# JoeHEZHAO/Optical-Flow-Guided-Feature-Pytorch

Measured on AMD Instinct MI355X. Metric: OFF-forward clips/sec (7-seg 224x224), higher is better.
Workload: dtype f32 (split-fp32: every fp32 operand as three bf16 planes = the fp32 value exactly, six exact plane products on the bf16 MFMA pipe, f32 accumulate); 1 GPU; RGB_OFF forward, batch=64 clips/GPU x 7 segments, nine 224x224-geometry feature maps; global_batch=64, segments=7, parallelism=clip-shard x1, slice_mode=reference_flat

## Files before the change

optical-flow-guided-feature-pytorch_amd/csrc/conv_igemm.hip:

```cpp
#include <cstdio>
#include <cstdlib>

#include "offk_common.h"
#include "offk_internal.h"

namespace offk {

struct ConvArgs {
  const float* x; int x_cs, x_coff;
  int n_img, H, W, Ci, Ho, Wo, pad;
  const float* w;
  const float* bias;
  int Co;
  const float* res; int res_cs, res_coff;
  float* y; int y_cs, y_coff;
  int flags, M;
  int gm, gn, splitk;
  int co_limit;
  int batch;
  int spread;
  long long x_bs, w_bs, y_bs;
  int ngroups, g_batch[4], g_Ci[4];
  long long g_x[4], g_w[4], g_y[4];
  float* pool_part;
  int pool_hw;
  float* partial;
  int no_dma;
  unsigned x_bytes, w_bytes;
#ifdef OFFK_CONV_TIMING
  unsigned long long* dbg;
#endif
#ifdef OFFK_TUNING_KNOBS
  int ablate;
#endif
};

constexpr int kDmaStages = 2;
template <int KH, int KW, int S, int TM, int TN, int WM, int WN, int PREC>
__global__ __launch_bounds__(256, 1) void conv_igemm_kernel(ConvArgs p) {
  static_assert(PREC == 0 || PREC == 2 || PREC == 4, "fp32 core only");
  constexpr bool LEAN = PREC >= 2;
#ifdef OFFK_CONV_TIMING
  const unsigned long long tm_t0 = __builtin_readcyclecounter();
  unsigned long long tm_t1 = 0, tm_t2 = 0, tm_ta = 0;
#endif
  if (p.ngroups > 0) {
    int b = blockIdx.y, ci = p.g_Ci[0], first = 0;
    long long gx = p.g_x[0], gw = p.g_w[0], gy = p.g_y[0];
#pragma unroll
    for (int g = 1; g < 4; ++g) {
      first += p.g_batch[g - 1];
      if (g < p.ngroups && (int)blockIdx.y >= first) { b = blockIdx.y - first; ci = p.g_Ci[g]; gx = p.g_x[g]; gw = p.g_w[g]; gy = p.g_y[g]; }
    }
    p.x += gx + (long long)b * p.M * ci; p.w += gw + (long long)b * p.Co * ci; p.y += gy + (long long)b * p.M * p.Co;
    p.Ci = ci; p.x_cs = ci; p.x_bytes = (unsigned)p.M * (unsigned)ci * 4u; p.w_bytes = (unsigned)p.Co * (unsigned)ci * 4u;
  } else if (gridDim.y > 1) { p.x += blockIdx.y * p.x_bs; p.w += blockIdx.y * p.w_bs; p.y += blockIdx.y * p.y_bs; }
  constexpr bool DMA = PREC == 4;
  constexpr int DST = kDmaStages;
  constexpr int BM = 32 * TM * WM, BN = 32 * TN * WN;
  extern __shared__ __attribute__((aligned(16))) float smem[];
  float* As0 = smem;
  float* Bs0 = smem + 2 * BM * LDS_K;

  const int lane = threadIdx.x & 63, wave = threadIdx.x >> 6;
  const int tid = threadIdx.x & 255;
  const int wm = (wave & 3) / WN, wn = (wave & 3) % WN;
  int lid;
  {
    const int nblk = gridDim.x, bid = blockIdx.x, xcd = bid & 7, q = nblk >> 3, r = nblk & 7;
    lid = (xcd < r ? xcd * (q + 1) : r * (q + 1) + (xcd - r) * q) + (bid >> 3);
  }
  const int nt = lid % p.gn, mt = (lid / p.gn) % p.gm, zs = lid / (p.gn * p.gm);
  const int m0 = mt * BM, n0 = nt * BN;
  constexpr int TAPS = KH * KW;
  const int K = TAPS * p.Ci;
  const int nkt_all = TAPS * (p.Ci / BK);
  const int kt_begin = p.splitk == 1 ? 0 : (int)((long long)nkt_all * zs / p.splitk);
  const int kt_end = p.splitk == 1 ? nkt_all : (int)((long long)nkt_all * (zs + 1) / p.splitk);

  constexpr int RSH = 3, RSTEP = 32;
  constexpr int NRA = BM / RSTEP, NRB = BN / RSTEP;
  constexpr int VA = 1, VB = 1;
  const int kpos = DMA ? 4 * ((tid & 7) ^ ((tid >> 4) & 7)) : 4 * (tid & 7);

  int hi0[NRA], wi0[NRA];
  int pix0[NRA];
  const bool flat = TAPS == 1 && S == 1 && p.pad == 0 && LEAN;
#pragma unroll
  for (int r = 0; r < NRA; ++r) {
    int m = m0 + (tid >> RSH) + RSTEP * r;
    bool ok = m < p.M;
    if (flat) { hi0[r] = ok ? 0 : -100000; wi0[r] = 0; pix0[r] = ok ? m : 0; continue; }
    int mm = ok ? m : 0;
    int img = mm / (p.Ho * p.Wo);
    int rem = mm - img * (p.Ho * p.Wo);
    int ho = rem / p.Wo, wo = rem - ho * p.Wo;
    hi0[r] = ok ? ho * S - p.pad : -100000;
    wi0[r] = wo * S - p.pad;
    pix0[r] = img * p.H * p.W;
  }
  const float* xbase = p.x + p.x_coff + kpos;
  const bool relu_in = p.flags & OFFK_CONV_RELU_IN_;
  const float* wbase = p.w + (size_t)(n0 + (tid >> 3)) * K + 4 * (tid & 7);

  typedef unsigned u32x4 __attribute__((ext_vector_type(4)));
  int rowoff[LEAN ? NRA : 1], woff[LEAN ? NRB : 1];
  unsigned inv[LEAN ? NRA : 1];
  __amdgpu_buffer_rsrc_t xrs, wrs;
  if constexpr (LEAN) {
    const int bias_px = p.pad * p.W + p.pad;
    xrs = __builtin_amdgcn_make_buffer_rsrc(const_cast<float*>(p.x) + p.x_coff - (long)bias_px * p.x_cs, 0,
                                            (int)(p.x_bytes + (unsigned)bias_px * p.x_cs * 4u), 0x00020000);
    wrs = __builtin_amdgcn_make_buffer_rsrc(const_cast<float*>(p.w), 0, (int)p.w_bytes, 0x00020000);
#pragma unroll
    for (int r = 0; r < NRA; ++r) {
      rowoff[r] = hi0[r] < -50000 ? 0 : flat ? (pix0[r] * p.x_cs + kpos) * 4
                                             : ((pix0[r] + (hi0[r] + p.pad) * p.W + (wi0[r] + p.pad)) * p.x_cs + kpos) * 4;
      unsigned m = 0;
#pragma unroll
      for (int kh = 0; kh < KH; ++kh) m |= (unsigned)(hi0[r] + kh) >= (unsigned)p.H ? 1u << kh : 0u;
#pragma unroll
      for (int kw = 0; kw < KW; ++kw) m |= (unsigned)(wi0[r] + kw) >= (unsigned)p.W ? 0x10000u << kw : 0u;
      if (flat) m = hi0[r] < -50000 ? 1u : 0u;
      inv[r] = m;
      if constexpr (TAPS == 1) rowoff[r] = m ? (int)0x80000000 : rowoff[r];
    }
#pragma unroll
    for (int r = 0; r < NRB; ++r) woff[r] = ((n0 + (tid >> 3) + 32 * r) * K + kpos) * 4;
  }
  typedef int i32x4 __attribute__((ext_vector_type(4)));
  i32x4 xdesc = {0, 0, 0, 0}, wdesc = {0, 0, 0, 0};
  unsigned lds_base = 0;
  if constexpr (DMA) {
    const int bias_px = p.pad * p.W + p.pad;
    const unsigned long long xa = reinterpret_cast<unsigned long long>(p.x + p.x_coff - (long)bias_px * p.x_cs);
    const unsigned long long wa = reinterpret_cast<unsigned long long>(p.w);
    xdesc = i32x4{(int)(unsigned)xa, (int)(unsigned)(xa >> 32) & 0xffff, (int)(p.x_bytes + (unsigned)bias_px * p.x_cs * 4u), 0x00020000};
    wdesc = i32x4{(int)(unsigned)wa, (int)(unsigned)(wa >> 32) & 0xffff, (int)p.w_bytes, 0x00020000};
    lds_base = (unsigned)(size_t)((__attribute__((address_space(3))) char*)smem) +
               (unsigned)__builtin_amdgcn_readfirstlane((int)(threadIdx.x >> 6)) * (8 * 128);
  }
  auto dma16 = [&](const i32x4& desc, unsigned lds_addr, int voff, int soff) {
    asm volatile("s_mov_b32 m0, %0\n\ts_nop 0\n\tbuffer_load_dwordx4 %1, %2, %3 offen lds"
                 :: "s"(lds_addr), "v"(voff), "s"(desc), "s"(soff) : "memory", "m0");
  };
  int dm_soff_a = 0, dm_soff_b = 0, dm_kh = 0, dm_kw = 0;
  auto dma_prep = [&](int kt) {
    if constexpr (DMA) {
      int chunk = kt / TAPS, tap = kt - chunk * TAPS, c0 = chunk * BK;
      dm_kh = tap / KW; dm_kw = tap - dm_kh * KW;
      dm_soff_a = ((dm_kh * p.W + dm_kw) * p.x_cs + c0) * 4; dm_soff_b = kt * BK * 4;
    }
  };
  auto dma_piece = [&](const int i, const int stage) {
    if constexpr (DMA) {
      const unsigned la = lds_base + stage * (BM * 128), lb = lds_base + DST * (BM * 128) + stage * (BN * 128);
// ... 639 lines not shown
    default: return hipErrorInvalidConfiguration;
  }
}
template <int KH, int KW, int S>
static hipError_t launch_shape(const ConvArgs& a, int cfg, int prec, hipStream_t st) {
  if (prec != 0) return hipErrorInvalidValue;
  if (a.x_bytes && !(a.flags & OFFK_CONV_RELU_IN_) && !a.no_dma) return launch_prec<KH, KW, S, 4>(a, cfg, st);
  return a.x_bytes ? launch_prec<KH, KW, S, 2>(a, cfg, st) : launch_prec<KH, KW, S, 0>(a, cfg, st);
}

void conv2d_auto_plan(long long M, int Co, int nkt, int* cfg_out, int* splitk_out, int precision) {
  static const int cand[] = {1, 2, 3, 4, 6, 8, 12};
  if (precision == 0) {
    static const int cand32[] = {1, 2, 3, 4, 6, 8, 12, 16, 24, 32, 48, 64};
    const long long blocks = ((M + 63) / 64) * (Co / 64);
    int sk = 1;
    for (int c : cand32) {
      if (c > 1 && nkt / c < (blocks * sk < 512 ? 16 : 24)) break;
      sk = c;
      if (blocks * c >= 3500) break;
    }
    *cfg_out = 3;
    *splitk_out = sk;
    return;
  }
  int cfg = (nkt >= 36 && Co % 128 == 0) ? 4 : 3;
  long long blocks = ((M + kTileBM[cfg] - 1) / kTileBM[cfg]) * (Co / kTileBN[cfg]);
  int sk = 1;
  for (int c : cand) {
    if (nkt / c < 16) break;
    sk = c;
    if (blocks * c >= 1536) break;
  }
  *cfg_out = cfg;
  *splitk_out = sk;
}

hipError_t conv2d_launch(const ConvDesc& d, hipStream_t st, const char** why) {
  *why = nullptr;
  if (d.precision != 0) { *why = "conv2d: precision must be 0 (fp32; the bf16x3 mode was retired in ABI v9)"; return hipErrorInvalidValue; }
  const bool narrow = d.co_limit > 0 && d.co_limit < d.Co;
  if (d.Ci % 32 || d.Co % 64 || d.x_cs % 4 || d.x_coff % 4 || d.y_cs <= 0 || (!narrow && (d.y_cs % 4 || d.y_coff % 4)) ||
      (d.res && (d.res_cs % 4 || d.res_coff % 4))) {
    *why = "conv2d: need Ci % 32 == 0, Co % 64 == 0, 16-byte aligned channel slices";
    return hipErrorInvalidValue;
  }
  ConvArgs a;
  a.x = d.x; a.x_cs = d.x_cs; a.x_coff = d.x_coff;
  a.n_img = d.n_img; a.H = d.H; a.W = d.W; a.Ci = d.Ci; a.pad = d.pad;
  a.Ho = (d.H + 2 * d.pad - d.KH) / d.stride + 1;
  a.Wo = (d.W + 2 * d.pad - d.KW) / d.stride + 1;
  a.w = d.w; a.bias = d.bias; a.Co = d.Co;
  a.res = d.res; a.res_cs = d.res_cs; a.res_coff = d.res_coff;
  a.y = d.y; a.y_cs = d.y_cs; a.y_coff = d.y_coff;
  a.flags = d.flags;
  {
    const unsigned long long xb = ((unsigned long long)d.n_img * d.H * d.W * d.x_cs - d.x_coff) * 4ull;
    const unsigned long long bias = (unsigned long long)(d.pad * d.W + d.pad) * d.x_cs * 4ull;
    const unsigned long long wb = (unsigned long long)d.Co * d.KH * d.KW * d.Ci * 4ull;
    const bool fits = xb + bias < 0x7fffffffull && wb < 0x7fffffffull;
    a.x_bytes = fits ? (unsigned)xb : 0u;
    a.w_bytes = fits ? (unsigned)wb : 0u;
    a.no_dma = 0;
#ifdef OFFK_NO_CONV_DMA
    a.no_dma = 1;
#endif
#ifdef OFFK_TUNING_KNOBS
    { const char* e = getenv("OFFK_CONV_DMA"); if (e && *e == '0') a.no_dma = 1; }
    { const char* e = getenv("OFFK_CONV_LEAN"); if (e && !((atoi(e) >> (d.precision & 1)) & 1)) a.x_bytes = 0; }
#endif
  }
  long long M = (long long)d.n_img * a.Ho * a.Wo;
  if (M <= 0 || M > 0x7fffffffLL - 256) { *why = "conv2d: bad problem size"; return hipErrorInvalidValue; }
  a.M = (int)M;
  const int nkt = d.KH * d.KW * (d.Ci / 32);
  int cfg = d.tile_cfg, sk = d.splitk;
  if (cfg < 0 || sk < 1) conv2d_auto_plan(M, d.Co, nkt, &cfg, &sk, d.precision);
  if (sk > nkt) sk = nkt;
  if (narrow) sk = 1;
  a.co_limit = narrow ? d.co_limit : d.Co;
  a.pool_part = d.pool_part; a.pool_hw = d.pool_hw;
  a.batch = d.batch > 1 ? d.batch : 1; a.x_bs = d.x_bstride; a.w_bs = d.w_bstride; a.y_bs = d.y_bstride;
  a.ngroups = d.ngroups;
  for (int g = 0; g < 4; ++g) { a.g_batch[g] = d.g_batch[g]; a.g_Ci[g] = d.g_Ci[g]; a.g_x[g] = d.g_x[g]; a.g_w[g] = d.g_w[g]; a.g_y[g] = d.g_y[g]; }
  if (d.ngroups > 0) {
    if (d.ngroups > 4 || d.x_coff || d.y_coff || d.y_cs != d.Co) { *why = "conv2d: grouped batches are dense [M][Ci] x [Co][Ci] -> [M][Co] problems"; return hipErrorInvalidValue; }
    int nb = 0;
    for (int g = 0; g < d.ngroups; ++g) {
      if (d.g_Ci[g] < 32 || d.g_Ci[g] % 32 || d.g_batch[g] < 1) { *why = "conv2d: bad batch group"; return hipErrorInvalidValue; }
      nb += d.g_batch[g];
    }
    a.batch = nb;
  }
  if (a.batch > 1) {
    if (d.KH != 1 || d.KW != 1 || d.res || d.pool_part || cfg == 6 || cfg == 7 || cfg == 10 || a.batch > 65535) { *why = "conv2d: batched launches are plain 1x1 GEMMs on a generic tile"; return hipErrorInvalidValue; }
    sk = 1;
  }
  if (d.pool_part) {
    if (d.pool_hw < 32 || cfg == 6 || cfg == 7 || cfg == 10) { *why = "conv2d: pooled partial sums need >= 32 rows per image and a generic tile"; return hipErrorInvalidValue; }
    sk = 1;
  }
  if (sk > 1 && !d.partial) sk = 1;
  while (sk > 1 && d.partial_floats < (size_t)sk * (size_t)M * d.Co) --sk;
  a.splitk = sk; a.partial = d.partial; a.gm = a.gn = 0;
#ifdef OFFK_TUNING_KNOBS
  { const char* e = getenv("OFFK_CONV_ABLATE"); a.ablate = e ? atoi(e) : 0; }
#endif
#ifdef OFFK_CONV_TIMING
  {
    static unsigned long long* dbg = nullptr;
    if (!dbg) { (void)hipMalloc(reinterpret_cast<void**>(&dbg), 128); (void)hipMemset(dbg, 0, 128); }
    a.dbg = dbg;
    if (getenv("OFFK_CONV_TIMING_DUMP")) {
      unsigned long long h[16];
      (void)hipMemcpy(h, dbg, 128, hipMemcpyDeviceToHost);
      fprintf(stderr, "[conv timing] consumer mma %llu barrier %llu ktiles %llu | producer store %llu load-issue %llu barrier %llu\n", h[0], h[1], h[2], h[3], h[4], h[5]);
      if (h[11])
        fprintf(stderr, "[conv timing, LDS-DMA form, wave 0, cycles per block] prologue %.0f (setup %.0f, first tile %.0f)  K loop %.0f (%.1f K-tiles: %.0f per tile)  epilogue %.0f (to the last store's issue %.0f, drain %.0f) | blocks %llu\n",
                (double)h[8] / h[11], (double)h[13] / h[11], (double)(h[8] - h[13]) / h[11], (double)h[9] / h[11], (double)h[12] / h[11], (double)h[9] / (double)h[12],
                (double)h[10] / h[11], (double)h[14] / h[11], (double)(h[10] - h[14]) / h[11], h[11]);
      (void)hipMemset(dbg, 0, 128);
    }
  }
#endif
  const int key = d.KH * 100 + d.KW * 10 + d.stride;
  hipError_t e;
  if (cfg == 10) { *why = "conv2d: tile_cfg 10 (the half-chunk patch kernel) existed for the bf16x3 mode only, retired in ABI v9"; return hipErrorInvalidValue; }
  if (cfg == 6 || cfg == 7) {
    if (narrow || d.KH != d.KW || d.H != d.W || d.pad != d.KH / 2) {
      *why = "conv2d: the patch kernel (tile_cfg 6 / 7) needs a square map and pad = k / 2";
      return hipErrorInvalidValue;
    }
    if (sk > d.Ci / 32) sk = d.Ci / 32;
    a.splitk = sk;
    e = launch_patch_shape(a, d.KH, d.stride, d.H, cfg == 6 ? 4 : 2, d.precision, st);
    if (e == hipErrorInvalidConfiguration) *why = "conv2d: the patch kernel covers 7x7s2@28, 5x5s2@14, 3x3s1@14, 3x3s1@7 with Co % 128 (cfg 6) / % 64 (cfg 7)";
    return e;
  }
  switch (key) {
    case 111: e = launch_shape<1, 1, 1>(a, cfg, d.precision, st); break;
    case 331: e = launch_shape<3, 3, 1>(a, cfg, d.precision, st); break;
    case 552: e = launch_shape<5, 5, 2>(a, cfg, d.precision, st); break;
    case 772: e = launch_shape<7, 7, 2>(a, cfg, d.precision, st); break;
    default: *why = "conv2d: unsupported kernel/stride (have 1x1s1, 3x3s1, 5x5s2, 7x7s2)"; return hipErrorInvalidValue;
  }
  if (e == hipErrorInvalidConfiguration) *why = "conv2d: tile configuration does not divide Co";
  return e;
}

__global__ void pack_oihw_kernel(const float* __restrict__ src, float* __restrict__ dst, int Co, int Ci, int KHW) {
  size_t n = (size_t)Co * Ci * KHW;
  for (size_t i = blockIdx.x * (size_t)blockDim.x + threadIdx.x; i < n; i += (size_t)gridDim.x * blockDim.x) {
    int cl = (int)(i & 31);
    size_t t = i >> 5;
    int tap = (int)(t % KHW);
    t /= KHW;
    int chunk = (int)(t % (Ci >> 5));
    int co = (int)(t / (Ci >> 5));
    dst[i] = src[((size_t)co * Ci + chunk * 32 + cl) * KHW + tap];
  }
}

hipError_t pack_conv_weight_launch(const float* src, int Co, int Ci, int KH, int KW, float* dst, hipStream_t st) {
  size_t n = (size_t)Co * Ci * KH * KW;
  int blocks = (int)((n + 255) / 256);
  if (blocks > 4096) blocks = 4096;
  hipLaunchKernelGGL(pack_oihw_kernel, dim3(blocks), dim3(256), 0, st, src, dst, Co, Ci, KH * KW);
  return hipGetLastError();
}

}
```

optical-flow-guided-feature-pytorch_amd/csrc/offk_api.hip:

```cpp
#include "../../include/offk.h"

#include <algorithm>
#include <cmath>
#include <cstdio>
#include <cstdlib>
#include <cstring>
#include <map>
#include <string>
#include <vector>

#include "offk_internal.h"

using namespace offk;

typedef const void* const* MapPtrs;

static bool path_switch(const char* name, int* min_p = nullptr) {
  const char* e = getenv(name);
  if (e && min_p && atoi(e) > 1) *min_p = atoi(e);
  return !(e && *e == '0');
}

static ConvDesc conv_desc(const float* x, int x_cs, int x_coff, int n_img, int H, int W, int Ci, const float* w, const float* bias, int Co, int KH,
                          int KW, int stride, int pad, const float* res, int res_cs, int res_coff, int flags, float* y, int y_cs, int y_coff,
                          int tile_cfg = -1, int splitk = 0, float* partial = nullptr, size_t partial_floats = 0, int precision = 0) {
  ConvDesc d;
  d.x = x; d.x_cs = x_cs; d.x_coff = x_coff; d.n_img = n_img; d.H = H; d.W = W; d.Ci = Ci;
  d.w = w; d.bias = bias; d.Co = Co; d.KH = KH; d.KW = KW; d.stride = stride; d.pad = pad;
  d.res = res; d.res_cs = res_cs; d.res_coff = res_coff; d.flags = flags;
  d.y = y; d.y_cs = y_cs; d.y_coff = y_coff;
  d.tile_cfg = tile_cfg; d.splitk = splitk; d.partial = partial; d.partial_floats = partial_floats; d.precision = precision;
  return d;
}

static hipError_t wino_gemms_launch(const WinoGroup* grp, int ngrp, int npoints, int rows, int Ci, int Co, const float* V, const float* U,
                                    float* M, bool persistent, hipStream_t s, const char** why, const void* U_planes = nullptr) {
  if (persistent || U_planes) {
    WinoGemmArgs a{};
    a.x = V; a.w = U; a.y = M; a.M = rows; a.Co = Co; a.ngroups = ngrp;
    for (int gi = 0; gi < ngrp; ++gi) {
      a.g_batch[gi] = grp[gi].batch; a.g_K[gi] = grp[gi].kmul * Ci;
      a.g_x[gi] = grp[gi].v_off; a.g_w[gi] = grp[gi].u_off; a.g_y[gi] = grp[gi].m_off;
    }
    a.w_planes = U_planes;
    if (U_planes && wino_gemm_split_supported(a)) return wino_gemm_split_launch(a, s);
    if (persistent && wino_gemm_supported(a)) return wino_gemm_launch(a, s);
  }
  const int K0 = grp[0].kmul * Ci;
  ConvDesc d = conv_desc(V, K0, 0, rows, 1, 1, K0, U, nullptr, Co, 1, 1, 1, 0, nullptr, 0, 0, 0, M, Co, 0, 3, 1);
#ifdef OFFK_TUNING_KNOBS
  { const char* e = getenv("OFFK_WINO_CFG"); if (e && (Co % 128 == 0 || atoi(e) == 1 || atoi(e) == 2)) d.tile_cfg = atoi(e); }
#endif
  d.batch = npoints; d.x_bstride = (long long)rows * K0; d.w_bstride = (long long)Co * K0; d.y_bstride = (long long)rows * Co;
  if (ngrp > 1) {
    d.ngroups = ngrp;
    for (int gi = 0; gi < ngrp; ++gi) {
      d.g_batch[gi] = grp[gi].batch; d.g_Ci[gi] = grp[gi].kmul * Ci;
      d.g_x[gi] = grp[gi].v_off; d.g_w[gi] = grp[gi].u_off; d.g_y[gi] = grp[gi].m_off;
    }
  }
  return conv2d_launch(d, s, why);
}
static bool wino_gemm_stage_default() {
  static const bool on = path_switch("OFFK_WINO_GEMM");
  return on;
}

namespace {

struct SiteSpec { const char* name; int C, H; };
const SiteSpec kSites[kNumSites] = {{"3a", 256, 28}, {"3b", 320, 28}, {"3c", 576, 14}, {"4a", 576, 14}, {"4b", 576, 14},
                                    {"4c", 608, 14}, {"4d", 608, 14}, {"5a", 1024, 7}, {"5b", 1024, 7}};
const int kPwOrder[kNumSites] = {7, 8, 5, 6, 2, 3, 4, 1, 0};
const int kSiteFusion[kNumSites] = {0, 0, 1, 1, 1, 1, 1, 2, 2};
const int kSiteCoff[kNumSites] = {0, 160, 0, 160, 320, 480, 640, 0, 160};
const int kFusionC[3] = {320, 1056, 832};

struct ConvSpec { const char* key; int Co, Ci, K, stride, pad; };
enum ConvId {
  C_T28, C1_28A, C2_28A, C3_28A, CB_28A, C1_28B, C2_28B, C3_28B, C1_28C, C2_28C, C3_28C,
  C_T14, C1_14A, C2_14A, C3_14A, CE_14A, C1_14B, C2_14B, C3_14B,
  C_T7, C1_7, C2_7, C3_7, CB_7, kNumConvs
};
const ConvSpec kConvs[kNumConvs] = {
    {"motion_conv_trans_28", 64, 320, 7, 2, 3},      {"motion_conv1_trans_28a", 64, 64, 1, 1, 0},
    {"motion_conv2_trans_28a", 64, 64, 3, 1, 1},     {"motion_conv3_trans_28a", 256, 64, 1, 1, 0},
    {"motion_conv_branch_28a", 256, 64, 1, 1, 0},    {"motion_conv1_trans_28b", 64, 256, 1, 1, 0},
    {"motion_conv2_trans_28b", 64, 64, 3, 1, 1},     {"motion_conv3_trans_28b", 256, 64, 1, 1, 0},
    {"motion_conv1_trans_28c", 64, 256, 1, 1, 0},    {"motion_conv2_trans_28c", 64, 64, 3, 1, 1},
    {"motion_conv3_trans_28c", 256, 64, 1, 1, 0},    {"motion_conv_trans_14", 128, 1056, 5, 2, 2},
    {"motion_conv1_trans_14a", 128, 128, 1, 1, 0},   {"motion_conv2_trans_14a", 128, 128, 3, 1, 1},
    {"motion_conv3_trans_14a", 512, 128, 1, 1, 0},   {"motion_conv_expand_trans_14a", 512, 128, 1, 1, 0},
    {"motion_conv1_trans_14b", 128, 512, 1, 1, 0},   {"motion_conv2_trans_14b", 128, 128, 3, 1, 1},
    {"motion_conv3_trans_14b", 512, 128, 3, 1, 1},   {"motion_conv_trans", 256, 832, 3, 1, 1},
    {"motion_conv1_trans", 256, 256, 1, 1, 0},       {"motion_conv2_trans", 256, 256, 3, 1, 1},
    {"motion_conv3_trans", 1024, 256, 1, 1, 0},      {"motion_conv_branch_trans", 1024, 256, 1, 1, 0}};
struct MergedSpec { const char* name; int main_id, branch_id; };
const MergedSpec kMerged[3] = {{"merged_28a", C3_28A, CB_28A}, {"merged_14a", C3_14A, CE_14A}, {"merged_7", C3_7, CB_7}};
const int kTunedP240[kNumConvs][2] = {
    {3, 2}, {-1, 0}, {-1, 0}, {-1, 0}, {-1, 0}, {-1, 0}, {-1, 0}, {-1, 0}, {-1, 0}, {-1, 0}, {-1, 0},
    {4, 4}, {-1, 0}, {-1, 0}, {-1, 0}, {-1, 0}, {-1, 0}, {-1, 0}, {-1, 0},
    {-1, 0}, {-1, 0}, {-1, 0}, {-1, 0}, {-1, 0}};
const int kMergedPlan[2][3][2] = {
    {{3, 1}, {3, 1}, {3, 1}},
    {{1, 1}, {3, 1}, {3, 1}}};
struct HeadSpec { const char* key; int C; };
const HeadSpec kHeads[3] = {{"fc_action_motion", 1024}, {"fc_action_motion_28", 256}, {"fc_action_motion_14", 512}};
const char* kSobelKey = "sobel_edge_diagonal.conv.weight";

enum SlotKind { SK_GEN_W, SK_GEN_B, SK_DOWN_W, SK_DOWN_B, SK_DW_W, SK_DW_B, SK_SOBEL, SK_CONV_W, SK_CONV_B, SK_FC_W, SK_FC_B };
struct Slot {
  std::string key;
  std::vector<int64_t> shape;
  SlotKind kind;
  int idx;
  bool set = false;
};

struct Derived {
  float* u = nullptr;
  float* u_planes = nullptr;
  float* u2 = nullptr;
  float* planes = nullptr;
  float* gemm_planes = nullptr;
  float* head = nullptr;
};
constexpr int kNumDerived = kNumConvs + 3;
constexpr int merged_slot(int m) { return kNumConvs + m; }

thread_local std::string g_err;

size_t align_up(size_t v, size_t a) { return (v + a - 1) / a * a; }

}

struct offk_handle {
  offk_config cfg;
  int N = 0, P = 0;
  std::vector<Slot> slots;
  std::map<std::string, int> index;
  float* pw_w[kNumSites] = {};
  float* pw_wt16[kNumSites] = {};
// ... 87 lines not shown

constexpr size_t kTraceMaxEvents = 1 << 16;
int trace_mark(offk_handle* h, hipStream_t st, const char* name) {
  if (h->profiling != 2 || h->tr_marks.size() >= kTraceMaxEvents) return OFFK_OK;
  int id = -1;
  if (name) {
    for (size_t i = 0; i < h->tr_names.size() && id < 0; ++i)
      if (h->tr_names[i] == name) id = (int)i;
    if (id < 0) { id = (int)h->tr_names.size(); h->tr_names.push_back(name); }
  }
  if (h->tr_marks.size() >= h->tr_events.size()) {
    hipEvent_t e;
    HIP_TRY(h, hipEventCreate(&e));
    h->tr_events.push_back(e);
  }
  HIP_TRY(h, hipEventRecord(h->tr_events[h->tr_marks.size()], st));
  h->tr_marks.push_back(id);
  return OFFK_OK;
}

int dev_alloc(offk_handle* h, float** p, size_t nfloats) {
  void* q = nullptr;
  HIP_TRY(h, hipMalloc(&q, nfloats * sizeof(float)));
  HIP_TRY(h, hipMemset(q, 0, nfloats * sizeof(float)));
  h->allocs.push_back(q);
  *p = static_cast<float*>(q);
  return OFFK_OK;
}

void add_slot(offk_handle* h, const std::string& key, std::vector<int64_t> shape, SlotKind kind, int idx) {
  Slot s;
  s.key = key; s.shape = std::move(shape); s.kind = kind; s.idx = idx;
  h->index[key] = (int)h->slots.size();
  h->slots.push_back(std::move(s));
}

void add_region(offk_handle* h, const std::string& name, size_t nfloats) {
  size_t off = align_up(h->ws_bytes, 256);
  h->regions[name] = std::make_pair(off, nfloats * sizeof(float));
  h->ws_bytes = off + nfloats * sizeof(float);
}

float* region(const offk_handle* h, void* ws, const char* name) {
  auto it = h->regions.find(name);
  return reinterpret_cast<float*>(static_cast<char*>(ws) + it->second.first);
}

void ub_plan(int H, int* strips, int* rows) {
  *rows = H >= 28 ? 7 : H;
  *strips = (H + *rows - 1) / *rows;
}
constexpr int kUbTpix = 8;

void plan_workspace(offk_handle* h) {
  const size_t N = h->N, P = h->P;
  for (int s = 0; s < kNumSites; ++s) {
    size_t hw = (size_t)kSites[s].H * kSites[s].H;
    add_region(h, std::string("G_") + kSites[s].name, N * hw * kGenCh);
    add_region(h, std::string("D_") + kSites[s].name, P * hw * kDownCh);
  }
  add_region(h, "fusion_28", P * 784 * 320);
  add_region(h, "fusion_14", P * 196 * 1056);
  add_region(h, "fusion_7", P * 49 * 832);
  add_region(h, "xt_28", P * 196 * 128);
  add_region(h, "t1_28", P * 196 * 64);
  add_region(h, "sa_28", P * 196 * 256);
  add_region(h, "sb_28", P * 196 * 256);
  add_region(h, "xu_14", P * 49 * 256);
  add_region(h, "u1_14", P * 49 * 128);
  add_region(h, "sa_14", P * 49 * 512);
  add_region(h, "xv_7", P * 49 * 512);
  add_region(h, "v1_7", P * 49 * 256);
  add_region(h, "sum_7", P * 49 * 1024);
  add_region(h, "logit_7", P * (size_t)h->cfg.num_classes);
  add_region(h, "logit_14", P * (size_t)h->cfg.num_classes);
  add_region(h, "logit_28", P * (size_t)h->cfg.num_classes);
  add_region(h, "pooled_7", P * 1024);
  add_region(h, "pooled_14", P * 512);
  add_region(h, "pooled_28", P * 256);
  add_region(h, "poolpart_28", (size_t)4 * P * 256);
  add_region(h, "poolpart_7", ((P * 49 + 31) / 32) * 2 * 1024);
  add_region(h, "poolpart_14", ((P * 49 + 31) / 32) * 2 * 512);
  if (h->cfg.precision == OFFK_PRECISION_FP32) {
    add_region(h, "wino_v", std::max((size_t)kWinoUnits4 * P * 1056, (size_t)kWino7Tiles * P * kWino7Units * 320));
    add_region(h, "wino_m", (size_t)kWinoPoints * P * 512);
    add_region(h, "poolpart_14t", (size_t)4 * P * 512);
    if (h->pool_first7) add_region(h, "poolpart_7t", (size_t)4 * P * 512);
  }
  h->splitk_floats = (size_t)std::min<size_t>(64, std::max<size_t>(8, 1536 / P)) * P * 196 * 64;
  add_region(h, "splitk", h->splitk_floats);
  h->ws_bytes = align_up(h->ws_bytes, 256);

  const size_t fwd_bytes = h->ws_bytes;
  long long work = 0;
  for (int s = 0; s < kNumSites; ++s) {
    const int hw = kSites[s].H * kSites[s].H;
    work += (long long)N * ((hw + 31) / 32) * ((kSites[s].C + 127) / 128);
  }
  h->wg_kpb = (int)std::max<long long>(4, (work + 1535) / 1536);
  for (int s = 0; s < kNumSites; ++s) {
    const size_t hw = (size_t)kSites[s].H * kSites[s].H;
    const std::string n = kSites[s].name;
    int strips, rows;
    ub_plan(kSites[s].H, &strips, &rows);
    const size_t kt_total = N * ((hw + 31) / 32), nchunks = (kt_total + h->wg_kpb - 1) / h->wg_kpb;
    const size_t cpad = (size_t)((kSites[s].C + 127) / 128) * 128;
    add_region(h, "dG_" + n, N * hw * kGenCh);
    add_region(h, "dD_" + n, P * hw * kDownCh);
    add_region(h, "dwp_" + n, P * strips * 10 * kDownCh);
    add_region(h, "wgs_" + n, nchunks * kUnitCh * cpad);
    add_region(h, "wgb_" + n, nchunks * kUnitCh);
    auto slot = [&](const std::string& key, size_t count) {
      h->grad_slots[key] = std::make_pair(h->grad_floats, count);
      h->grad_floats += count;
    };
    slot("motion_conv_gen_" + n + ".weight", (size_t)kGenCh * kSites[s].C);
    slot("motion_conv_gen_" + n + ".bias", kGenCh);
    slot("motion_spatial_down_" + n + ".weight", (size_t)kDownCh * kSites[s].C);
    slot("motion_spatial_down_" + n + ".bias", kDownCh);
    if (h->cfg.variant != OFFK_VARIANT_DIAG_SOBEL) {
      slot("motion_spatial_grad_" + n + ".weight", (size_t)kDownCh * 9);
      slot("motion_spatial_grad_" + n + ".bias", kDownCh);
    }
  }
  h->train_ws_bytes = align_up(h->ws_bytes, 256);
  h->ws_bytes = fwd_bytes;
}

struct DeviceGuard {
  int prev = -1;
  bool changed = false;
  explicit DeviceGuard(int want) {
    if (hipGetDevice(&prev) == hipSuccess && prev != want) changed = hipSetDevice(want) == hipSuccess;
  }
  ~DeviceGuard() { if (changed) (void)hipSetDevice(prev); }
};

int check_ready(offk_handle* h) {
  for (const Slot& s : h->slots)
    if (!s.set) return fail(h, OFFK_ERR_MISSING_WEIGHT, "weight not set: " + s.key);
  return OFFK_OK;
}

bool slot_set(const offk_handle* h, const std::string& key) {
  auto it = h->index.find(key);
  return it != h->index.end() && h->slots[it->second].set;
}

int site_weights_ready(offk_handle* h, int site, bool need_pw, bool need_dw) {
  const std::string n = kSites[site].name;
  if (need_pw)
    for (const char* k : {"motion_conv_gen_", "motion_spatial_down_"})
      for (const char* sfx : {".weight", ".bias"})
        if (!slot_set(h, std::string(k) + n + sfx)) return fail(h, OFFK_ERR_MISSING_WEIGHT, std::string("weight not set: ") + k + n + sfx);
  if (need_dw) {
    if (h->cfg.variant == OFFK_VARIANT_DIAG_SOBEL) {
      if (!slot_set(h, kSobelKey)) return fail(h, OFFK_ERR_MISSING_WEIGHT, std::string("weight not set: ") + kSobelKey);
    } else {
      for (const char* sfx : {".weight", ".bias"})
        if (!slot_set(h, "motion_spatial_grad_" + n + sfx)) return fail(h, OFFK_ERR_MISSING_WEIGHT, "weight not set: motion_spatial_grad_" + n + sfx);
    }
  }
  return OFFK_OK;
}

void pw_weight_ptrs(const offk_handle* h, int site, const float** w, const float** w_down, const float** b,
                    const float** b_down) {
// ... 219 lines not shown
  for (int i = 0; i < kNumSites; ++i) {
    const int s = kPwOrder[i];
    PtSite& o = pt.s[i];
    const offk_feat_parts& fp = feats[s];
    for (int q = 0; q < 4; ++q) { o.xp[q] = q < fp.n_parts ? fp.data[q] : nullptr; o.cp[q] = q < fp.n_parts ? fp.channels[q] : 0; }
    o.nparts = fp.n_parts;
    pw_weight_ptrs(h, s, &o.w, &o.w_down, &o.bias, &o.bias_down);
    o.wt = nullptr;
    o.wt16 = h->pw_wt16[s];
    o.wt16s = h->pw_wt16s[s];
    o.D = region(h, ws, (std::string("D_") + kSites[s].name).c_str());
    o.M = region(h, ws, fus[kSiteFusion[s]]);
    o.m_cs = kFusionC[kSiteFusion[s]]; o.m_coff = kSiteCoff[s];
    o.C = kSites[s].C; o.HW = kSites[s].H * kSites[s].H;
  }
  if (ev) HIP_TRY(h, hipEventRecord(ev[0], st));
  TRY(launch_k1t(h, st, pt, feat_dtype, cl));
  if (ev) HIP_TRY(h, hipEventRecord(ev[1], st));
  { int rc = trace_mark(h, st, "units:sobel S-blocks (K2 spatial half)"); if (rc != OFFK_OK) return rc; }
  { int rc = run_sobel_tdiff_all(h, st, ws, 3); if (rc != OFFK_OK) return rc; }
  if (ev) HIP_TRY(h, hipEventRecord(ev[2], st));
  return OFFK_OK;
}

int check_feat_train(offk_handle* h, const FeatKind& k, int feat_dtype, const void* const* feats, int first, int count, const char* fn) {
  const std::string f(fn), maps = std::string(": ") + k.noun + " feature map";
  if (!(feat_dtype == OFFK_FEAT_F32 && k.f32_ok) && feat_dtype != OFFK_FEAT_BF16 && feat_dtype != OFFK_FEAT_F16)
    return fail(h, OFFK_ERR_INVALID, f + ": unknown feat_dtype " + std::to_string(feat_dtype) + " (OFFK_FEAT_F32 / _BF16 / _F16)");
  if (!k.cl && h->cfg.feat_layout == OFFK_FEAT_NHWC) return fail(h, OFFK_ERR_INVALID, f + maps + "s are NCHW-only (this handle is NHWC)");
  for (int i = 0; i < count; ++i) {
    const SiteSpec& site = kSites[first + i];
    if (!feats[i]) return fail(h, OFFK_ERR_INVALID, f + ": null feature map");
    if (reinterpret_cast<uintptr_t>(feats[i]) & (k.align_train - 1))
      return fail(h, OFFK_ERR_INVALID, f + maps + " pointers must be " + std::to_string(k.align_train) + "-byte aligned (site " + site.name + ")");
    if (feat_dtype != OFFK_FEAT_F32 && (unsigned long long)h->N * site.H * site.H * site.C * 2ull >= kFeat16MaxBytes)
      return fail(h, OFFK_ERR_INVALID, f + ": 16-bit feature maps of 2 GiB or more are not supported (site " + site.name + ")");
  }
  return OFFK_OK;
}

int pw_reduce_site(offk_handle* h, void* stream, const FeatKind* k, int feat_dtype, int site, const void* feat, float* G, float* D, const char* fn) {
  if (!h || site < 0 || site >= kNumSites || !feat || !G || !D) return fail(h, OFFK_ERR_INVALID, std::string(fn) + ": bad argument");
  if (k) TRY(check_feat_train(h, *k, feat_dtype, &feat, site, 1, fn));
  TRY(site_weights_ready(h, site, true, false));
  DeviceGuard guard(h->cfg.device);
  hipStream_t st = static_cast<hipStream_t>(stream);
  PwParams pp;
  memset(&pp, 0, sizeof(pp));
  pp.nsites = 1; pp.L = h->cfg.length; pp.P = h->P; pp.slice_mode = h->cfg.slice_mode;
  pp.nhwc = k ? k->cl : h->cfg.feat_layout == OFFK_FEAT_NHWC;
  pp.zeros = h->zero_page;
  TRY(finalize_pw(h, st));
  fill_pw_site(h, site, whole_map(site, static_cast<const float*>(feat)), G, D, &pp.s[0]);
  pp.total_blocks = pw_blocks_for(pp.s[0].M);
  return launch_k1(h, st, pp, feat_dtype, false);
}

int off_units_whole(offk_handle* h, void* stream, const FeatKind* k, int feat_dtype, const void* const feats[OFFK_NUM_SITES], void* workspace,
                    bool train, uint64_t drop_seed, double drop_p, const char* fn) {
  if (!h || !feats || !workspace) return fail(h, OFFK_ERR_INVALID, std::string(fn) + ": null argument");
  DropCfg drop;
  if (train) TRY(make_drop(h, drop_seed, drop_p, &drop));
  if (k) TRY(check_feat_train(h, *k, feat_dtype, feats, 0, kNumSites, fn));
  offk_feat_parts parts[kNumSites];
  TRY(whole_maps(h, feats, parts, fn));
  for (int s = 0; s < kNumSites; ++s) TRY(site_weights_ready(h, s, true, true));
  DeviceGuard guard(h->cfg.device);
  return run_off_units(h, static_cast<hipStream_t>(stream), parts, workspace, nullptr, k ? k->cl : h->cfg.feat_layout == OFFK_FEAT_NHWC, drop,
                       feat_dtype);
}

struct View { const float* p; int cs, coff; };

enum DerivedKind {
  DK_U_F43,
  DK_U_POLY,
  DK_U_F54,
  DK_CHAIN_U2,
  DK_PLANES,
  DK_U_PLANES,
  DK_HEAD_COMPOSED
};
DerivedKind u_kind(const ConvSpec& c) { return c.K == 7 ? DK_U_F54 : c.K == 5 ? DK_U_POLY : DK_U_F43; }
int u_units(DerivedKind k) { return k == DK_U_F54 ? kWino7Units : k == DK_U_POLY ? kWinoUnits4 : kWinoPoints; }
size_t u_elems(const ConvSpec& c) { return (size_t)u_units(u_kind(c)) * c.Co * c.Ci; }
int wino_phases(const ConvSpec& c) { return u_kind(c) == DK_U_POLY ? 4 : 1; }
int wino_conv_groups(const ConvSpec& c, long long rows, WinoGroup grp[4]) {
  return u_kind(c) == DK_U_F54 ? wino7_groups(rows, c.Ci, c.Co, grp) : wino_groups(wino_phases(c), rows, c.Ci, c.Co, grp);
}
size_t plane_floats(size_t elems) { return (elems * 3 + 1) / 2; }

enum { ON_7X7 = 1, ON_SPLIT_GEMM = 2, ON_CHAIN_WINO = 4, ON_SPLIT_CHAIN = 8, ON_SPLIT_MID = 16, ON_POOL_FIRST7 = 32 };
struct DerivedRow {
  int slot;
  DerivedKind kind;
  float* Derived::*image;
  int needs = 0;
  int skip_bit = 0;
  int alloc_K = 0;
};
bool derived_exists(const offk_handle* h, const DerivedRow& r) {
  const int on = h->wino_7x7 * ON_7X7 | h->split_gemm * ON_SPLIT_GEMM | h->chain_wino * ON_CHAIN_WINO | (h->chain && h->split_chain) * ON_SPLIT_CHAIN |
                 (h->wino_mid && h->split_mid) * ON_SPLIT_MID | h->pool_first7 * ON_POOL_FIRST7;
  const bool shape = r.kind != DK_U_PLANES || (kConvs[r.slot].Co % 64 == 0 && kConvs[r.slot].Ci >= 64);
  return h->winograd && !(r.needs & ~on) && shape && !(h->split_gemm_skip & r.skip_bit);
}

const DerivedRow kDerived[] = {
    {C3_14B, DK_U_F43, &Derived::u}, {C_T7, DK_U_F43, &Derived::u}, {C2_7, DK_U_F43, &Derived::u}, {C2_14A, DK_U_F43, &Derived::u},
    {C2_14B, DK_U_F43, &Derived::u}, {C_T14, DK_U_POLY, &Derived::u}, {C_T28, DK_U_F54, &Derived::u, ON_7X7},
    {C3_14B, DK_U_PLANES, &Derived::u_planes, ON_SPLIT_GEMM, 1}, {C_T7, DK_U_PLANES, &Derived::u_planes, ON_SPLIT_GEMM, 2},
    {C2_7, DK_U_PLANES, &Derived::u_planes, ON_SPLIT_GEMM, 4}, {C2_14A, DK_U_PLANES, &Derived::u_planes, ON_SPLIT_GEMM, 8},
    {C2_14B, DK_U_PLANES, &Derived::u_planes, ON_SPLIT_GEMM, 16}, {C_T14, DK_U_PLANES, &Derived::u_planes, ON_SPLIT_GEMM, 32},
    {C_T28, DK_U_PLANES, &Derived::u_planes, ON_7X7 | ON_SPLIT_GEMM, 64},
    {merged_slot(1), DK_PLANES, &Derived::gemm_planes, ON_SPLIT_GEMM, 128}, {merged_slot(2), DK_PLANES, &Derived::gemm_planes, ON_SPLIT_GEMM, 128},
    {C1_14B, DK_PLANES, &Derived::gemm_planes, ON_SPLIT_GEMM, 128},
    {C2_28A, DK_CHAIN_U2, &Derived::u2, ON_CHAIN_WINO}, {C2_28B, DK_CHAIN_U2, &Derived::u2, ON_CHAIN_WINO}, {C2_28C, DK_CHAIN_U2, &Derived::u2, ON_CHAIN_WINO},
    {C1_28A, DK_PLANES, &Derived::planes, ON_SPLIT_CHAIN, 0, 256}, {C2_28A, DK_PLANES, &Derived::planes, ON_SPLIT_CHAIN}, {C3_28A, DK_PLANES, &Derived::planes, ON_SPLIT_CHAIN},
    {CB_28A, DK_PLANES, &Derived::planes, ON_SPLIT_CHAIN},
    {C1_28B, DK_PLANES, &Derived::planes, ON_SPLIT_CHAIN}, {C2_28B, DK_PLANES, &Derived::planes, ON_SPLIT_CHAIN}, {C3_28B, DK_PLANES, &Derived::planes, ON_SPLIT_CHAIN},
    {C1_28C, DK_PLANES, &Derived::planes, ON_SPLIT_CHAIN}, {C2_28C, DK_PLANES, &Derived::planes, ON_SPLIT_CHAIN}, {C3_28C, DK_PLANES, &Derived::planes, ON_SPLIT_CHAIN},
    {C1_14A, DK_PLANES, &Derived::planes, ON_SPLIT_MID}, {C1_7, DK_PLANES, &Derived::planes, ON_SPLIT_MID},
    {merged_slot(2), DK_HEAD_COMPOSED, &Derived::head, ON_POOL_FIRST7}};

struct Matrix { const float* w; int Co, K; };
Matrix slot_matrix(const offk_handle* h, int slot) {
  if (slot < kNumConvs) return Matrix{h->conv_w[slot], kConvs[slot].Co, kConvs[slot].Ci * kConvs[slot].K * kConvs[slot].K};
  const MergedSpec& m = kMerged[slot - kNumConvs];
  return Matrix{h->merged_w[slot - kNumConvs], kConvs[m.main_id].Co, kConvs[m.main_id].Ci + kConvs[m.branch_id].Ci};
}
size_t derived_floats(const offk_handle* h, const DerivedRow& r) {
  switch (r.kind) {
    case DK_U_F43: case DK_U_POLY: case DK_U_F54: return (size_t)u_units(r.kind) * kConvs[r.slot].Co * kConvs[r.slot].Ci;
    case DK_CHAIN_U2: return (size_t)16 * 64 * 64;
    case DK_PLANES: { const Matrix m = slot_matrix(h, r.slot); return plane_floats((size_t)m.Co * (r.alloc_K ? r.alloc_K : m.K)); }
    case DK_U_PLANES: return plane_floats(u_elems(kConvs[r.slot]));
    case DK_HEAD_COMPOSED: return (size_t)h->cfg.num_classes * (slot_matrix(h, r.slot).K + 1);
  }
  return 0;
}
int pack_derived(offk_handle* h, const DerivedRow& r, hipStream_t st) {
  const Derived& d = h->derived[r.slot];
  switch (r.kind) {
    case DK_U_F43: case DK_U_POLY:
      HIP_TRY(h, wino_weight_launch(h->conv_w[r.slot], kConvs[r.slot].Co, kConvs[r.slot].Ci, wino_phases(kConvs[r.slot]), d.u, st));
      break;
    case DK_U_F54: HIP_TRY(h, wino7_weight_launch(h->conv_w[r.slot], kConvs[r.slot].Co, kConvs[r.slot].Ci, d.u, st)); break;
    case DK_CHAIN_U2: HIP_TRY(h, chain_wino_weight_launch(h->conv_w[r.slot], d.u2, st)); break;
    case DK_PLANES: {
      const Matrix m = slot_matrix(h, r.slot);
      HIP_TRY(h, wino_pack_split_launch(m.w, d.*r.image, m.Co, m.K, 1, st));
      break;
    }
    case DK_U_PLANES: {
      const ConvSpec& c = kConvs[r.slot];
      WinoGroup grp[4];
      const int ngrp = wino_conv_groups(c, 1, grp);
      for (int g = 0; g < ngrp; ++g)
        HIP_TRY(h, wino_pack_split_launch(d.u + grp[g].u_off, reinterpret_cast<char*>(d.u_planes) + grp[g].u_off * 6, c.Co, grp[g].kmul * c.Ci, grp[g].batch, st));
      break;
    }
    case DK_HEAD_COMPOSED: {
      const Matrix m = slot_matrix(h, r.slot);
      HIP_TRY(h, head_compose_launch(h->fc_w[0], h->fc_b[0], h->cfg.num_classes, m.w, h->merged_b[r.slot - kNumConvs], m.Co, m.K, d.head,
                                     d.head + (size_t)h->cfg.num_classes * m.K, st));
      break;
    }
  }
  return OFFK_OK;
}

int finalize_merged(offk_handle* h, hipStream_t st) {
  if (!h->merged_dirty) return OFFK_OK;
  for (int m = 0; m < 3; ++m) {
    const ConvSpec& a = kConvs[kMerged[m].main_id];
    const ConvSpec& b = kConvs[kMerged[m].branch_id];
    const size_t K = (size_t)a.Ci + b.Ci;
    HIP_TRY(h, hipMemcpy2DAsync(h->merged_w[m], K * 4, h->conv_w[kMerged[m].main_id], (size_t)a.Ci * 4, (size_t)a.Ci * 4, a.Co, hipMemcpyDeviceToDevice, st));
    HIP_TRY(h, hipMemcpy2DAsync(h->merged_w[m] + a.Ci, K * 4, h->conv_w[kMerged[m].branch_id], (size_t)b.Ci * 4, (size_t)b.Ci * 4, a.Co, hipMemcpyDeviceToDevice, st));
    HIP_TRY(h, vec_add_launch(h->conv_b[kMerged[m].main_id], h->conv_b[kMerged[m].branch_id], h->merged_b[m], a.Co, st));
  }
  h->merged_dirty = false;
  return OFFK_OK;
}
int finalize_derived(offk_handle* h, hipStream_t st) {
  if (!h->derived_dirty) return OFFK_OK;
  for (const DerivedRow& r : kDerived)
    if (h->derived[r.slot].*r.image) TRY(pack_derived(h, r, st));
  h->derived_dirty = false;
  return OFFK_OK;
}

constexpr int RI = OFFK_CONV_RELU_IN_, RP = OFFK_CONV_RELU_PRE_, RO = OFFK_CONV_RELU_POST_;
int trace_mark(offk_handle* h, hipStream_t st, const char* key, const char* what) {
  return h->profiling != 2 ? OFFK_OK : trace_mark(h, st, (std::string(key) + what).c_str());
}
WinoMidArgs wino_mid_args(const float* M, const float* bias_in, int phases_in, int n_img, int Cin, float* x, int x_cs, int x_coff, const float* w1,
                          const float* b1, int Cmid, float* V, const void* w1p = nullptr) {
  WinoMidArgs m;
  m.M = M; m.bias_in = bias_in; m.phases_in = phases_in; m.x = x; m.x_cs = x_cs; m.x_coff = x_coff;
  m.w1 = w1; m.b1 = b1; m.Cin = Cin; m.Cmid = Cmid; m.n_img = n_img; m.V = V; m.w1p = w1p;
  return m;
}
ChainArgs chain_args(const float* x, int x_cs, int x_coff, int n_img, int Cin, int relu_in, const float* w1, const float* b1, const float* w2,
                     const float* b2, const float* w3, const float* b3, int K3, const float* res, int res_cs, int res_coff, float* y, int y_cs,
                     int y_coff) {
  ChainArgs a{};
  a.x = x; a.x_cs = x_cs; a.x_coff = x_coff; a.Cin = Cin; a.relu_in = relu_in ? 1 : 0;
  a.w1 = w1; a.b1 = b1; a.w2 = w2; a.b2 = b2; a.w3 = w3; a.b3 = b3; a.K3 = K3;
  a.res = res; a.res_cs = res_cs; a.res_coff = res_coff; a.y = y; a.y_cs = y_cs; a.y_coff = y_coff;
  a.n_img = n_img; a.relu_out = 1;
  const unsigned long long xb = ((unsigned long long)n_img * 196 * x_cs - x_coff) * 4ull;
  a.x_bytes = xb < 0x7fffffffull ? (unsigned)xb : 0u;
  return a;
}

struct Fwd {
  offk_handle* h;
  hipStream_t s;
  void* ws;
  int n;
  hipEvent_t* ev = nullptr;
  float *F14, *F7;
  float *wino_V, *wino_M;
  float* splitk;
  float *out7, *out14, *out28;
  float *l7, *l14, *l28;
  FcPooledJobs fcj{};
  bool wino, w7, mid, w5, chained, fold, fold14t, pool7;

  float* reg(const char* name) const { return region(h, ws, name); }

  int init(offk_handle* handle, hipStream_t st, void* workspace, float* o7, float* o14, float* o28, bool stage_only = false) {
    h = handle; s = st; ws = workspace; n = h->P; out7 = o7; out14 = o14; out28 = o28;
    if (h->profiling == 1 && !stage_only) {
      const size_t per = OFFK_NUM_STAGES + 1;
      if ((h->ev_used + 1) * per > h->events.size() && h->events.size() < 4096 * per) {
        for (size_t i = 0; i < per; ++i) {
          hipEvent_t e;
          HIP_TRY(h, hipEventCreate(&e));
          h->events.push_back(e);
        }
      }
      if ((h->ev_used + 1) * per <= h->events.size()) ev = &h->events[h->ev_used++ * per];
    }
    wino = h->winograd;
    w7 = h->derived[C_T28].u && wino && h->wino_7x7 && n >= h->wino7_min_p;
    mid = wino && h->wino_mid;
    w5 = wino && h->wino_5x5 && n >= h->wino5_min_p;
    chained = h->chain && n >= h->chain_min_p && (unsigned long long)n * 196 * 256 * 4ull < 0x7fffffffull;
    auto generic = [](int cfg) { return cfg != 6 && cfg != 7 && cfg != 10; };
    fold = h->fold_pool && generic(h->conv_cfg[C3_14B]) && generic(h->merged_cfg[2]);
    fold14t = wino && h->fold_pool;
    pool7 = h->pool_first7 && mid && fold14t && h->derived[merged_slot(2)].head;
    F14 = reg("fusion_14"); F7 = reg("fusion_7"); splitk = reg("splitk");
    wino_V = wino ? reg("wino_v") : nullptr;
    wino_M = wino ? reg("wino_m") : nullptr;
    const bool cons = h->cfg.consensus == OFFK_CONSENSUS_AVG;
    l7 = cons ? reg("logit_7") : out7; l14 = cons ? reg("logit_14") : out14; l28 = cons ? reg("logit_28") : out28;
    fcj.n_img = n; fcj.ncls = h->cfg.num_classes;
    return OFFK_OK;
  }

  int conv_raw(const char* name, int Co, int Ci, int K, int stride, int pad, const float* w, const float* bias, int cfg, int sk, int H, View x,
               const float* res, int res_cs, int res_coff, int flags, float* y, int y_cs, int y_coff, const void* w_planes, float* pool_part) {
    if (w_planes && K == 1 && stride == 1 && pad == 0 && !res && !(flags & OFFK_CONV_RELU_IN_)) {
      WinoGemmArgs a{};
      a.x = x.p; a.w = w; a.y = y; a.M = n * H * H; a.Co = Co; a.ngroups = 1; a.g_batch[0] = 1; a.g_K[0] = Ci;
      a.w_planes = w_planes;
      a.epilogue = 1; a.x_rs = x.cs; a.x_coff = x.coff; a.y_rs = y_cs; a.y_coff = y_coff; a.bias = bias;
      a.relu = (flags & (OFFK_CONV_RELU_PRE_ | OFFK_CONV_RELU_POST_)) ? 1 : 0;
      a.pool_part = pool_part; a.pool_hw = pool_part ? H * H : 0;
      if (wino_gemm_split_supported(a)) {
        TRY(trace_mark(h, s, name));
        hipError_t e = wino_gemm_split_launch(a, s);
        if (e != hipSuccess) return fail_hip(h, e, name);
        return OFFK_OK;
      }
    }
    ConvDesc d = conv_desc(x.p, x.cs, x.coff, n, H, H, Ci, w, bias, Co, K, K, stride, pad, res, res_cs, res_coff, flags, y, y_cs, y_coff, cfg, sk,
                           splitk, h->splitk_floats, h->cfg.precision);
    d.pool_part = pool_part; d.pool_hw = pool_part ? H * H / (stride * stride) : 0;
    const char* why = nullptr;
    TRY(trace_mark(h, s, name));
    hipError_t e = conv2d_launch(d, s, &why);
    if (e != hipSuccess) return fail(h, why ? OFFK_ERR_INVALID : OFFK_ERR_HIP, std::string(name) + ": " + (why ? why : hipGetErrorString(e)));
    return OFFK_OK;
  }
  int conv(ConvId id, int H, View x, const float* res, int res_cs, int res_coff, int flags, float* y, int y_cs, int y_coff, float* pool_part = nullptr) {
    const ConvSpec& c = kConvs[id];
    return conv_raw(c.key, c.Co, c.Ci, c.K, c.stride, c.pad, h->conv_w[id], h->conv_b[id], h->conv_cfg[id], h->conv_splitk[id], H, x, res, res_cs,
                    res_coff, flags, y, y_cs, y_coff, h->derived[id].gemm_planes, pool_part);
  }
  int conv_merged(int m, int H, View x, int flags, float* y, int y_cs, int y_coff, float* pool_part = nullptr) {
    const Matrix w = slot_matrix(h, merged_slot(m));
    return conv_raw(kMerged[m].name, w.Co, w.K, 1, 1, 0, w.w, h->merged_b[m], h->merged_cfg[m], h->merged_sk[m], H, x, nullptr, 0, 0, flags, y, y_cs,
                    y_coff, h->derived[merged_slot(m)].gemm_planes, pool_part);
  }

  int wino_in(ConvId id, View x) {
    const ConvSpec& c = kConvs[id];
    TRY(trace_mark(h, s, c.key, " [winograd: input transform]"));
    if (u_kind(c) == DK_U_F54) HIP_TRY(h, wino7_input_launch(x.p, x.cs, x.coff, n, c.Ci, wino_V, s));
    else HIP_TRY(h, wino_input_launch(x.p, x.cs, x.coff, n, c.Ci, wino_phases(c), wino_V, s));
    return OFFK_OK;
  }
  int wino_mm(ConvId id) {
    const ConvSpec& c = kConvs[id];
    const bool f54 = u_kind(c) == DK_U_F54;
    TRY(trace_mark(h, s, c.key, f54 ? " [winograd: 64 GEMMs]" : " [winograd: 121 GEMMs]"));
    const int rows = f54 ? kWino7Tiles * n : n;
    WinoGroup grp[4];
    const int ngrp = wino_conv_groups(c, rows, grp);
    const char* why = nullptr;
    hipError_t e = wino_gemms_launch(grp, ngrp, f54 ? kWino7Points : kWinoPoints, rows, c.Ci, c.Co, wino_V, h->derived[id].u, wino_M, h->wino_gemm, s, &why,
                                     h->derived[id].u_planes);
    if (e != hipSuccess) return fail(h, why ? OFFK_ERR_INVALID : OFFK_ERR_HIP, std::string(c.key) + " (winograd): " + (why ? why : hipGetErrorString(e)));
    return OFFK_OK;
  }
  int wino_out(ConvId id, const float* res, int res_cs, int res_coff, int flags, float* y, int y_cs, int y_coff, float* pool_t, int pool_cs = 0) {
    const ConvSpec& c = kConvs[id];
    TRY(trace_mark(h, s, c.key, " [winograd: output transform]"));
    if (u_kind(c) == DK_U_F54) HIP_TRY(h, wino7_output_launch(wino_M, n, c.Co, h->conv_b[id], flags, y, y_cs, y_coff, s));
    else HIP_TRY(h, wino_output_launch(wino_M, n, c.Co, wino_phases(c), h->conv_b[id], res, res_cs, res_coff, flags, y, y_cs, y_coff, pool_t, s, pool_cs, 0));
    return OFFK_OK;
  }
  int wino_conv(ConvId id, View x, const float* res, int res_cs, int res_coff, int flags, float* y, int y_cs, int y_coff, float* pool_t) {
    TRY(wino_in(id, x));
    TRY(wino_mm(id));
    return wino_out(id, res, res_cs, res_coff, flags, y, y_cs, y_coff, pool_t);
  }
  int wino_between(ConvId a, ConvId c1, float* xa, int xa_cs, int xa_coff, const char* name, float* pool_t = nullptr) {
    const bool has = c1 != kNumConvs;
    WinoMidArgs m = wino_mid_args(wino_M, h->conv_b[a], wino_phases(kConvs[a]), n, kConvs[a].Co, xa, xa_cs, xa_coff, has ? h->conv_w[c1] : nullptr,
                                        has ? h->conv_b[c1] : nullptr, kConvs[has ? c1 : a].Co, wino_V, has ? h->derived[c1].planes : nullptr);
    m.pool_part = pool_t; m.pool_cs = xa_cs; m.pool_coff = xa_coff;
    TRY(trace_mark(h, s, name));
    HIP_TRY(h, wino_mid_launch(m, s));
    return OFFK_OK;
  }
  int conv_t_c1_c2(ConvId ct, bool wino_t, int H, View F, ConvId c1, ConvId c2, float* xx, int cs, float* t, const char* between,
                   float* pool_t = nullptr) {
    const int half = cs / 2;
    if (wino_t && mid) {
      TRY(wino_in(ct, F));
      TRY(wino_mm(ct));
      TRY(wino_between(ct, c1, xx, cs, half, between, pool_t));
      TRY(wino_mm(c2));
      return wino_out(c2, nullptr, 0, 0, RP, xx, cs, 0, pool_t, pool_t ? cs : 0);
    }
    if (wino_t) TRY(wino_conv(ct, F, nullptr, 0, 0, RP, xx, cs, half, nullptr));
    else TRY(conv(ct, H, F, nullptr, 0, 0, RP, xx, cs, half));
    TRY(conv(c1, 7, View{xx, cs, half}, nullptr, 0, 0, RP, t, half, 0));
    if (wino) return wino_conv(c2, View{t, half, 0}, nullptr, 0, 0, RP, xx, cs, 0, nullptr);
    return conv(c2, 7, View{t, half, 0}, nullptr, 0, 0, RP, xx, cs, 0);
  }

  int chain(const char* name, View x, int Cin, int relu_in, ConvId c1, ConvId c2, ConvId c3, int m, bool split_branch, const float* res, float* y, int y_cs, int y_coff) {
    const bool merged = m >= 0 && !split_branch;
    ChainArgs a = chain_args(x.p, x.cs, x.coff, n, Cin, relu_in, h->conv_w[c1], h->conv_b[c1], h->conv_w[c2], h->conv_b[c2],
                             merged ? h->merged_w[m] : h->conv_w[c3], merged ? h->merged_b[m] : h->conv_b[c3], merged ? 128 : 64, res, 256, 0, y, y_cs, y_coff);
    a.u2 = h->derived[c2].u2;
    a.w1p = h->derived[c1].planes; a.w2p = h->derived[c2].planes; a.w3p = h->derived[c3].planes;
    if (split_branch) { a.wbp = h->derived[kMerged[m].branch_id].planes; a.bbr = h->conv_b[kMerged[m].branch_id]; }
    TRY(trace_mark(h, s, name));
    const char* why = nullptr;
    hipError_t e = chain14_split_supported(a) ? chain14_split_launch(a, s, &why) : chain14_launch(a, s, &why);
    if (e != hipSuccess) return fail(h, why ? OFFK_ERR_INVALID : OFFK_ERR_HIP, std::string(name) + ": " + (why ? why : hipGetErrorString(e)));
    return OFFK_OK;
  }

  int head(int k, float* logits, const float* part, int tiles, const float* x, int x_cs, int x_coff, int Hh, int maxpool, const char* pooled_name) {
    const int C = kHeads[k].C;
    if (part) { fcj.job[fcj.njobs++] = FcPooledJob{part, 49, tiles, C, h->fc_w[k], h->fc_b[k], logits}; return OFFK_OK; }
    float* pooled = reg(pooled_name);
    TRY(trace_mark(h, s, k == 0 ? "head_7 (pool + fc)" : k == 1 ? "head_28 (pool + fc)" : "head_14 (pool + fc)"));
    hipError_t e = pool_launch(x, x_cs, x_coff, n, Hh, Hh, C, maxpool, pooled, s);
    if (e == hipSuccess) e = fc_launch(pooled, n, C, h->fc_w[k], h->fc_b[k], h->cfg.num_classes, logits, s);
    if (e != hipSuccess) return fail_hip(h, e, "head");
    return OFFK_OK;
  }

  int units(const offk_feat_parts feats[], int feat_dtype, bool cl) {
    if (cl) return run_off_units_fused(h, s, feats, ws, ev, feat_dtype, true);
    if (h->fused_units && h->cfg.feat_layout != OFFK_FEAT_NHWC) return run_off_units_fused(h, s, feats, ws, ev, feat_dtype);
    return run_off_units(h, s, feats, ws, ev, h->cfg.feat_layout == OFFK_FEAT_NHWC);
  }

  int fusion28() {
    float *F28 = reg("fusion_28"), *xt = reg("xt_28"), *t1 = reg("t1_28"), *sa = reg("sa_28"), *sb = reg("sb_28");
    if (w7) TRY(wino_conv(C_T28, View{F28, 320, 0}, nullptr, 0, 0, 0, xt, 128, 64, nullptr));
    else TRY(conv(C_T28, 28, View{F28, 320, 0}, nullptr, 0, 0, 0, xt, 128, 64));
    if (chained) {
      TRY(chain("chain_28a = motion_conv1_trans_28a + motion_conv2_trans_28a + merged_28a", View{xt, 128, 64}, 64, 1, C1_28A, C2_28A, C3_28A, 0,
                h->derived[CB_28A].planes != nullptr, nullptr, sa, 256, 0));
      TRY(chain("chain_28b = motion_conv1_trans_28b + motion_conv2_trans_28b + motion_conv3_trans_28b", View{sa, 256, 0}, 256, 0, C1_28B, C2_28B, C3_28B,
// ... 909 lines not shown
  if (!x || !w || !y || n_img < 1 || H < 1 || W < 1) return fail(nullptr, OFFK_ERR_INVALID, "offk_conv2d: bad argument");
  return offk_conv2d_ex(stream, x, x_cstride, x_coff, n_img, H, W, Ci, w, bias, Co, KH, KW, stride, pad, res, res_cstride, res_coff, flags, y,
                        y_cstride, y_coff, -1, 0, nullptr, 0, 0);
}

int offk_conv2d_ex(void* stream, const float* x, int x_cstride, int x_coff, int n_img, int H, int W, int Ci, const float* w,
                   const float* bias, int Co, int KH, int KW, int stride, int pad, const float* res, int res_cstride,
                   int res_coff, int flags, float* y, int y_cstride, int y_coff, int tile_cfg, int splitk, float* partial,
                   size_t partial_floats, int precision) {
  if (!x || !w || !y || n_img < 1 || H < 1 || W < 1) return fail(nullptr, OFFK_ERR_INVALID, "offk_conv2d_ex: bad argument");
  const ConvDesc d = conv_desc(x, x_cstride, x_coff, n_img, H, W, Ci, w, bias, Co, KH, KW, stride, pad, res, res_cstride, res_coff, flags, y,
                               y_cstride, y_coff, tile_cfg, splitk, partial, partial_floats, precision);
  const char* why = nullptr;
  hipError_t e = conv2d_launch(d, static_cast<hipStream_t>(stream), &why);
  if (e != hipSuccess) return fail(nullptr, why ? OFFK_ERR_INVALID : OFFK_ERR_HIP, why ? why : hipGetErrorString(e));
  return OFFK_OK;
}

int offk_bottleneck_chain14(void* stream, const float* x, int x_cstride, int x_coff, int n_img, int Cin, int relu_in,
                            const float* w1, const float* b1, const float* w2_packed, const float* b2, const float* w3,
                            const float* b3, int K3, const float* res, int res_cstride, int res_coff, float* y, int y_cstride,
                            int y_coff) {
  if (!x || !w1 || !b1 || !w2_packed || !b2 || !w3 || !b3 || !y || n_img < 1)
    return fail(nullptr, OFFK_ERR_INVALID, "offk_bottleneck_chain14: bad argument");
  const ChainArgs a = chain_args(x, x_cstride, x_coff, n_img, Cin, relu_in, w1, b1, w2_packed, b2, w3, b3, K3, res, res_cstride, res_coff, y,
                                 y_cstride, y_coff);
  const char* why = nullptr;
  hipError_t e = chain14_launch(a, static_cast<hipStream_t>(stream), &why);
  if (e != hipSuccess) return fail(nullptr, why ? OFFK_ERR_INVALID : OFFK_ERR_HIP, why ? why : hipGetErrorString(e));
  return OFFK_OK;
}

int offk_bottleneck_chain14_split(void* stream, const float* x, int x_cstride, int x_coff, int n_img, int Cin, int relu_in,
                                  const float* w1, const float* b1, const float* w2_packed, const float* b2, const float* w3,
                                  const float* b3, const float* branch_w, const float* branch_b, const float* res, int res_cstride,
                                  int res_coff, float* y, int y_cstride, int y_coff, void* scratch, size_t scratch_bytes) {
  const char* who = "offk_bottleneck_chain14_split";
  if (!x || !w1 || !b1 || !w2_packed || !b2 || !w3 || !b3 || !y || !scratch || n_img < 1 || (Cin != 64 && Cin != 256) || (branch_w && !branch_b))
    return fail(nullptr, OFFK_ERR_INVALID, std::string(who) + ": bad argument");
  if (x_coff < 0 || y_coff < 0 || (res && res_coff < 0)) return fail(nullptr, OFFK_ERR_INVALID, std::string(who) + ": negative channel offset");
  if (x_cstride < x_coff + Cin) return fail(nullptr, OFFK_ERR_INVALID, std::string(who) + ": x_cstride < x_coff + Cin");
  if (y_cstride < y_coff + 256) return fail(nullptr, OFFK_ERR_INVALID, std::string(who) + ": y_cstride < y_coff + 256");
  if (res && res_cstride < res_coff + 256) return fail(nullptr, OFFK_ERR_INVALID, std::string(who) + ": res_cstride < res_coff + 256");
  if (branch_w && res) return fail(nullptr, OFFK_ERR_INVALID, std::string(who) + ": the branch form takes no residual (res must be NULL)");
  {
    const size_t rows = (size_t)n_img * 196 * sizeof(float);
    const uintptr_t y0 = reinterpret_cast<uintptr_t>(y), y1 = y0 + rows * (size_t)y_cstride;
    const uintptr_t x0 = reinterpret_cast<uintptr_t>(x), x1 = x0 + rows * (size_t)x_cstride;
    if (y0 < x1 && x0 < y1) return fail(nullptr, OFFK_ERR_INVALID, std::string(who) + ": y overlaps x (the chain does not run in place)");
    if (res) {
      const uintptr_t r0 = reinterpret_cast<uintptr_t>(res), r1 = r0 + rows * (size_t)res_cstride;
      if (y0 < r1 && r0 < y1) return fail(nullptr, OFFK_ERR_INVALID, std::string(who) + ": y overlaps res (the chain does not run in place)");
    }
  }
  const size_t e1 = (size_t)64 * Cin, e2 = (size_t)64 * 576, e3 = (size_t)256 * 64;
  if (scratch_bytes < 6 * (e1 + e2 + 2 * e3)) return fail(nullptr, OFFK_ERR_INVALID, std::string(who) + ": scratch too small");
  hipStream_t st = static_cast<hipStream_t>(stream);
  char* sp = static_cast<char*>(scratch);
  ChainArgs a = chain_args(x, x_cstride, x_coff, n_img, Cin, relu_in, w1, b1, w2_packed, b2, w3, b3, 64, res, res_cstride, res_coff, y, y_cstride,
                           y_coff);
  a.w1p = sp; a.w2p = sp + 6 * e1; a.w3p = sp + 6 * (e1 + e2);
  hipError_t e = wino_pack_split_launch(w1, const_cast<void*>(a.w1p), 64, Cin, 1, st);
  if (e == hipSuccess) e = wino_pack_split_launch(w2_packed, const_cast<void*>(a.w2p), 64, 576, 1, st);
  if (e == hipSuccess) e = wino_pack_split_launch(w3, const_cast<void*>(a.w3p), 256, 64, 1, st);
  if (e == hipSuccess && branch_w) {
    a.wbp = sp + 6 * (e1 + e2 + e3); a.bbr = branch_b;
    e = wino_pack_split_launch(branch_w, const_cast<void*>(a.wbp), 256, 64, 1, st);
  }
  if (e != hipSuccess) return fail_hip(nullptr, e, who);
  const char* why = nullptr;
  e = chain14_split_launch(a, st, &why);
  if (e != hipSuccess) return fail(nullptr, why ? OFFK_ERR_INVALID : OFFK_ERR_HIP, std::string(who) + ": " + (why ? why : hipGetErrorString(e)));
  return OFFK_OK;
}

namespace {
int winograd_entry(const char* who, void* stream, const float* x, int x_cstride, int x_coff, int n_img, int Ci, int phases,
                   const float* w_packed, const float* bias, int Co, const float* res, int res_cstride, int res_coff, int flags,
                   float* y, int y_cstride, int y_coff, float* scratch, size_t scratch_floats, float* pool_part) {
  if (!x || !w_packed || !y || !scratch || n_img < 1 || Ci < 32 || (Ci & 31) || Co < 64 || (Co & 63) || (flags & OFFK_CONV_RELU_IN_))
    return fail(nullptr, OFFK_ERR_INVALID, std::string(who) + ": bad argument (Ci % 32 == 0, Co % 64 == 0, no RELU_IN)");
  const bool f54 = phases == 7;
  const size_t T = f54 ? (size_t)kWino7Tiles * n_img : (size_t)n_img;
  const size_t units = f54 ? kWino7Units : phases == 4 ? kWinoUnits4 : kWinoPoints, points = f54 ? kWino7Points : kWinoPoints;
  const size_t need = units * Ci * ((size_t)Co + T) + points * T * Co;
  if (scratch_floats < need) return fail(nullptr, OFFK_ERR_INVALID, std::string(who) + ": scratch too small");
  hipStream_t st = static_cast<hipStream_t>(stream);
  float* U = scratch;
  float* V = U + units * Co * Ci;
  float* M = V + units * T * Ci;
  hipError_t e = f54 ? wino7_weight_launch(w_packed, Co, Ci, U, st) : wino_weight_launch(w_packed, Co, Ci, phases, U, st);
  if (e == hipSuccess) e = f54 ? wino7_input_launch(x, x_cstride, x_coff, n_img, Ci, V, st) : wino_input_launch(x, x_cstride, x_coff, n_img, Ci, phases, V, st);
  if (e != hipSuccess) return fail_hip(nullptr, e, who);
  WinoGroup grp[4];
  const int ngrp = f54 ? wino7_groups((long long)T, Ci, Co, grp) : wino_groups(phases, (long long)T, Ci, Co, grp);
  {
    const char* why = nullptr;
    e = wino_gemms_launch(grp, ngrp, (int)points, (int)T, Ci, Co, V, U, M, wino_gemm_stage_default(), st, &why);
    if (e != hipSuccess) return fail(nullptr, why ? OFFK_ERR_INVALID : OFFK_ERR_HIP, why ? why : hipGetErrorString(e));
  }
  e = f54 ? wino7_output_launch(M, n_img, Co, bias, flags, y, y_cstride, y_coff, st)
          : wino_output_launch(M, n_img, Co, phases, bias, res, res_cstride, res_coff, flags, y, y_cstride, y_coff, pool_part, st);
  if (e != hipSuccess) return fail_hip(nullptr, e, who);
  return OFFK_OK;
}
}

int offk_winograd_conv3x3(void* stream, const float* x, int x_cstride, int x_coff, int n_img, int Ci, const float* w_packed,
                          const float* bias, int Co, const float* res, int res_cstride, int res_coff, int flags, float* y,
                          int y_cstride, int y_coff, float* scratch, size_t scratch_floats, float* pool_part) {
  return winograd_entry("offk_winograd_conv3x3", stream, x, x_cstride, x_coff, n_img, Ci, 1, w_packed, bias, Co, res, res_cstride,
                        res_coff, flags, y, y_cstride, y_coff, scratch, scratch_floats, pool_part);
}

int offk_winograd_conv5x5s2(void* stream, const float* x, int x_cstride, int x_coff, int n_img, int Ci, const float* w_packed,
                            const float* bias, int Co, const float* res, int res_cstride, int res_coff, int flags, float* y,
                            int y_cstride, int y_coff, float* scratch, size_t scratch_floats) {
  return winograd_entry("offk_winograd_conv5x5s2", stream, x, x_cstride, x_coff, n_img, Ci, 4, w_packed, bias, Co, res, res_cstride,
                        res_coff, flags, y, y_cstride, y_coff, scratch, scratch_floats, nullptr);
}

int offk_winograd_conv7x7s2(void* stream, const float* x, int x_cstride, int x_coff, int n_img, int Ci, const float* w_packed,
                            const float* bias, int Co, int flags, float* y, int y_cstride, int y_coff, float* scratch,
                            size_t scratch_floats) {
  return winograd_entry("offk_winograd_conv7x7s2", stream, x, x_cstride, x_coff, n_img, Ci, 7, w_packed, bias, Co, nullptr, 0, 0, flags, y, y_cstride,
                        y_coff, scratch, scratch_floats, nullptr);
}

int offk_winograd_between(void* stream, const float* M, const float* bias_in, int phases_in, int n_img, int Cin, float* x,
                          int x_cstride, int x_coff, const float* w1, const float* b1, int Cmid, float* V) {
  const char* who = "offk_winograd_between";
  if (!M || !V || n_img < 1 || (w1 && !b1) || (x && (x_cstride < x_coff + Cin || (x_cstride & 3) || (x_coff & 3) || x_coff < 0)))
    return fail(nullptr, OFFK_ERR_INVALID, std::string(who) + ": bad argument");
  if (!wino_mid_supported(Cin, Cmid, w1 != nullptr, phases_in))
    return fail(nullptr, OFFK_ERR_INVALID, std::string(who) + ": shape not built ((Cin, Cmid) = (128, 128) / (256, 256); phases_in 1, or 4 with Cin 128)");
  hipError_t e = wino_mid_launch(wino_mid_args(M, bias_in, phases_in, n_img, Cin, x, x_cstride, x_coff, w1, b1, Cmid, V), static_cast<hipStream_t>(stream));
  if (e != hipSuccess) return fail_hip(nullptr, e, who);
  return OFFK_OK;
}

int offk_winograd_between_ex(void* stream, const float* M, const float* bias_in, int phases_in, int n_img, int Cin, float* x,
                             int x_cstride, int x_coff, const float* w1, const float* b1, int Cmid, float* V, int precision,
                             void* scratch, size_t scratch_bytes) {
  const char* who = "offk_winograd_between_ex";
  if (precision == OFFK_PRECISION_FP32) return offk_winograd_between(stream, M, bias_in, phases_in, n_img, Cin, x, x_cstride, x_coff, w1, b1, Cmid, V);
  if (precision != OFFK_PRECISION_F32SPLIT || !w1 || !b1 || !scratch || scratch_bytes < (size_t)Cmid * Cin * 6)
    return fail(nullptr, OFFK_ERR_INVALID, std::string(who) + ": split-fp32 needs the 1x1 conv and Cmid * Cin * 6 bytes of scratch");
  if (!M || !V || n_img < 1 || (x && (x_cstride < x_coff + Cin || (x_cstride & 3) || (x_coff & 3) || x_coff < 0)))
    return fail(nullptr, OFFK_ERR_INVALID, std::string(who) + ": bad argument");
  if (!wino_mid_supported(Cin, Cmid, true, phases_in))
    return fail(nullptr, OFFK_ERR_INVALID, std::string(who) + ": shape not built ((Cin, Cmid) = (128, 128) / (256, 256); phases_in 1, or 4 with Cin 128)");
  hipStream_t st = static_cast<hipStream_t>(stream);
  hipError_t e = wino_pack_split_launch(w1, scratch, Cmid, Cin, 1, st);
  if (e != hipSuccess) return fail_hip(nullptr, e, who);
  e = wino_mid_launch(wino_mid_args(M, bias_in, phases_in, n_img, Cin, x, x_cstride, x_coff, w1, b1, Cmid, V, scratch), st);
  if (e != hipSuccess) return fail_hip(nullptr, e, who);
  return OFFK_OK;
}

int offk_batched_gemm_nt(void* stream, const float* x, const float* w, float* y, int batch, int M, int K, int Co, int precision,
                         void* scratch, size_t scratch_bytes) {
  const char* who = "offk_batched_gemm_nt";
  if (!x || !w || !y || batch < 1 || M < 1 || K < 32 || (K & 31) || Co < 64 || (Co & 63))
    return fail(nullptr, OFFK_ERR_INVALID, std::string(who) + ": bad argument (K % 32 == 0, Co % 64 == 0)");
  if (precision != OFFK_PRECISION_FP32 && precision != OFFK_PRECISION_F32SPLIT)
    return fail(nullptr, OFFK_ERR_INVALID, std::string(who) + ": precision must be OFFK_PRECISION_FP32 or OFFK_PRECISION_F32SPLIT");
  hipStream_t st = static_cast<hipStream_t>(stream);
  WinoGroup grp{batch, 1, 0, 0, 0};
  const void* planes = nullptr;
  if (precision == OFFK_PRECISION_F32SPLIT) {
    if (K < 64) return fail(nullptr, OFFK_ERR_INVALID, std::string(who) + ": the split-fp32 form takes K >= 64");
    if (!scratch || scratch_bytes < (size_t)batch * Co * K * 6)
      return fail(nullptr, OFFK_ERR_INVALID, std::string(who) + ": scratch smaller than batch * Co * K * 6 bytes (the plane image of w)");
    hipError_t e = wino_pack_split_launch(w, scratch, Co, K, batch, st);
    if (e != hipSuccess) return fail_hip(nullptr, e, who);
    planes = scratch;
  }
  const char* why = nullptr;
  hipError_t e = wino_gemms_launch(&grp, 1, batch, M, K, Co, x, w, y, true, st, &why, planes);
  if (e != hipSuccess) return fail(nullptr, why ? OFFK_ERR_INVALID : OFFK_ERR_HIP, std::string(who) + ": " + (why ? why : hipGetErrorString(e)));
  return OFFK_OK;
}

int offk_set_conv_plan(offk_handle* h, const char* conv_key, int tile_cfg, int splitk) {
  if (!h || !conv_key) return fail(h, OFFK_ERR_INVALID, "offk_set_conv_plan: null argument");
  for (int c = 0; c < kNumConvs; ++c)
    if (!strcmp(kConvs[c].key, conv_key)) {
      h->conv_cfg[c] = tile_cfg < 0 ? -1 : tile_cfg;
      h->conv_splitk[c] = splitk < 1 ? 0 : splitk;
      return OFFK_OK;
    }
  for (int m = 0; m < 3; ++m)
    if (!strcmp(kMerged[m].name, conv_key)) {
      h->merged_cfg[m] = tile_cfg < 0 ? -1 : tile_cfg;
      h->merged_sk[m] = splitk < 1 ? 0 : splitk;
      return OFFK_OK;
    }
  return fail(h, OFFK_ERR_UNKNOWN_KEY, std::string("offk_set_conv_plan: unknown conv ") + conv_key);
}

int offk_pack_conv_weight(void* stream, const float* w_oihw, int Co, int Ci, int KH, int KW, float* w_ohwi) {
  if (!w_oihw || !w_ohwi || Co < 1 || Ci < 32 || (Ci & 31) || KH < 1 || KW < 1) return fail(nullptr, OFFK_ERR_INVALID, "offk_pack_conv_weight: bad argument (Ci % 32 == 0)");
  hipError_t e = pack_conv_weight_launch(w_oihw, Co, Ci, KH, KW, w_ohwi, static_cast<hipStream_t>(stream));
  if (e != hipSuccess) return fail_hip(nullptr, e, "offk_pack_conv_weight");
  return OFFK_OK;
}

int offk_head(void* stream, const float* x, int x_cstride, int x_coff, int n_img, int H, int W, int C, int maxpool,
              const float* fc_w, const float* fc_b, int num_classes, float* out) {
  if (!x || !fc_w || !fc_b || !out) return fail(nullptr, OFFK_ERR_INVALID, "offk_head: null argument");
  const char* why = nullptr;
  hipError_t e = head_launch(x, x_cstride, x_coff, n_img, H, W, C, maxpool, fc_w, fc_b, num_classes, out,
                             static_cast<hipStream_t>(stream), &why);
  if (e != hipSuccess) return fail(nullptr, why ? OFFK_ERR_INVALID : OFFK_ERR_HIP, why ? why : hipGetErrorString(e));
  return OFFK_OK;
}

int offk_segment_consensus(void* stream, const float* x, int B, int T, int C, float* out) {
  if (!x || !out || B < 1 || T < 1 || C < 1) return fail(nullptr, OFFK_ERR_INVALID, "offk_segment_consensus: bad argument");
  hipError_t e = consensus_launch(x, B, T, C, out, static_cast<hipStream_t>(stream));
  if (e != hipSuccess) return fail_hip(nullptr, e, "offk_segment_consensus");
  return OFFK_OK;
}

int offk_score_fusion(void* stream, const float* const* scores, const float* weights, int n_sets, int videos, int crops,
                      int classes, float* fused, int32_t* pred) {
  if (!scores || !weights || !fused || n_sets < 1 || n_sets > 8 || videos < 1 || crops < 1 || classes < 1)
    return fail(nullptr, OFFK_ERR_INVALID, "offk_score_fusion: bad argument (1..8 score sets)");
  for (int i = 0; i < n_sets; ++i)
    if (!scores[i]) return fail(nullptr, OFFK_ERR_INVALID, "offk_score_fusion: null score set");
  hipError_t e = score_fusion_launch(scores, weights, n_sets, videos, crops, classes, fused, pred, static_cast<hipStream_t>(stream));
  if (e != hipSuccess) return fail_hip(nullptr, e, "offk_score_fusion");
  return OFFK_OK;
}

int offk_nchw_to_nhwc(void* stream, const float* src, int n_img, int C, int HW, float* dst) {
  if (!src || !dst || n_img < 1 || n_img > 65535 || C < 1 || HW < 1) return fail(nullptr, OFFK_ERR_INVALID, "offk_nchw_to_nhwc: bad argument");
  hipError_t e = nchw_to_nhwc_launch(src, n_img, C, HW, dst, static_cast<hipStream_t>(stream));
  if (e != hipSuccess) return fail_hip(nullptr, e, "offk_nchw_to_nhwc");
  return OFFK_OK;
}

int offk_nhwc_to_nchw(void* stream, const float* src, int cstride, int coff, int n_img, int C, int HW, float* dst) {
  if (!src || !dst || n_img < 1 || n_img > 65535 || C < 1 || HW < 1 || coff < 0 || coff + C > cstride)
    return fail(nullptr, OFFK_ERR_INVALID, "offk_nhwc_to_nchw: bad argument");
  hipError_t e = nhwc_to_nchw_launch(src, cstride, coff, n_img, C, HW, dst, static_cast<hipStream_t>(stream));
  if (e != hipSuccess) return fail_hip(nullptr, e, "offk_nhwc_to_nchw");
  return OFFK_OK;
}

}
// ... 1 lines not shown
```

optical-flow-guided-feature-pytorch_amd/csrc/offk_common.h:

```cpp
#pragma once
#include <hip/hip_runtime.h>
#include <stdint.h>

namespace offk {

typedef float f32x16 __attribute__((ext_vector_type(16)));

constexpr int BK = 32;
constexpr int LDS_K = BK + 4;

template <int TM, int TN>
struct WaveAcc {
  f32x16 acc[TM][TN];

  __device__ __forceinline__ void zero() {
#pragma unroll
    for (int a = 0; a < TM; ++a)
#pragma unroll
      for (int b = 0; b < TN; ++b)
#pragma unroll
        for (int r = 0; r < 16; ++r) acc[a][b][r] = 0.f;
  }

  __device__ __forceinline__ void mma_ktile(const float* As, const float* Bs, int lane) {
    const int r = lane & 31, h = lane >> 5;
    float4 a[2][TM], b[2][TN];
    auto rd = [&](int g, float4 (&aa)[TM], float4 (&bb)[TN]) {
#pragma unroll
      for (int t = 0; t < TM; ++t)
        aa[t] = *reinterpret_cast<const float4*>(As + (t * 32 + r) * LDS_K + 8 * g + 4 * h);
#pragma unroll
      for (int t = 0; t < TN; ++t)
        bb[t] = *reinterpret_cast<const float4*>(Bs + (t * 32 + r) * LDS_K + 8 * g + 4 * h);
    };
    rd(0, a[0], b[0]);
#pragma unroll
    for (int g = 0; g < BK / 8; ++g) {
      if (g + 1 < BK / 8) rd(g + 1, a[(g + 1) & 1], b[(g + 1) & 1]);
      __builtin_amdgcn_sched_barrier(0);
#pragma unroll
      for (int tm = 0; tm < TM; ++tm)
#pragma unroll
        for (int tn = 0; tn < TN; ++tn) {
          acc[tm][tn] = __builtin_amdgcn_mfma_f32_32x32x2f32(a[g & 1][tm].x, b[g & 1][tn].x, acc[tm][tn], 0, 0, 0);
          acc[tm][tn] = __builtin_amdgcn_mfma_f32_32x32x2f32(a[g & 1][tm].y, b[g & 1][tn].y, acc[tm][tn], 0, 0, 0);
          acc[tm][tn] = __builtin_amdgcn_mfma_f32_32x32x2f32(a[g & 1][tm].z, b[g & 1][tn].z, acc[tm][tn], 0, 0, 0);
          acc[tm][tn] = __builtin_amdgcn_mfma_f32_32x32x2f32(a[g & 1][tm].w, b[g & 1][tn].w, acc[tm][tn], 0, 0, 0);
        }
      __builtin_amdgcn_sched_barrier(0);
    }
  }
};

typedef __bf16 bf16x8 __attribute__((ext_vector_type(8)));

__device__ __forceinline__ int xcd_contiguous(int j, int n) {
#ifdef OFFK_NO_XCD_REMAP
  return j;
#endif
  const int c = j & 7, idx = j >> 3, q = n >> 3, r = n & 7;
  return (c < r ? c * (q + 1) : r * (q + 1) + (c - r) * q) + idx;
}

__device__ __forceinline__ int acc_row(int reg, int h) { return (reg & 3) + 8 * (reg >> 2) + 4 * h; }

__device__ __forceinline__ float4 relu4(float4 v) {
  return make_float4(fmaxf(v.x, 0.f), fmaxf(v.y, 0.f), fmaxf(v.z, 0.f), fmaxf(v.w, 0.f));
}

__host__ __device__ __forceinline__ unsigned long long mix64(unsigned long long z) {
  z = (z ^ (z >> 30)) * 0xBF58476D1CE4E5B9ull;
  z = (z ^ (z >> 27)) * 0x94D049BB133111EBull;
  return z ^ (z >> 31);
}
__device__ __forceinline__ float4 drop_mul(unsigned long long base, unsigned long long q, unsigned thresh, float scale) {
  const unsigned long long u = mix64(base + (q + 1) * 0x9E3779B97F4A7C15ull);
  return make_float4(((unsigned)u & 0xFFFFu) >= thresh ? scale : 0.f, ((unsigned)(u >> 16) & 0xFFFFu) >= thresh ? scale : 0.f,
                     ((unsigned)(u >> 32) & 0xFFFFu) >= thresh ? scale : 0.f, (unsigned)(u >> 48) >= thresh ? scale : 0.f);
}

}
```

optical-flow-guided-feature-pytorch_amd/csrc/offk_internal.h:

```cpp
#pragma once
#include <hip/hip_runtime.h>
#include <stddef.h>
#include <stdint.h>

namespace offk {

hipError_t lds_attr_once(const void* kernel, int bytes);

constexpr int OFFK_CONV_RELU_IN_ = 1, OFFK_CONV_RELU_PRE_ = 2, OFFK_CONV_RELU_POST_ = 4;
constexpr int kNumSites = 9;
constexpr int kGenCh = 128, kDownCh = 32, kUnitCh = 160;

struct ConvDesc {
  const float* x; int x_cs, x_coff;
  int n_img, H, W, Ci;
  const float* w;
  const float* bias;
  int Co, KH, KW, stride, pad;
  const float* res; int res_cs, res_coff;
  int flags;
  float* y; int y_cs, y_coff;
  int tile_cfg = -1, splitk = 0;
  float* partial = nullptr;
  size_t partial_floats = 0;
  int precision = 0;
  int co_limit = 0;
  int batch = 1;
  long long x_bstride = 0, w_bstride = 0, y_bstride = 0;
  int ngroups = 0;
  int g_batch[4] = {0, 0, 0, 0}, g_Ci[4] = {0, 0, 0, 0};
  long long g_x[4] = {0, 0, 0, 0}, g_w[4] = {0, 0, 0, 0}, g_y[4] = {0, 0, 0, 0};
  float* pool_part = nullptr;
  int pool_hw = 0;
};
void conv2d_auto_plan(long long M, int Co, int nkt, int* cfg_out, int* splitk_out, int precision);
hipError_t conv2d_launch(const ConvDesc& d, hipStream_t st, const char** why);
hipError_t pack_conv_weight_launch(const float* src, int Co, int Ci, int KH, int KW, float* dst, hipStream_t st);

struct ChainArgs {
  const float* x; int x_cs, x_coff;
  int Cin;
  int relu_in;
  const float* w1; const float* b1;
  const float* w2; const float* b2;
  const float* u2;
  const float* w3; const float* b3;
  int K3;
  const float* res; int res_cs, res_coff;
  float* y; int y_cs, y_coff;
  int n_img, relu_out;
  unsigned x_bytes;
  const void* w1p = nullptr; const void* w2p = nullptr; const void* w3p = nullptr;
  const void* wbp = nullptr; const float* bbr = nullptr;
#ifdef OFFK_CHAIN_TIMING
  unsigned long long* dbg;
#endif
};
hipError_t chain14_launch(const ChainArgs& a, hipStream_t st, const char** why);
bool chain14_split_supported(const ChainArgs& a);
hipError_t chain14_split_launch(const ChainArgs& a, hipStream_t st, const char** why);
hipError_t chain_wino_weight_launch(const float* w2_packed, float* U, hipStream_t st);

constexpr int kWinoPoints = 121, kWinoUnits4 = 400;
hipError_t wino_weight_launch(const float* w_packed, int Co, int Ci, int phases, float* U, hipStream_t st);
hipError_t wino_input_launch(const float* x, int x_cs, int x_coff, int n_img, int Ci, int phases, float* V, hipStream_t st);
hipError_t wino_output_launch(const float* M, int n_img, int Co, int phases, const float* bias, const float* res, int res_cs,
                              int res_coff, int flags, float* y, int y_cs, int y_coff, float* pool_part, hipStream_t st, int pool_cs = 0,
                              int pool_coff = 0);
struct WinoGroup { int batch, kmul; long long v_off, u_off, m_off; };
int wino_groups(int phases, long long rows, int Ci, int Co, WinoGroup out[4]);
struct WinoGemmArgs {
  const float* x; const float* w; float* y;
  int M, Co;
  int ngroups, g_batch[4], g_K[4];
  long long g_x[4], g_w[4], g_y[4];
  int gm, gn, total_items;
  const void* w_planes = nullptr;
  long long x_bytes = 0, w_bytes = 0, y_bytes = 0;
  int epilogue = 0, x_rs = 0, x_coff = 0, y_rs = 0, y_coff = 0, relu = 0, pool_hw = 0;
  const float* bias = nullptr;
  float* pool_part = nullptr;
};
bool wino_gemm_supported(const WinoGemmArgs& a);
hipError_t wino_gemm_launch(const WinoGemmArgs& a, hipStream_t st);
bool wino_gemm_split_supported(const WinoGemmArgs& a);
hipError_t wino_gemm_split_launch(const WinoGemmArgs& a, hipStream_t st);
hipError_t wino_pack_split_launch(const float* U, void* img, int Co, int K, int nproblems, hipStream_t st);
struct WinoMidArgs {
  const float* M;
  const float* bias_in;
  int phases_in;
  float* x; int x_cs, x_coff;
  const float* w1;
  const float* b1;
  int Cin, Cmid, n_img;
  float* V;
  int nsplit = 0;
  const void* w1p = nullptr;
  float* pool_part = nullptr;
  int pool_cs = 0, pool_coff = 0;
};
bool wino_mid_supported(int Cin, int Cmid, bool gemm, int phases_in);
hipError_t wino_mid_launch(const WinoMidArgs& a, hipStream_t st);
constexpr int kWino7Units = 225, kWino7Points = 64, kWino7Tiles = 9;
hipError_t wino7_weight_launch(const float* w_packed, int Co, int Ci, float* U, hipStream_t st);
hipError_t wino7_input_launch(const float* x, int x_cs, int x_coff, int n_img, int Ci, float* V, hipStream_t st);
hipError_t wino7_output_launch(const float* M, int n_img, int Co, const float* bias, int flags, float* y, int y_cs, int y_coff, hipStream_t st);
int wino7_groups(long long T, int Ci, int Co, WinoGroup out[4]);

struct PwSite {
  const float* xp[4];
  int cp[4];
  int nparts;
  const float* w;
  const float* w_down;
  const float* bias;
  const float* bias_down;
  float* G;
  float* D;
  int C, HW, M;
  int blk_begin;
};
struct PwParams {
  PwSite s[kNumSites];
  int nsites, total_blocks;
  int L, P, slice_mode, nhwc;
  const float* zeros;
#ifdef OFFK_TUNING_KNOBS
  int ablate;
#endif
};
int pw_blocks_for(int M);
hipError_t pw_reduce_launch(const PwParams& p, hipStream_t st);
constexpr int kFeatF32 = 0, kFeatBf16 = 1, kFeatF16 = 2;
constexpr int kFeatCl = 4;
bool pw_reduce_feat16_supported(const PwParams& p);
hipError_t pw_reduce_feat16_launch(const PwParams& p, int feat_dtype, hipStream_t st);
hipError_t pw_reduce_cl16_launch(const PwParams& p, int feat_dtype, hipStream_t st);

struct UfsSite {
  const float* xp[4];
  int cp[4];
  int nparts;
  const float* wg;
  const float* wd;
  void* wimg;
  const float* bias;
  const float* bias_down;
  float* G;
  float* D;
  int C, HW, M;
  int blk_begin;
  int pack_begin;
};
struct UfsParams {
  UfsSite s[kNumSites];
  int nsites, total_blocks, pack_blocks, L, P, slice_mode;
};
int units_fwd_split_pack_blocks(int C);
size_t units_fwd_split_image_bytes(int C);
hipError_t units_fwd_split_pack_launch(const UfsParams& p, hipStream_t st);
hipError_t units_fwd_split_launch(const UfsParams& p, int feat_dtype, bool cl, hipStream_t st);

struct PtSite {
  const float* xp[4];
  int cp[4];
  int nparts;
  const float* w;
  const float* w_down;
  const float* wt;
  const float* wt16;
  const void* wt16s;
  const float* bias;
  const float* bias_down;
  float* D;
  float* M;
  int m_cs, m_coff;
  int C, HW;
  int chunks;
  int nrem;
  int rsh;
  int qpc;
  int blk_begin;
};
struct PtParams {
  PtSite s[kNumSites];
  int nsites, total_blocks;
  int B, L, P, slice_mode, tgroups;
  int f32split;
  int bdirect;
  const float* zeros;
// ... 174 lines not shown
```

optical-flow-guided-feature-pytorch_amd/csrc/wino_gemm.hip:

```cpp
#include <cstdio>
#include <cstdlib>

#include "offk_common.h"
#include "offk_internal.h"

namespace offk {

namespace {
typedef int i32x4 __attribute__((ext_vector_type(4)));
typedef float f32x16 __attribute__((ext_vector_type(16)));
constexpr int WG_BM = 64, WG_BN = 64;
constexpr int WG_STAGE = (WG_BM + WG_BN) * 128;
constexpr int WG_LDS = 2 * WG_STAGE;
constexpr int WG_RESIDENT = 4 * 256;
}

__global__ __launch_bounds__(256) void wino_gemm_kernel(WinoGemmArgs p) {
  extern __shared__ __attribute__((aligned(16))) char wg_lds[];
  const int tid = threadIdx.x, lane = tid & 63;
  const int wave = __builtin_amdgcn_readfirstlane(tid >> 6);
  const int wm = wave >> 1, wn = wave & 1;
  const int r32 = lane & 31, hh = lane >> 5;
  const unsigned lds_base = (unsigned)(size_t)((__attribute__((address_space(3))) char*)wg_lds);

  const int lrow = tid >> 3, kpos = 4 * ((tid & 7) ^ ((tid >> 4) & 7));
  const unsigned dma_dst = lds_base + (unsigned)wave * (8 * 128);
  auto dma16 = [&](const i32x4& desc, unsigned lds_addr, int voff, int soff) {
    asm volatile("s_mov_b32 m0, %0\n\ts_nop 0\n\tbuffer_load_dwordx4 %1, %2, %3 offen lds"
                 :: "s"(lds_addr), "v"(voff), "s"(desc), "s"(soff) : "memory", "m0");
  };
  const int sw = hh ^ ((r32 >> 1) & 7);
  int aoff[4], boff[4];
#pragma unroll
  for (int g = 0; g < 4; ++g) {
    aoff[g] = (wm * 32 + r32) * 128 + ((sw ^ (2 * g)) << 4);
    boff[g] = WG_BM * 128 + (wn * 32 + r32) * 128 + ((sw ^ (2 * g)) << 4);
  }

  const int gx = p.gm * p.gn;
  const int nK0 = p.g_K[0], nK1 = p.g_K[1], nK2 = p.g_K[2], nK3 = p.g_K[3];
  const int nB0 = p.g_batch[0], nB1 = p.g_batch[1], nB2 = p.g_batch[2];
  const long long oX0 = p.g_x[0], oX1 = p.g_x[1], oX2 = p.g_x[2], oX3 = p.g_x[3];
  const long long oW0 = p.g_w[0], oW1 = p.g_w[1], oW2 = p.g_w[2], oW3 = p.g_w[3];
  const long long oY0 = p.g_y[0], oY1 = p.g_y[1], oY2 = p.g_y[2], oY3 = p.g_y[3];
  const int ngroups = p.ngroups, argM = p.M, argCo = p.Co, gn = p.gn, total_items = p.total_items;
  const float* const argx = p.x; const float* const argw = p.w; float* const argy = p.y;
  struct Item {
    i32x4 adesc, bdesc;
    int a_off[2], b_off[2];
    int nkt;
    float* y;
    int m0, n0;
  };
  auto locate = [&](int l, Item& it) {
    const int prob = __builtin_amdgcn_readfirstlane(l / gx), bx = l - prob * gx;
    const int xcd = bx & 7, q = gx >> 3, r = gx & 7;
    const int lid = (xcd < r ? xcd * (q + 1) : r * (q + 1) + (xcd - r) * q) + (bx >> 3);
    const int mt = __builtin_amdgcn_readfirstlane(lid / gn), nt = lid - mt * gn;
    int b = prob, K = nK0;
    long long ox = oX0, ow = oW0, oy = oY0;
    if (ngroups > 1 && prob >= nB0) { b = prob - nB0; K = nK1; ox = oX1; ow = oW1; oy = oY1; }
    if (ngroups > 2 && prob >= nB0 + nB1) { b = prob - nB0 - nB1; K = nK2; ox = oX2; ow = oW2; oy = oY2; }
    if (ngroups > 3 && prob >= nB0 + nB1 + nB2) { b = prob - nB0 - nB1 - nB2; K = nK3; ox = oX3; ow = oW3; oy = oY3; }
    const float* xa = argx + ox + (long long)b * argM * K;
    const float* wa = argw + ow + (long long)b * argCo * K;
    it.y = argy + oy + (long long)b * argM * argCo;
    const unsigned long long xu = reinterpret_cast<unsigned long long>(xa), wu = reinterpret_cast<unsigned long long>(wa);
    auto sc = [](int v) { return __builtin_amdgcn_readfirstlane(v); };
    it.adesc = i32x4{sc((int)(unsigned)xu), sc((int)(unsigned)(xu >> 32) & 0xffff), sc(argM * K * 4), 0x00020000};
    it.bdesc = i32x4{sc((int)(unsigned)wu), sc((int)(unsigned)(wu >> 32) & 0xffff), sc(argCo * K * 4), 0x00020000};
    it.m0 = mt * WG_BM; it.n0 = nt * WG_BN; it.nkt = sc(K >> 5);
#pragma unroll
    for (int r = 0; r < 2; ++r) {
      const int m = it.m0 + lrow + 32 * r;
      it.a_off[r] = m < argM ? (m * K + kpos) * 4 : (int)0x80000000;
      it.b_off[r] = ((it.n0 + lrow + 32 * r) * K + kpos) * 4;
    }
  };
  auto dma_piece = [&](const Item& it, const int i, int t, const int st) {
    const unsigned dst = dma_dst + st * WG_STAGE + (i < 2 ? i * 32 * 128 : WG_BM * 128 + (i - 2) * 32 * 128);
    const int soff = __builtin_amdgcn_readfirstlane(t * 128);
#ifdef OFFK_WG_ABLATE
    if (i < 2) dma16(it.adesc, dst, (OFFK_WG_ABLATE & 1) ? (int)0x80000000 : it.a_off[i], soff);
    else dma16(it.bdesc, dst, (OFFK_WG_ABLATE & 2) ? (int)0x80000000 : it.b_off[i - 2], soff);
#else
    if (i < 2) dma16(it.adesc, dst, it.a_off[i], soff);
    else dma16(it.bdesc, dst, it.b_off[i - 2], soff);
#endif
  };

  f32x16 acc;
  auto zero = [&]() {
#pragma unroll
    for (int i = 0; i < 16; ++i) acc[i] = 0.f;
    asm volatile("" : "+a"(acc));
  };
  auto mma = [&](const int st, const bool issue, const Item& ld, int ld_t) {
    const char* const base = wg_lds + st * WG_STAGE;
    float4 a[2], b[2];
    a[0] = *reinterpret_cast<const float4*>(base + aoff[0]);
    b[0] = *reinterpret_cast<const float4*>(base + boff[0]);
#pragma unroll
    for (int g = 0; g < 4; ++g) {
      if (g + 1 < 4) {
        a[(g + 1) & 1] = *reinterpret_cast<const float4*>(base + aoff[g + 1]);
        b[(g + 1) & 1] = *reinterpret_cast<const float4*>(base + boff[g + 1]);
      }
      __builtin_amdgcn_sched_barrier(0);
      if (issue && g < 2) {
        dma_piece(ld, g, ld_t, st ^ 1);
        dma_piece(ld, g + 2, ld_t, st ^ 1);
        __builtin_amdgcn_sched_barrier(0);
      }
      acc = __builtin_amdgcn_mfma_f32_32x32x2f32(a[g & 1].x, b[g & 1].x, acc, 0, 0, 0);
      acc = __builtin_amdgcn_mfma_f32_32x32x2f32(a[g & 1].y, b[g & 1].y, acc, 0, 0, 0);
      acc = __builtin_amdgcn_mfma_f32_32x32x2f32(a[g & 1].z, b[g & 1].z, acc, 0, 0, 0);
      acc = __builtin_amdgcn_mfma_f32_32x32x2f32(a[g & 1].w, b[g & 1].w, acc, 0, 0, 0);
      __builtin_amdgcn_sched_barrier(0);
    }
    asm volatile("" : "+a"(acc));
  };
  auto store_tile = [&](const Item& it) {
    const unsigned long long yu = reinterpret_cast<unsigned long long>(it.y);
    const __amdgpu_buffer_rsrc_t yrs = __builtin_amdgcn_make_buffer_rsrc(reinterpret_cast<float*>(yu), 0, argM * argCo * 4, 0x00020000);
    const int co4 = argCo * 4, mb = it.m0 + wm * 32;
    const int voff = (4 * hh * argCo + it.n0 + wn * 32 + r32) * 4;
#pragma unroll
    for (int reg = 0; reg < 16; ++reg)
      __builtin_amdgcn_raw_buffer_store_b32(__float_as_uint(acc[reg]), yrs, voff + (mb + (reg & 3) + 8 * (reg >> 2)) * co4, 0, 0);
  };

  int l = (int)blockIdx.x;
  Item cp, ld;
  locate(l, ld);
  cp = ld;
#pragma unroll
  for (int i = 0; i < 4; ++i) dma_piece(ld, i, 0, 0);
  int ld_t = 1, cp_t = 0;
  bool more = true;
  bool ld_next = false;
  zero();
  asm volatile("s_waitcnt vmcnt(0)" ::: "memory");
  __syncthreads();

  auto step = [&](const int ST) -> bool {
    if (more && ld_t == ld.nkt) {
      l += (int)gridDim.x;
      if (l < total_items) { locate(l, ld); ld_t = 0; ld_next = true; } else more = false;
    }
    mma(ST, more, ld, ld_t);
    if (more) ++ld_t;
    ++cp_t;
    const bool item_done = cp_t == cp.nkt;
    if (item_done) {
      store_tile(cp);
      asm volatile("s_waitcnt vmcnt(16)" ::: "memory");
    } else {
      asm volatile("s_waitcnt vmcnt(0)" ::: "memory");
    }
    __syncthreads();
    if (item_done) {
      if (!ld_next) return false;
      cp.y = ld.y; cp.m0 = ld.m0; cp.n0 = ld.n0; cp.nkt = ld.nkt; cp_t = 0; ld_next = false;
      zero();
    }
    return true;
  };
  for (;;) {
    if (!step(0)) break;
    if (!step(1)) break;
  }
}

bool wino_gemm_supported(const WinoGemmArgs& a) {
  if (a.M <= 0 || a.Co % WG_BN || a.ngroups < 1 || a.ngroups > 4) return false;
  long long problems = 0;
  for (int g = 0; g < a.ngroups; ++g) {
    if (a.g_K[g] % 32 || a.g_K[g] <= 0 || (long long)a.M * a.g_K[g] * 4 >= 0x7fffff00ll || (long long)a.Co * a.g_K[g] * 4 >= 0x7fffff00ll) return false;
    problems += a.g_batch[g];
  }
  if ((long long)a.M * a.Co * 4 >= 0x7f000000ll) return false;
  const long long total = problems * ((a.M + WG_BM - 1) / WG_BM) * (a.Co / WG_BN);
  return total > 0 && total < (1ll << 30);
}

hipError_t wino_gemm_launch(const WinoGemmArgs& a_in, hipStream_t st) {
  WinoGemmArgs a = a_in;
  if (!wino_gemm_supported(a)) return hipErrorInvalidValue;
  int problems = 0;
  for (int g = 0; g < a.ngroups; ++g) problems += a.g_batch[g];
  a.gm = (a.M + WG_BM - 1) / WG_BM;
  a.gn = a.Co / WG_BN;
  a.total_items = (int)((long long)problems * a.gm * a.gn);
  hipError_t e = lds_attr_once(reinterpret_cast<const void*>(wino_gemm_kernel), WG_LDS);
  if (e != hipSuccess) return e;
  const int grid = a.total_items < WG_RESIDENT ? a.total_items : WG_RESIDENT;
  hipLaunchKernelGGL(wino_gemm_kernel, dim3(grid), dim3(256), WG_LDS, st, a);
  return hipGetLastError();
}

}
```

optical-flow-guided-feature-pytorch_amd/csrc/wino_gemm_split.hip:

```cpp
#include <climits>
#include <cstdio>
#include <cstdlib>

#include "offk_common.h"
#include "offk_internal.h"

#ifndef OFFK_GS_EXP
#define OFFK_GS_EXP 0
#endif

namespace offk {

namespace {
typedef float f32x4 __attribute__((ext_vector_type(4)));
typedef unsigned u32x4 __attribute__((ext_vector_type(4)));
typedef unsigned u32x2 __attribute__((ext_vector_type(2)));
constexpr int GS_BM = 64;
constexpr int GS_GRP = 256;
constexpr int GS_PLANE = 4 * GS_GRP;
constexpr int GS_RT = 3 * GS_PLANE;
constexpr int GS_STAGE = 4 * GS_RT;
constexpr int GS_LDS = 2 * GS_STAGE;
#ifndef OFFK_GS_BLOCKS
#define OFFK_GS_BLOCKS 3
#endif
#ifndef OFFK_GS_BLOCKS_CT1
#define OFFK_GS_BLOCKS_CT1 3
#endif
constexpr int GS_RESIDENT = OFFK_GS_BLOCKS * 256;
constexpr int GS_RESIDENT_CT1 = OFFK_GS_BLOCKS_CT1 * 256;
constexpr int GS_OOB = (int)0x80000000;
}

template <int CT, bool EPI>
__global__ __launch_bounds__(256, OFFK_GS_BLOCKS) void wino_gemm_split_kernel(WinoGemmArgs p) {
  constexpr int NT = 4 * CT;
  constexpr int GS_BN = 64 * CT;
  extern __shared__ __attribute__((aligned(16))) char gs_planes[];
  const int tid = threadIdx.x, lane = tid & 63;
  const int wave = __builtin_amdgcn_readfirstlane(tid >> 6);
  const int li = lane & 15, lg = lane >> 4;

  const int lrow = tid >> 3, lc = tid & 7, lgp = lc >> 1;
  char* const pl_wr = gs_planes + (lrow >> 4) * GS_RT + lgp * GS_GRP + (((lrow & 15) ^ (2 * lgp)) << 4) + (lc & 1) * 8;
  const char* const xrd = gs_planes + lg * GS_GRP + ((li ^ (2 * lg)) << 4);

  const __amdgpu_buffer_rsrc_t xrs = __builtin_amdgcn_make_buffer_rsrc(const_cast<float*>(p.x), 0, (int)p.x_bytes, 0x00020000);
  const __amdgpu_buffer_rsrc_t wrs = __builtin_amdgcn_make_buffer_rsrc(const_cast<void*>(p.w_planes), 0, (int)p.w_bytes, 0x00020000);
  const __amdgpu_buffer_rsrc_t yrs = __builtin_amdgcn_make_buffer_rsrc(p.y, 0, (int)p.y_bytes, 0x00020000);

  const int gx = p.gm * p.gn;
  const int nK0 = p.g_K[0], nK1 = p.g_K[1], nK2 = p.g_K[2], nK3 = p.g_K[3];
  const int nB0 = p.g_batch[0], nB1 = p.g_batch[1], nB2 = p.g_batch[2];
  const long long oX0 = p.g_x[0], oX1 = p.g_x[1], oX2 = p.g_x[2], oX3 = p.g_x[3];
  const long long oW0 = p.g_w[0], oW1 = p.g_w[1], oW2 = p.g_w[2], oW3 = p.g_w[3];
  const long long oY0 = p.g_y[0], oY1 = p.g_y[1], oY2 = p.g_y[2], oY3 = p.g_y[3];
  const int ngroups = p.ngroups, argM = p.M, argCo = p.Co, total_items = p.total_items;
  const int gm = p.gm;
  const int main_items = (total_items / gx / 8) * 8 * gx;
  const int x_rs = p.x_rs, y_rs = EPI ? p.y_rs : p.Co;
  const int ukstep = (argCo >> 4) * 3072;
  const int grid = (int)gridDim.x;
  auto sc = [](int v) { return __builtin_amdgcn_readfirstlane(v); };

  int x_l = (int)blockIdx.x, x_t = 0, x_nkt = 0, x_soff = 0, x_off[2] = {GS_OOB, GS_OOB};
  int pu_soff = 0, pu_nkt = 0, pc_ysoff = 0, pc_m0 = 0, pc_n0 = 0;
  int pd_ysoff = 0, pd_m0 = 0, pd_n0 = 0, pd_nkt = 0;
  auto locate = [&](int l) {
    int prob, lid;
    if (l < main_items) { const int j = l >> 3, jq = sc(j / gx); prob = jq * 8 + (l & 7); lid = j - jq * gx; }
    else { const int lr = l - main_items; const int pq = sc(lr / gx); prob = (main_items / gx) + pq; lid = lr - pq * gx; }
    prob = sc(prob);
    const int nt = sc(lid / gm), mt = lid - nt * gm;
    int b = prob, K = nK0;
    long long ox = oX0, ow = oW0, oy = oY0;
    if (ngroups > 1 && prob >= nB0) { b = prob - nB0; K = nK1; ox = oX1; ow = oW1; oy = oY1; }
    if (ngroups > 2 && prob >= nB0 + nB1) { b = prob - nB0 - nB1; K = nK2; ox = oX2; ow = oW2; oy = oY2; }
    if (ngroups > 3 && prob >= nB0 + nB1 + nB2) { b = prob - nB0 - nB1 - nB2; K = nK3; ox = oX3; ow = oW3; oy = oY3; }
    const int m0 = mt * GS_BM, n0 = nt * GS_BN;
    x_soff = sc((int)((ox + (long long)b * argM * K) * 4));
    x_nkt = sc(K >> 5);
#pragma unroll
    for (int r2 = 0; r2 < 2; ++r2) {
      const int m = m0 + lrow + 32 * r2;
      x_off[r2] = m < argM ? (m * (EPI ? x_rs : K) + lc * 4) * 4 : GS_OOB;
    }
    pu_soff = sc((int)((ow + (long long)b * argCo * K) * 6) + ((n0 >> 4) + CT * wave) * 3072);
    pu_nkt = x_nkt;
    pc_ysoff = sc((int)((oy + (long long)b * argM * argCo) * 4));
    pc_m0 = m0; pc_n0 = n0;
  };
  int u_l = x_l, u_t = 0, u_nkt = 0, u_soff = 0, u_voff = lane * 16;
  int c_l = x_l, c_t = 0, c_nkt = 0, c_ysoff = 0, c_m0 = 0, c_n0 = 0;

  u32x4 xr[2][2];
  u32x4 wr[2][CT][3];
  auto load_x = [&](const int set, const int r) {
    xr[set][r] = __builtin_bit_cast(u32x4, __builtin_amdgcn_raw_buffer_load_b128(xrs, x_off[r], x_soff + x_t * 128, 0));
  };
  auto load_u = [&](const int set, const int n) {
#if defined(OFFK_GS_EXP) && (OFFK_GS_EXP & 16)
    wr[set][n / 3][n % 3] = __builtin_bit_cast(u32x4, __builtin_amdgcn_raw_buffer_load_b128(wrs, u_voff, u_soff + n * 1024, 0));
#else
    wr[set][n / 3][n % 3] = __builtin_bit_cast(u32x4, __builtin_amdgcn_raw_buffer_load_b128(wrs, u_voff, u_soff + u_t * ukstep + n * 1024, 0));
#endif
  };
  auto adv_x = [&]() {
    ++x_t;
    if (x_t == x_nkt) {
      x_l += grid; x_t = 0;
      if (x_l < total_items) locate(x_l);
      else { x_off[0] = GS_OOB; x_off[1] = GS_OOB; x_nkt = INT_MAX; }
    }
  };
  auto adv_u = [&]() {
    ++u_t;
    if (u_t == u_nkt) {
      u_l += grid; u_t = 0;
      if (u_l < total_items) { u_soff = pu_soff; u_nkt = pu_nkt; pd_ysoff = pc_ysoff; pd_m0 = pc_m0; pd_n0 = pc_n0; pd_nkt = pu_nkt; }
      else { u_voff = GS_OOB; u_nkt = INT_MAX; }
    }
  };

  typedef float f32x2 __attribute__((ext_vector_type(2)));
  unsigned ch[4], cm[4];
  f32x2 cr[2], cl[2];
  auto cut_slice = [&](const int s, const int set, const int r, const int st) {
    const u32x4& x = xr[set][r];
    if (s == 0) {
#pragma unroll
      for (int e = 0; e < 4; ++e) ch[e] = x[e] & 0xffff0000u;
    } else if (s == 1) {
#pragma unroll
      for (int e = 0; e < 2; ++e)
        cr[e] = f32x2{__uint_as_float(x[2 * e]), __uint_as_float(x[2 * e + 1])} - f32x2{__uint_as_float(ch[2 * e]), __uint_as_float(ch[2 * e + 1])};
    } else if (s == 2) {
#pragma unroll
      for (int e = 0; e < 4; ++e) cm[e] = __float_as_uint(cr[e >> 1][e & 1]) & 0xffff0000u;
    } else if (s == 3) {
#pragma unroll
      for (int e = 0; e < 2; ++e) cl[e] = cr[e] - f32x2{__uint_as_float(cm[2 * e]), __uint_as_float(cm[2 * e + 1])};
    } else {
      char* dst = pl_wr + st * GS_STAGE + r * 2 * GS_RT + (s - 4) * GS_PLANE;
      u32x2 d;
      if (s == 4) d = u32x2{__builtin_amdgcn_perm(x[1], x[0], 0x07060302), __builtin_amdgcn_perm(x[3], x[2], 0x07060302)};
      else if (s == 5) d = u32x2{__builtin_amdgcn_perm(cm[1], cm[0], 0x07060302), __builtin_amdgcn_perm(cm[3], cm[2], 0x07060302)};
      else d = u32x2{__builtin_amdgcn_perm(__float_as_uint(cl[0][1]), __float_as_uint(cl[0][0]), 0x07060302),
                     __builtin_amdgcn_perm(__float_as_uint(cl[1][1]), __float_as_uint(cl[1][0]), 0x07060302)};
      *reinterpret_cast<u32x2*>(dst) = d;
    }
  };
  constexpr int CUT_SLICES = 7;

  f32x4 acc[NT], acs[NT];
#pragma unroll
  for (int i = 0; i < NT; ++i) { acc[i] = f32x4{0.f, 0.f, 0.f, 0.f}; acs[i] = f32x4{0.f, 0.f, 0.f, 0.f}; }
  auto mf = [&](f32x4 c, const u32x4& a, const u32x4& b) {
    return __builtin_amdgcn_mfma_f32_16x16x32_bf16(__builtin_bit_cast(bf16x8, a), __builtin_bit_cast(bf16x8, b), c, 0, 0, 0);
  };
#define OFFK_SB __builtin_amdgcn_sched_barrier(0)

  const int st_voff = (li * y_rs + CT * wave * 16 + 4 * lg) * 4;
  auto store_item = [&]() {
    const int ybase = c_ysoff + (c_m0 * y_rs + c_n0) * 4;
#pragma unroll
    for (int i = 0; i < NT; ++i) acc[i] += acs[i];
    if (EPI) {
#pragma unroll
      for (int ct = 0; ct < CT; ++ct) {
        f32x4 b4 = {0.f, 0.f, 0.f, 0.f};
        if (p.bias) b4 = *reinterpret_cast<const f32x4*>(p.bias + c_n0 + (CT * wave + ct) * 16 + 4 * lg);
#pragma unroll
        for (int rt = 0; rt < 4; ++rt) {
          f32x4& a = acc[rt * CT + ct];
          a += b4;
          if (p.relu) a = f32x4{fmaxf(a.x, 0.f), fmaxf(a.y, 0.f), fmaxf(a.z, 0.f), fmaxf(a.w, 0.f)};
        }
      }
      if (p.pool_part) {
#pragma unroll
        for (int sl = 0; sl < 2; ++sl) {
          const int slab = (c_m0 >> 5) + sl;
          const int b1 = ((slab * 32) / p.pool_hw + 1) * p.pool_hw;
#pragma unroll
          for (int ct = 0; ct < CT; ++ct) {
            f32x4 s0 = {0.f, 0.f, 0.f, 0.f}, s1 = {0.f, 0.f, 0.f, 0.f};
#pragma unroll
            for (int h2 = 0; h2 < 2; ++h2) {
              const int m = slab * 32 + h2 * 16 + li;
              const f32x4 v = acc[(2 * sl + h2) * CT + ct];
              const bool in = m < argM, first = m < b1;
              const f32x4 z4 = {0.f, 0.f, 0.f, 0.f};
              s0 += in && first ? v : z4;
              s1 += in && !first ? v : z4;
            }
#pragma unroll
            for (int d = 1; d < 16; d <<= 1) {
#pragma unroll
              for (int e = 0; e < 4; ++e) { s0[e] += __shfl_xor(s0[e], d); s1[e] += __shfl_xor(s1[e], d); }
            }
            if (li == 0 && slab * 32 < argM) {
              float* pp = p.pool_part + (size_t)slab * 2 * argCo + c_n0 + (CT * wave + ct) * 16 + 4 * lg;
              *reinterpret_cast<f32x4*>(pp) = s0;
              *reinterpret_cast<f32x4*>(pp + argCo) = s1;
            }
          }
        }
      }
    }
#pragma unroll
    for (int i = 0; i < NT; ++i) {
      const int rt = i / CT;
      const int voff = li < argM - c_m0 - rt * 16 ? st_voff : GS_OOB;
      __builtin_amdgcn_raw_buffer_store_b128(__builtin_bit_cast(u32x4, acc[i]), yrs, voff, ybase + (rt * 16 * y_rs + (i % CT) * 16) * 4, 0);
      OFFK_SB;
      asm volatile("s_nop 1");
      OFFK_SB;
    }
#pragma unroll
    for (int i = 0; i < NT; ++i) { acc[i] = f32x4{0.f, 0.f, 0.f, 0.f}; acs[i] = f32x4{0.f, 0.f, 0.f, 0.f}; }
  };

  locate(x_l);
  u_soff = pu_soff; u_nkt = pu_nkt;
  c_ysoff = pc_ysoff; c_m0 = pc_m0; c_n0 = pc_n0; c_nkt = pu_nkt;
  load_x(0, 0); load_x(0, 1);
  adv_x();
  load_x(1, 0); load_x(1, 1);
  adv_x();
#pragma unroll
  for (int n = 0; n < 3 * CT; ++n) load_u(0, n);
  adv_u();
#pragma unroll
  for (int r = 0; r < 2; ++r)
#pragma unroll
    for (int s = 0; s < CUT_SLICES; ++s) cut_slice(s, 0, r, 0);
  __syncthreads();

  auto step = [&](const int ST) -> bool {
    u32x4 xb[4][3];
    const char* const rd = xrd + ST * GS_STAGE;
#pragma unroll
    for (int rt = 0; rt < 4; ++rt) xb[rt][0] = *reinterpret_cast<const u32x4*>(rd + rt * GS_RT);
#pragma unroll
    for (int rt = 0; rt < 4; ++rt) xb[rt][2] = *reinterpret_cast<const u32x4*>(rd + rt * GS_RT + 2 * GS_PLANE);
#pragma unroll
    for (int rt = 0; rt < 4; ++rt) xb[rt][1] = *reinterpret_cast<const u32x4*>(rd + rt * GS_RT + GS_PLANE);
    OFFK_SB;
    constexpr int WP[6] = {2, 0, 1, 1, 0, 0}, XP[6] = {0, 2, 1, 0, 1, 0};
    constexpr int NJ = 2 + 3 * CT + 2 * CUT_SLICES, NS = 5 * NT;
    auto job = [&](const int j) {
      if (j < 2) { if (!(OFFK_GS_EXP & 8)) load_x(ST, j); }
      else if (j < 2 + 2 * CUT_SLICES) { if (!(OFFK_GS_EXP & 1)) { const int c = j - 2; cut_slice(c % CUT_SLICES, ST ^ 1, c / CUT_SLICES, ST ^ 1); } }
      else if (!(OFFK_GS_EXP & 4)) { const int u = j - 2 - 2 * CUT_SLICES; load_u(ST ^ 1, (u % CT) * 3 + 2 - u / CT); }
    };
#pragma unroll
    for (int q = 0; q < 6; ++q) {
#pragma unroll
      for (int i = 0; i < NT; ++i) {
        const int n = q * NT + i, rt = i / CT, ct = i % CT;
        if (q < 5) acs[i] = mf(acs[i], wr[ST][ct][WP[q]], xb[rt][XP[q]]);
        else acc[i] = mf(acc[i], wr[ST][ct][WP[q]], xb[rt][XP[q]]);
        if (n < NS) {
#pragma unroll
          for (int j = (n * NJ + NS - 1) / NS; j < ((n + 1) * NJ + NS - 1) / NS; ++j) job(j);
        }
        OFFK_SB;
      }
    }
    ++c_t;
    bool go_on = true;
    if (c_t == c_nkt) {
      store_item();
      c_l += grid; c_t = 0;
      if (c_l < total_items) { c_ysoff = pd_ysoff; c_m0 = pd_m0; c_n0 = pd_n0; c_nkt = pd_nkt; }
      else go_on = false;
    }
    adv_u();
    adv_x();
    __syncthreads();
    return go_on;
  };
  for (;;) {
    if (!step(0)) break;
    if (!step(1)) break;
  }
}

__global__ void wino_pack_split_kernel(const float* __restrict__ U, uint4* __restrict__ img, int Co, int K, int nproblems) {
  const long long item = (long long)blockIdx.x * blockDim.x + threadIdx.x;
  const int nct = Co >> 4, nkt = K >> 5;
  const long long per = (long long)nkt * nct * 64;
  if (item >= per * nproblems) return;
  const int prob = (int)(item / per);
  const int rem = (int)(item - prob * per);
  const int lane = rem & 63, ct = (rem >> 6) % nct, kt = (rem >> 6) / nct;
  const int li = lane & 15, g = lane >> 4;
  const float* row = U + ((size_t)prob * Co + ct * 16 + li) * K + kt * 32 + 8 * g;
  unsigned h[8], m[8], l[8];
#pragma unroll
  for (int e = 0; e < 8; ++e) {
    const unsigned x = __float_as_uint(row[e]);
    h[e] = x & 0xffff0000u;
    const float r1 = __uint_as_float(x) - __uint_as_float(h[e]);
    m[e] = __float_as_uint(r1) & 0xffff0000u;
    l[e] = __float_as_uint(r1 - __uint_as_float(m[e]));
  }
  auto pk = [](const unsigned (&v)[8]) {
    return uint4{(v[0] >> 16) | (v[1] & 0xffff0000u), (v[2] >> 16) | (v[3] & 0xffff0000u), (v[4] >> 16) | (v[5] & 0xffff0000u),
                 (v[6] >> 16) | (v[7] & 0xffff0000u)};
  };
  uint4* o = img + (((size_t)prob * nkt + kt) * nct + ct) * 3 * 64 + lane;
  o[0] = pk(h); o[64] = pk(m); o[128] = pk(l);
}

hipError_t wino_pack_split_launch(const float* U, void* img, int Co, int K, int nproblems, hipStream_t st) {
  if (Co % 16 || K % 32 || nproblems <= 0) return hipErrorInvalidValue;
  const long long items = (long long)nproblems * (K / 32) * (Co / 16) * 64;
  hipLaunchKernelGGL(wino_pack_split_kernel, dim3((unsigned)((items + 255) / 256)), dim3(256), 0, st, U, reinterpret_cast<uint4*>(img), Co, K,
                     nproblems);
  return hipGetLastError();
}

bool wino_gemm_split_supported(const WinoGemmArgs& a) {
  if (!a.w_planes || a.M <= 0 || a.Co % 64 || a.ngroups < 1 || a.ngroups > 4) return false;
  long long problems = 0, xe = 0, we = 0, ye = 0;
  for (int g = 0; g < a.ngroups; ++g) {
    if (a.g_K[g] % 32 || a.g_K[g] < 64 || a.g_batch[g] <= 0) return false;
    problems += a.g_batch[g];
    xe = std::max(xe, a.g_x[g] + (long long)a.g_batch[g] * a.M * a.g_K[g]);
    we = std::max(we, a.g_w[g] + (long long)a.g_batch[g] * a.Co * a.g_K[g]);
    ye = std::max(ye, a.g_y[g] + (long long)a.g_batch[g] * a.M * a.Co);
    if ((long long)a.M * a.g_K[g] * 4 >= 0x7fffff00ll) return false;
  }
  if (xe * 4 >= 0x7fffff00ll || we * 6 >= 0x7fffff00ll || ye * 4 >= 0x7fffff00ll) return false;
  const long long total = problems * ((a.M + GS_BM - 1) / GS_BM) * (a.Co / 64);
  return total > 0 && total < (1ll << 30);
}

hipError_t wino_gemm_split_launch(const WinoGemmArgs& a_in, hipStream_t st) {
  WinoGemmArgs a = a_in;
  if (!wino_gemm_split_supported(a)) return hipErrorInvalidValue;
  long long problems = 0, xe = 0, we = 0, ye = 0;
  for (int g = 0; g < a.ngroups; ++g) {
    problems += a.g_batch[g];
    xe = std::max(xe, a.g_x[g] + (long long)a.g_batch[g] * a.M * a.g_K[g]);
    we = std::max(we, a.g_w[g] + (long long)a.g_batch[g] * a.Co * a.g_K[g]);
    ye = std::max(ye, a.g_y[g] + (long long)a.g_batch[g] * a.M * a.Co);
  }
  a.x_bytes = xe * 4; a.w_bytes = we * 6; a.y_bytes = ye * 4;
  a.gm = (a.M + GS_BM - 1) / GS_BM;
  const bool wide = a.Co % 128 == 0;
  a.gn = a.Co / (wide ? 128 : 64);
  a.total_items = (int)(problems * a.gm * a.gn);
  const bool epi = a.epilogue != 0;
  if (epi) {
    if (problems != 1 || a.x_rs < a.g_K[0] || a.y_rs < a.Co || ((a.x_rs | a.y_rs | a.x_coff | a.y_coff) & 3) || a.x_coff < 0 || a.y_coff < 0 ||
        (a.pool_part && a.pool_hw < 32))
      return hipErrorInvalidValue;
    a.x += a.x_coff; a.y += a.y_coff;
    a.x_bytes = ((long long)(a.M - 1) * a.x_rs + a.g_K[0]) * 4;
    a.y_bytes = ((long long)(a.M - 1) * a.y_rs + a.Co) * 4;
    if (a.x_bytes >= 0x7fffff00ll || a.y_bytes >= 0x7fffff00ll) return hipErrorInvalidValue;
  }
  const void* fn = wide ? (epi ? reinterpret_cast<const void*>(wino_gemm_split_kernel<2, true>) : reinterpret_cast<const void*>(wino_gemm_split_kernel<2, false>))
                        : (epi ? reinterpret_cast<const void*>(wino_gemm_split_kernel<1, true>) : reinterpret_cast<const void*>(wino_gemm_split_kernel<1, false>));
  hipError_t e = lds_attr_once(fn, GS_LDS);
  if (e != hipSuccess) return e;
  const int resident = wide ? GS_RESIDENT : GS_RESIDENT_CT1;
  const int grid = a.total_items < resident ? a.total_items : resident;
  if (wide && epi) hipLaunchKernelGGL((wino_gemm_split_kernel<2, true>), dim3(grid), dim3(256), GS_LDS, st, a);
  else if (wide) hipLaunchKernelGGL((wino_gemm_split_kernel<2, false>), dim3(grid), dim3(256), GS_LDS, st, a);
  else if (epi) hipLaunchKernelGGL((wino_gemm_split_kernel<1, true>), dim3(grid), dim3(256), GS_LDS, st, a);
  else hipLaunchKernelGGL((wino_gemm_split_kernel<1, false>), dim3(grid), dim3(256), GS_LDS, st, a);
  return hipGetLastError();
}

}
```

optical-flow-guided-feature-pytorch_amd/csrc/winograd.hip:

```cpp
#include "offk_common.h"
#include "offk_internal.h"
#include "winograd_common.h"

namespace offk {

namespace {
template <int NPH, int CY, int CX>
__device__ __forceinline__ void wino_input_tile(const float* __restrict__ xi, int x_cs, int R, int img, int Ci, int pa, int pb,
                                                unsigned c, float* __restrict__ V) {
  constexpr int NY = CY ? 5 : 6, NX = CX ? 5 : 6, W = NPH == 1 ? 7 : 14, STEP = NPH == 1 ? 1 : 2;
  constexpr int oy = CY ? 4 : 0, ox = CX ? 4 : 0;
  const unsigned c4 = c * 4u;
  float t[NY][NX];
#pragma unroll
  for (int j = 0; j < NX; ++j)
#pragma unroll
    for (int i = 0; i < NY; ++i) {
      const int row = oy - 1 + i, col = ox - 1 + j;
      t[i][j] = row >= 0 && row < 7 && col >= 0 && col < 7
                    ? *reinterpret_cast<const float*>(reinterpret_cast<const char*>(xi + (size_t)((STEP * row + pa) * W + STEP * col + pb) * x_cs) + c4)
                    : 0.f;
    }
#pragma unroll
  for (int j = 0; j < NX; ++j) {
// ... 81 lines not shown
      float v = yv[j] + bv;
      if (relu_pre) v = fmaxf(v, 0.f);
      if (a.res) v += a.res[pix * a.res_cs + a.res_coff + c];
      if (relu_post) v = fmaxf(v, 0.f);
      a.y[pix * a.y_cs + a.y_coff + c] = v;
      psum += v;
    }
  }
  if (a.pool_part) a.pool_part[((size_t)img * 4 + 2 * CY + CX) * a.pool_cs + a.pool_coff + c] = psum;
}
}
template <int NPH>
__global__ __launch_bounds__(256) void wino_output_kernel(WinoOutArgs a) {
  const int cw = (a.Co + 63) >> 6;
  const int wid = __builtin_amdgcn_readfirstlane((int)((blockIdx.x * 256u + threadIdx.x) >> 6));
  if (wid >= 4 * a.n_img * cw) return;
  const int cls = wid / (a.n_img * cw), r0 = wid - cls * (a.n_img * cw), img = r0 / cw;
  const unsigned c = (unsigned)(r0 - img * cw) * 64u + (threadIdx.x & 63u);
  if (c >= (unsigned)a.Co) return;
  switch (cls) {
    case 0: wino_output_tile<NPH, 0, 0>(a, img, c); break;
    case 1: wino_output_tile<NPH, 0, 1>(a, img, c); break;
    case 2: wino_output_tile<NPH, 1, 0>(a, img, c); break;
    default: wino_output_tile<NPH, 1, 1>(a, img, c); break;
  }
}

namespace {
template <int NPH, int CY, int CX>
__device__ __forceinline__ void wino_weight_tile(const float (&g)[3][3], int Co, int co, int Ci, int ci, int pa, int pb, int kk,
                                                 float* __restrict__ U) {
  constexpr int NY = CY ? 5 : 6, NX = CX ? 5 : 6;
  float t[NY][3];
#pragma unroll
  for (int v = 0; v < 3; ++v) {
    float gc[3], u[NY];
#pragma unroll
    for (int i = 0; i < 3; ++i) gc[i] = g[i][v];
    wg(gc, u);
#pragma unroll
    for (int i = 0; i < NY; ++i) t[i][v] = u[i];
  }
  const int K = NPH * Ci;
#pragma unroll
  for (int i = 0; i < NY; ++i) {
    float u[NX];
    wg(t[i], u);
#pragma unroll
    for (int j = 0; j < NX; ++j) {
      if constexpr (NPH == 1) {
        U[((size_t)wino_mindex<1, CY, CX>(i, j) * Co + co) * K + kk] = u[j];
      } else {
        WinoPlace pl;
        if (wino_place4<CY, CX>(i, j, pa, pb, pl))
          U[((size_t)pl.base_ci * Co + ((size_t)pl.idx * Co + co) * pl.kmul + pl.slot) * Ci + ci] = u[j];
      }
    }
  }
}
}
template <int NPH>
__global__ __launch_bounds__(256) void wino_weight_kernel(const float* __restrict__ w, int Co, int Ci, float* __restrict__ U) {
  constexpr int KS = NPH == 1 ? 3 : 5, STEP = NPH == 1 ? 1 : 2;
  const int K = NPH * Ci;
  const long long gid = (long long)blockIdx.x * 256 + threadIdx.x;
  if (gid >= (long long)Co * K) return;
  const int co = (int)(gid / K), kk = (int)(gid - (long long)co * K);
  const int ph = kk / Ci, ci = kk - ph * Ci, pa = ph >> 1, pb = ph & 1;
  const float* wp = w + ((size_t)(co * (Ci / 32) + ci / 32) * (KS * KS)) * 32 + (ci & 31);
  float g[3][3];
#pragma unroll
  for (int i = 0; i < 3; ++i)
#pragma unroll
    for (int j = 0; j < 3; ++j) {
      const int kh = STEP * i + pa, kw = STEP * j + pb;
      g[i][j] = kh < KS && kw < KS ? wp[(size_t)(kh * KS + kw) * 32] : 0.f;
    }
  wino_weight_tile<NPH, 0, 0>(g, Co, co, Ci, ci, pa, pb, kk, U);
  wino_weight_tile<NPH, 0, 1>(g, Co, co, Ci, ci, pa, pb, kk, U);
  wino_weight_tile<NPH, 1, 0>(g, Co, co, Ci, ci, pa, pb, kk, U);
  wino_weight_tile<NPH, 1, 1>(g, Co, co, Ci, ci, pa, pb, kk, U);
}

int wino_groups(int phases, long long rows, int Ci, int Co, WinoGroup out[4]) {
  if (phases == 1) { out[0] = WinoGroup{kWinoPoints, 1, 0, 0, 0}; return 1; }
  const int batch[4] = {81, 18, 18, 4}, kmul[4] = {4, 2, 2, 1}, base[4] = {0, 324, 360, 396}, first[4] = {0, 81, 99, 117};
  for (int g = 0; g < 4; ++g)
    out[g] = WinoGroup{batch[g], kmul[g], (long long)base[g] * rows * Ci, (long long)base[g] * Co * Ci, (long long)first[g] * rows * Co};
  return 4;
}

hipError_t wino_weight_launch(const float* w_packed, int Co, int Ci, int phases, float* U, hipStream_t st) {
  const long long n = (long long)Co * Ci * phases;
  if (phases == 4) hipLaunchKernelGGL(wino_weight_kernel<4>, dim3((unsigned)((n + 255) / 256)), dim3(256), 0, st, w_packed, Co, Ci, U);
  else hipLaunchKernelGGL(wino_weight_kernel<1>, dim3((unsigned)((n + 255) / 256)), dim3(256), 0, st, w_packed, Co, Ci, U);
  return hipGetLastError();
}

hipError_t wino_input_launch(const float* x, int x_cs, int x_coff, int n_img, int Ci, int phases, float* V, hipStream_t st) {
  const long long waves = (long long)4 * n_img * phases * ((Ci + 63) / 64);
  if (phases == 4) hipLaunchKernelGGL(wino_input_kernel<4>, dim3((unsigned)((waves + 3) / 4)), dim3(256), 0, st, x, x_cs, x_coff, n_img, Ci, V);
  else hipLaunchKernelGGL(wino_input_kernel<1>, dim3((unsigned)((waves + 3) / 4)), dim3(256), 0, st, x, x_cs, x_coff, n_img, Ci, V);
  return hipGetLastError();
}

hipError_t wino_output_launch(const float* M, int n_img, int Co, int phases, const float* bias, const float* res, int res_cs,
                              int res_coff, int flags, float* y, int y_cs, int y_coff, float* pool_part, hipStream_t st, int pool_cs, int pool_coff) {
  if (pool_part && pool_cs > 0 && (pool_coff < 0 || pool_coff + Co > pool_cs)) return hipErrorInvalidValue;
  WinoOutArgs a;
  a.M = M; a.bias = bias; a.res = res; a.res_cs = res_cs; a.res_coff = res_coff;
  a.y = y; a.y_cs = y_cs; a.y_coff = y_coff; a.pool_part = pool_part;
  a.pool_cs = pool_cs > 0 ? pool_cs : Co; a.pool_coff = pool_cs > 0 ? pool_coff : 0;
  a.n_img = n_img; a.Co = Co; a.flags = flags;
  const long long waves = (long long)4 * n_img * ((Co + 63) / 64);
  if (phases == 4) hipLaunchKernelGGL(wino_output_kernel<4>, dim3((unsigned)((waves + 3) / 4)), dim3(256), 0, st, a);
  else hipLaunchKernelGGL(wino_output_kernel<1>, dim3((unsigned)((waves + 3) / 4)), dim3(256), 0, st, a);
  return hipGetLastError();
}

}
```

optical-flow-guided-feature-pytorch_amd/csrc/winograd7.hip:

```cpp
#include "offk_common.h"
#include "offk_internal.h"

namespace offk {

namespace {
__device__ __forceinline__ void bt8(const float (&d)[8], float (&t)[8]) {
  t[0] = fmaf(-5.25f, d[4], fmaf(5.25f, d[2], -d[0])) + d[6];
  t[1] = fmaf(-4.25f, d[4], fmaf(-4.25f, d[3], d[1] + d[2])) + d[5] + d[6];
  t[2] = fmaf(-4.25f, d[4], fmaf(4.25f, d[3], -d[1] + d[2])) - d[5] + d[6];
  t[3] = fmaf(0.5f, d[5], fmaf(-5.0f, d[4], fmaf(-2.5f, d[3], fmaf(4.0f, d[2], 2.0f * d[1])))) + d[6];
  t[4] = fmaf(-0.5f, d[5], fmaf(-5.0f, d[4], fmaf(2.5f, d[3], fmaf(4.0f, d[2], -2.0f * d[1])))) + d[6];
  t[5] = fmaf(2.0f, d[5], fmaf(-1.25f, d[4], fmaf(-2.5f, d[3], fmaf(0.25f, d[2], 0.5f * d[1])))) + d[6];
  t[6] = fmaf(-2.0f, d[5], fmaf(-1.25f, d[4], fmaf(2.5f, d[3], fmaf(0.25f, d[2], -0.5f * d[1])))) + d[6];
  t[7] = fmaf(-5.25f, d[5], fmaf(5.25f, d[3], -d[1])) + d[7];
}
__device__ __forceinline__ void at5x8(const float (&m)[8], float (&s)[5]) {
  s[0] = m[0] + m[1] + m[2] + m[3] + m[4] + m[5] + m[6];
  s[1] = fmaf(-2.0f, m[6], fmaf(2.0f, m[5], fmaf(-0.5f, m[4], fmaf(0.5f, m[3], m[1] - m[2]))));
  s[2] = fmaf(4.0f, m[6], fmaf(4.0f, m[5], fmaf(0.25f, m[4], fmaf(0.25f, m[3], m[1] + m[2]))));
  s[3] = fmaf(-8.0f, m[6], fmaf(8.0f, m[5], fmaf(-0.125f, m[4], fmaf(0.125f, m[3], m[1] - m[2]))));
  s[4] = fmaf(16.0f, m[6], fmaf(16.0f, m[5], fmaf(0.0625f, m[4], fmaf(0.0625f, m[3], m[1] + m[2])))) + m[7];
}
__device__ __forceinline__ void g8(const float (&g)[4], float (&u)[8]) {
  u[0] = -g[0];
  u[1] = fmaf((float)-0.2222222222222222, g[3], fmaf((float)-0.2222222222222222, g[2], fmaf((float)-0.2222222222222222, g[1], (float)-0.2222222222222222 * g[0])));
  u[2] = fmaf((float)0.2222222222222222, g[3], fmaf((float)-0.2222222222222222, g[2], fmaf((float)0.2222222222222222, g[1], (float)-0.2222222222222222 * g[0])));
  u[3] = fmaf((float)0.08888888888888889, g[3], fmaf((float)0.17777777777777778, g[2], fmaf((float)0.35555555555555557, g[1], (float)0.7111111111111111 * g[0])));
  u[4] = fmaf((float)-0.08888888888888889, g[3], fmaf((float)0.17777777777777778, g[2], fmaf((float)-0.35555555555555557, g[1], (float)0.7111111111111111 * g[0])));
  u[5] = fmaf((float)0.08888888888888889, g[3], fmaf((float)0.044444444444444446, g[2], fmaf((float)0.022222222222222223, g[1], (float)0.011111111111111112 * g[0])));
  u[6] = fmaf((float)-0.08888888888888889, g[3], fmaf((float)0.044444444444444446, g[2], fmaf((float)-0.022222222222222223, g[1], (float)0.011111111111111112 * g[0])));
  u[7] = g[3];
}

struct Wino7Place { int base_ci, idx, kmul, slot; };
__device__ __forceinline__ bool wino7_place(int p, int q, int pa, int pb, Wino7Place& o) {
  if (p != 0 && q != 0) { o = Wino7Place{0, (p - 1) * 7 + (q - 1), 4, 2 * pa + pb}; return true; }
  if (p == 0 && q != 0) { o = Wino7Place{196, q - 1, 2, pb}; return pa == 1; }
  if (q == 0 && p != 0) { o = Wino7Place{210, p - 1, 2, pa}; return pb == 1; }
  o = Wino7Place{224, 0, 1, 0};
  return pa == 1 && pb == 1;
}
__device__ __forceinline__ int wino7_mindex(int p, int q) {
  return p != 0 && q != 0 ? (p - 1) * 7 + (q - 1) : (p == 0 && q != 0 ? 49 + q - 1 : (q == 0 && p != 0 ? 56 + p - 1 : 63));
}
}

__global__ __launch_bounds__(256) void wino7_input_kernel(const float* __restrict__ x, int x_cs, int x_coff, int n_img, int Ci,
                                                          float* __restrict__ V) {
  const int T = n_img * kWino7Tiles, cw = (Ci + 63) >> 6;
  const int wid = __builtin_amdgcn_readfirstlane((int)((blockIdx.x * 256u + threadIdx.x) >> 6));
  if (wid >= T * 4 * cw) return;
  const int tile = wid / (4 * cw), r = wid - tile * 4 * cw, ph = r / cw, pa = ph >> 1, pb = ph & 1;
  const unsigned c = (unsigned)(r - ph * cw) * 64u + (threadIdx.x & 63u);
  if (c >= (unsigned)Ci) return;
  const unsigned c4 = c * 4u;
  const int img = tile / kWino7Tiles, tt = tile - img * kWino7Tiles, oy = (tt / 3) * 5, ox = (tt % 3) * 5;
  const float* xi = x + (size_t)img * 784 * x_cs + x_coff;
  float t[8][8];
#pragma unroll
  for (int j = 0; j < 8; ++j) {
    const int col = ox - 2 + j, cc = min(max(col, 0), 13);
#pragma unroll
    for (int i = 0; i < 8; ++i) {
      const int row = oy - 2 + i, rr = min(max(row, 0), 13);
      t[i][j] = *reinterpret_cast<const float*>(reinterpret_cast<const char*>(xi + (size_t)((2 * rr + pa) * 28 + 2 * cc + pb) * x_cs) + c4);
    }
  }
#pragma unroll
  for (int j = 0; j < 8; ++j) {
    const int col = ox - 2 + j;
    float d[8];
#pragma unroll
    for (int i = 0; i < 8; ++i) {
      const int row = oy - 2 + i;
      d[i] = (unsigned)row < 14u && (unsigned)col < 14u ? t[i][j] : 0.f;
    }
    float tc[8];
    bt8(d, tc);
#pragma unroll
    for (int i = 0; i < 8; ++i) t[i][j] = tc[i];
  }
#pragma unroll
  for (int p = 0; p < 8; ++p) {
    float v[8];
    bt8(t[p], v);
#pragma unroll
    for (int q = 0; q < 8; ++q) {
      Wino7Place pl;
      if (wino7_place(p, q, pa, pb, pl))
        __builtin_nontemporal_store(v[q], reinterpret_cast<float*>(reinterpret_cast<char*>(V + ((size_t)pl.base_ci * T + ((size_t)pl.idx * T + tile) * pl.kmul + pl.slot) * Ci) + c4));
    }
  }
}

struct Wino7OutArgs {
  const float* M;
  const float* bias;
  float* y; int y_cs, y_coff;
  int n_img, Co, flags;
};
__global__ __launch_bounds__(256) void wino7_output_kernel(Wino7OutArgs a) {
  const int T = a.n_img * kWino7Tiles;
  const long long gid = (long long)blockIdx.x * 256 + threadIdx.x;
  if (gid >= (long long)T * a.Co) return;
  const int tile = (int)(gid / a.Co), c = (int)(gid - (long long)tile * a.Co);
  const int img = tile / kWino7Tiles, tt = tile - img * kWino7Tiles, oy = (tt / 3) * 5, ox = (tt % 3) * 5;
  const float* mp = a.M + (size_t)tile * a.Co + c;
  const size_t pstride = (size_t)T * a.Co;
  float s[5][8];
#pragma unroll
  for (int q = 0; q < 8; ++q) {
    float m[8];
#pragma unroll
    for (int p = 0; p < 8; ++p) m[p] = mp[(size_t)wino7_mindex(p, q) * pstride];
    float sc[5];
    at5x8(m, sc);
#pragma unroll
    for (int i = 0; i < 5; ++i) s[i][q] = sc[i];
  }
  const float bv = a.bias ? a.bias[c] : 0.f;
  const bool relu = (a.flags & OFFK_CONV_RELU_PRE_) || (a.flags & OFFK_CONV_RELU_POST_);
#pragma unroll
  for (int i = 0; i < 5; ++i) {
    float yv[5];
    at5x8(s[i], yv);
    const int row = oy + i;
#pragma unroll
    for (int j = 0; j < 5; ++j) {
      const int col = ox + j;
      if (row < 14 && col < 14) {
        float v = yv[j] + bv;
        if (relu) v = fmaxf(v, 0.f);
        a.y[((size_t)img * 196 + row * 14 + col) * a.y_cs + a.y_coff + c] = v;
      }
    }
  }
}

__global__ __launch_bounds__(256) void wino7_weight_kernel(const float* __restrict__ w, int Co, int Ci, float* __restrict__ U) {
  const int K = 4 * Ci;
  const long long gid = (long long)blockIdx.x * 256 + threadIdx.x;
  if (gid >= (long long)Co * K) return;
  const int co = (int)(gid / K), kk = (int)(gid - (long long)co * K);
  const int ph = kk / Ci, ci = kk - ph * Ci, pa = ph >> 1, pb = ph & 1;
  const float* wp = w + ((size_t)(co * (Ci / 32) + ci / 32) * 49) * 32 + (ci & 31);
  float t[8][4];
#pragma unroll
  for (int v = 0; v < 4; ++v) {
    float g[4];
#pragma unroll
    for (int u = 0; u < 4; ++u) {
      const int kh = 2 * u - 1 + pa, kw = 2 * v - 1 + pb;
      g[u] = kh >= 0 && kw >= 0 ? wp[(size_t)(kh * 7 + kw) * 32] : 0.f;
    }
    float uu[8];
    g8(g, uu);
#pragma unroll
    for (int p = 0; p < 8; ++p) t[p][v] = uu[p];
  }
#pragma unroll
  for (int p = 0; p < 8; ++p) {
    float uu[8];
    g8(t[p], uu);
#pragma unroll
    for (int q = 0; q < 8; ++q) {
      Wino7Place pl;
      if (wino7_place(p, q, pa, pb, pl))
        U[((size_t)pl.base_ci * Co + ((size_t)pl.idx * Co + co) * pl.kmul + pl.slot) * Ci + ci] = uu[q];
    }
  }
}

int wino7_groups(long long T, int Ci, int Co, WinoGroup out[4]) {
  const int batch[4] = {49, 7, 7, 1}, kmul[4] = {4, 2, 2, 1}, base[4] = {0, 196, 210, 224}, first[4] = {0, 49, 56, 63};
  for (int g = 0; g < 4; ++g)
    out[g] = WinoGroup{batch[g], kmul[g], (long long)base[g] * T * Ci, (long long)base[g] * Co * Ci, (long long)first[g] * T * Co};
  return 4;
}

hipError_t wino7_weight_launch(const float* w_packed, int Co, int Ci, float* U, hipStream_t st) {
  const long long n = (long long)Co * Ci * 4;
  hipLaunchKernelGGL(wino7_weight_kernel, dim3((unsigned)((n + 255) / 256)), dim3(256), 0, st, w_packed, Co, Ci, U);
  return hipGetLastError();
}

hipError_t wino7_input_launch(const float* x, int x_cs, int x_coff, int n_img, int Ci, float* V, hipStream_t st) {
  const long long waves = (long long)n_img * kWino7Tiles * 4 * ((Ci + 63) / 64);
  hipLaunchKernelGGL(wino7_input_kernel, dim3((unsigned)((waves + 3) / 4)), dim3(256), 0, st, x, x_cs, x_coff, n_img, Ci, V);
  return hipGetLastError();
}

hipError_t wino7_output_launch(const float* M, int n_img, int Co, const float* bias, int flags, float* y, int y_cs, int y_coff,
                               hipStream_t st) {
  Wino7OutArgs a;
  a.M = M; a.bias = bias; a.y = y; a.y_cs = y_cs; a.y_coff = y_coff;
  a.n_img = n_img; a.Co = Co; a.flags = flags;
  const long long n = (long long)n_img * kWino7Tiles * Co;
  hipLaunchKernelGGL(wino7_output_kernel, dim3((unsigned)((n + 255) / 256)), dim3(256), 0, st, a);
  return hipGetLastError();
}

}
```

Measured before the change: 24600 clips/s.

## Skip padded Winograd F(5,4) tile points for border tiles via per-group rows and weight selection

Reorganises the 7x7 Winograd path so border tiles of the 14x14 output, which only need 7 of 8 transform points in one or both dimensions, use smaller 8x7/7x8/7x7 transforms. The V/M buffers are regrouped into up to 8 GEMM groups, each with its own row count, and a per-problem weight-selection table maps each GEMM back to the shared U weights. The aim is to drop the GEMM rows and transform work that only produced padded outputs. In exchange it adds grouping metadata read from kernarg memory, an early exit for M tiles past a group's row count, and considerably more index bookkeeping across the input, output and GEMM kernels.

After: 24700 clips/s (median of 6 runs). Within noise of the previous version (+0.4%).

```diff
diff --git a/optical-flow-guided-feature-pytorch_amd/csrc/conv_igemm.hip b/optical-flow-guided-feature-pytorch_amd/csrc/conv_igemm.hip
--- a/optical-flow-guided-feature-pytorch_amd/csrc/conv_igemm.hip
+++ b/optical-flow-guided-feature-pytorch_amd/csrc/conv_igemm.hip
@@ -20,8 +20,10 @@
   int batch;
   int spread;
   long long x_bs, w_bs, y_bs;
-  int ngroups, g_batch[4], g_Ci[4];
-  long long g_x[4], g_w[4], g_y[4];
+  int ngroups, g_batch[9], g_Ci[9], g_M[9];
+  long long g_x[9], g_w[9], g_y[9];
+  int w_sel_on;
+  unsigned w_sel[32];
   float* pool_part;
   int pool_hw;
   float* partial;
@@ -45,14 +47,18 @@
   unsigned long long tm_t1 = 0, tm_t2 = 0, tm_ta = 0;
 #endif
   if (p.ngroups > 0) {
-    int b = blockIdx.y, ci = p.g_Ci[0], first = 0;
-    long long gx = p.g_x[0], gw = p.g_w[0], gy = p.g_y[0];
-#pragma unroll
-    for (int g = 1; g < 4; ++g) {
-      first += p.g_batch[g - 1];
-      if (g < p.ngroups && (int)blockIdx.y >= first) { b = blockIdx.y - first; ci = p.g_Ci[g]; gx = p.g_x[g]; gw = p.g_w[g]; gy = p.g_y[g]; }
-    }
-    p.x += gx + (long long)b * p.M * ci; p.w += gw + (long long)b * p.Co * ci; p.y += gy + (long long)b * p.M * p.Co;
+    const auto* const kp = kernarg_as<ConvArgs>();
+    int g = 0, first = 0, gfirst = 0;
+    for (int i = 1; i < p.ngroups; ++i) {
+      first += kp->g_batch[i - 1];
+      if ((int)blockIdx.y >= first) { g = i; gfirst = first; }
+    }
+    g = __builtin_amdgcn_readfirstlane(g);
+    const int b = blockIdx.y - gfirst, ci = kp->g_Ci[g], gM = kp->g_M[g];
+    const long long gx = kp->g_x[g], gw = kp->g_w[g], gy = kp->g_y[g];
+    const int wb = p.w_sel_on ? (int)((kp->w_sel[blockIdx.y >> 2] >> ((blockIdx.y & 3) * 8)) & 255u) : b;
+    p.M = gM;
+    p.x += gx + (long long)b * p.M * ci; p.w += gw + (long long)wb * p.Co * ci; p.y += gy + (long long)b * p.M * p.Co;
     p.Ci = ci; p.x_cs = ci; p.x_bytes = (unsigned)p.M * (unsigned)ci * 4u; p.w_bytes = (unsigned)p.Co * (unsigned)ci * 4u;
   } else if (gridDim.y > 1) { p.x += blockIdx.y * p.x_bs; p.w += blockIdx.y * p.w_bs; p.y += blockIdx.y * p.y_bs; }
   constexpr bool DMA = PREC == 4;
@@ -72,6 +78,7 @@
   }
   const int nt = lid % p.gn, mt = (lid / p.gn) % p.gm, zs = lid / (p.gn * p.gm);
   const int m0 = mt * BM, n0 = nt * BN;
+  if (m0 >= p.M) return;
   constexpr int TAPS = KH * KW;
   const int K = TAPS * p.Ci;
   const int nkt_all = TAPS * (p.Ci / BK);
@@ -877,14 +884,20 @@
   a.pool_part = d.pool_part; a.pool_hw = d.pool_hw;
   a.batch = d.batch > 1 ? d.batch : 1; a.x_bs = d.x_bstride; a.w_bs = d.w_bstride; a.y_bs = d.y_bstride;
   a.ngroups = d.ngroups;
-  for (int g = 0; g < 4; ++g) { a.g_batch[g] = d.g_batch[g]; a.g_Ci[g] = d.g_Ci[g]; a.g_x[g] = d.g_x[g]; a.g_w[g] = d.g_w[g]; a.g_y[g] = d.g_y[g]; }
+  for (int g = 0; g < 9; ++g) {
+    a.g_batch[g] = d.g_batch[g]; a.g_Ci[g] = d.g_Ci[g]; a.g_x[g] = d.g_x[g]; a.g_w[g] = d.g_w[g]; a.g_y[g] = d.g_y[g];
+    a.g_M[g] = d.g_M[g] > 0 ? d.g_M[g] : (int)M;
+  }
+  a.w_sel_on = d.ngroups > 0 ? d.w_sel_on : 0;
+  for (int i = 0; i < 32; ++i) a.w_sel[i] = d.w_sel[i];
   if (d.ngroups > 0) {
-    if (d.ngroups > 4 || d.x_coff || d.y_coff || d.y_cs != d.Co) { *why = "conv2d: grouped batches are dense [M][Ci] x [Co][Ci] -> [M][Co] problems"; return hipErrorInvalidValue; }
+    if (d.ngroups > 9 || d.x_coff || d.y_coff || d.y_cs != d.Co) { *why = "conv2d: grouped batches are dense [M][Ci] x [Co][Ci] -> [M][Co] problems"; return hipErrorInvalidValue; }
     int nb = 0;
     for (int g = 0; g < d.ngroups; ++g) {
-      if (d.g_Ci[g] < 32 || d.g_Ci[g] % 32 || d.g_batch[g] < 1) { *why = "conv2d: bad batch group"; return hipErrorInvalidValue; }
+      if (d.g_Ci[g] < 32 || d.g_Ci[g] % 32 || d.g_batch[g] < 1 || a.g_M[g] > M) { *why = "conv2d: bad batch group"; return hipErrorInvalidValue; }
       nb += d.g_batch[g];
     }
+    if (d.w_sel_on && nb > 128) { *why = "conv2d: a weight selection covers at most 128 problems"; return hipErrorInvalidValue; }
     a.batch = nb;
   }
   if (a.batch > 1) {
diff --git a/optical-flow-guided-feature-pytorch_amd/csrc/offk_api.hip b/optical-flow-guided-feature-pytorch_amd/csrc/offk_api.hip
--- a/optical-flow-guided-feature-pytorch_amd/csrc/offk_api.hip
+++ b/optical-flow-guided-feature-pytorch_amd/csrc/offk_api.hip
@@ -35,18 +35,31 @@
 
 static hipError_t wino_gemms_launch(const WinoGroup* grp, int ngrp, int npoints, int rows, int Ci, int Co, const float* V, const float* U,
                                     float* M, bool persistent, hipStream_t s, const char** why, const void* U_planes = nullptr) {
+  unsigned w_sel[kMaxWinoSel / 4] = {};
+  int w_sel_on = 0, nprob = 0;
+  for (int gi = 0; gi < ngrp; ++gi) {
+    for (int i = 0; i < grp[gi].batch; ++i, ++nprob) {
+      const unsigned sel = grp[gi].nsel ? grp[gi].u_sel[i] : (unsigned)i;
+      if (nprob < kMaxWinoSel) w_sel[nprob >> 2] |= (sel & 255u) << ((nprob & 3) * 8);
+    }
+    w_sel_on |= grp[gi].nsel != 0;
+  }
+  if (w_sel_on && nprob > kMaxWinoSel) { *why = "winograd GEMMs: a weight selection covers at most 128 problems"; return hipErrorInvalidValue; }
   if (persistent || U_planes) {
     WinoGemmArgs a{};
     a.x = V; a.w = U; a.y = M; a.M = rows; a.Co = Co; a.ngroups = ngrp;
     for (int gi = 0; gi < ngrp; ++gi) {
-      a.g_batch[gi] = grp[gi].batch; a.g_K[gi] = grp[gi].kmul * Ci;
+      a.g_batch[gi] = grp[gi].batch; a.g_K[gi] = grp[gi].kmul * Ci; a.g_M[gi] = (int)grp[gi].rows;
       a.g_x[gi] = grp[gi].v_off; a.g_w[gi] = grp[gi].u_off; a.g_y[gi] = grp[gi].m_off;
     }
+    a.w_sel_on = w_sel_on;
+    for (int i = 0; i < kMaxWinoSel / 4; ++i) a.w_sel[i] = w_sel[i];
     a.w_planes = U_planes;
     if (U_planes && wino_gemm_split_supported(a)) return wino_gemm_split_launch(a, s);
     if (persistent && wino_gemm_supported(a)) return wino_gemm_launch(a, s);
   }
-  const int K0 = grp[0].kmul * Ci;
+  int K0 = 0;
+  for (int gi = 0; gi < ngrp; ++gi) K0 = std::max(K0, grp[gi].kmul * Ci);
   ConvDesc d = conv_desc(V, K0, 0, rows, 1, 1, K0, U, nullptr, Co, 1, 1, 1, 0, nullptr, 0, 0, 0, M, Co, 0, 3, 1);
 #ifdef OFFK_TUNING_KNOBS
   { const char* e = getenv("OFFK_WINO_CFG"); if (e && (Co % 128 == 0 || atoi(e) == 1 || atoi(e) == 2)) d.tile_cfg = atoi(e); }
@@ -55,9 +68,11 @@
   if (ngrp > 1) {
     d.ngroups = ngrp;
     for (int gi = 0; gi < ngrp; ++gi) {
-      d.g_batch[gi] = grp[gi].batch; d.g_Ci[gi] = grp[gi].kmul * Ci;
+      d.g_batch[gi] = grp[gi].batch; d.g_Ci[gi] = grp[gi].kmul * Ci; d.g_M[gi] = (int)grp[gi].rows;
       d.g_x[gi] = grp[gi].v_off; d.g_w[gi] = grp[gi].u_off; d.g_y[gi] = grp[gi].m_off;
     }
+    d.w_sel_on = w_sel_on;
+    for (int i = 0; i < kMaxWinoSel / 4; ++i) d.w_sel[i] = w_sel[i];
   }
   return conv2d_launch(d, s, why);
 }
@@ -311,7 +326,7 @@
   add_region(h, "poolpart_7", ((P * 49 + 31) / 32) * 2 * 1024);
   add_region(h, "poolpart_14", ((P * 49 + 31) / 32) * 2 * 512);
   if (h->cfg.precision == OFFK_PRECISION_FP32) {
-    add_region(h, "wino_v", std::max((size_t)kWinoUnits4 * P * 1056, (size_t)kWino7Tiles * P * kWino7Units * 320));
+    add_region(h, "wino_v", std::max((size_t)kWinoUnits4 * P * 1056, (size_t)kWino7Tiles * P * kWino7UUnits * 320));
     add_region(h, "wino_m", (size_t)kWinoPoints * P * 512);
     add_region(h, "poolpart_14t", (size_t)4 * P * 512);
     if (h->pool_first7) add_region(h, "poolpart_7t", (size_t)4 * P * 512);
@@ -697,11 +712,14 @@
   DK_HEAD_COMPOSED
 };
 DerivedKind u_kind(const ConvSpec& c) { return c.K == 7 ? DK_U_F54 : c.K == 5 ? DK_U_POLY : DK_U_F43; }
-int u_units(DerivedKind k) { return k == DK_U_F54 ? kWino7Units : k == DK_U_POLY ? kWinoUnits4 : kWinoPoints; }
+int u_units(DerivedKind k) { return k == DK_U_F54 ? kWino7UUnits : k == DK_U_POLY ? kWinoUnits4 : kWinoPoints; }
 size_t u_elems(const ConvSpec& c) { return (size_t)u_units(u_kind(c)) * c.Co * c.Ci; }
 int wino_phases(const ConvSpec& c) { return u_kind(c) == DK_U_POLY ? 4 : 1; }
-int wino_conv_groups(const ConvSpec& c, long long rows, WinoGroup grp[4]) {
-  return u_kind(c) == DK_U_F54 ? wino7_groups(rows, c.Ci, c.Co, grp) : wino_groups(wino_phases(c), rows, c.Ci, c.Co, grp);
+int wino_conv_groups(const ConvSpec& c, long long n, WinoGroup grp[kMaxWinoGroups]) {
+  return u_kind(c) == DK_U_F54 ? wino7_groups(n, c.Ci, c.Co, grp) : wino_groups(wino_phases(c), n, c.Ci, c.Co, grp);
+}
+int wino_u_groups(const ConvSpec& c, WinoGroup grp[kMaxWinoGroups]) {
+  return u_kind(c) == DK_U_F54 ? wino7_u_groups(c.Ci, c.Co, grp) : wino_groups(wino_phases(c), 1, c.Ci, c.Co, grp);
 }
 size_t plane_floats(size_t elems) { return (elems * 3 + 1) / 2; }
 
@@ -769,8 +787,8 @@
     }
     case DK_U_PLANES: {
       const ConvSpec& c = kConvs[r.slot];
-      WinoGroup grp[4];
-      const int ngrp = wino_conv_groups(c, 1, grp);
+      WinoGroup grp[kMaxWinoGroups];
+      const int ngrp = wino_u_groups(c, grp);
       for (int g = 0; g < ngrp; ++g)
         HIP_TRY(h, wino_pack_split_launch(d.u + grp[g].u_off, reinterpret_cast<char*>(d.u_planes) + grp[g].u_off * 6, c.Co, grp[g].kmul * c.Ci, grp[g].batch, st));
       break;
@@ -925,8 +943,8 @@
     const bool f54 = u_kind(c) == DK_U_F54;
     TRY(trace_mark(h, s, c.key, f54 ? " [winograd: 64 GEMMs]" : " [winograd: 121 GEMMs]"));
     const int rows = f54 ? kWino7Tiles * n : n;
-    WinoGroup grp[4];
-    const int ngrp = wino_conv_groups(c, rows, grp);
+    WinoGroup grp[kMaxWinoGroups];
+    const int ngrp = wino_conv_groups(c, n, grp);
     const char* why = nullptr;
     hipError_t e = wino_gemms_launch(grp, ngrp, f54 ? kWino7Points : kWinoPoints, rows, c.Ci, c.Co, wino_V, h->derived[id].u, wino_M, h->wino_gemm, s, &why,
                                      h->derived[id].u_planes);
@@ -2002,7 +2020,7 @@
     return fail(nullptr, OFFK_ERR_INVALID, std::string(who) + ": bad argument (Ci % 32 == 0, Co % 64 == 0, no RELU_IN)");
   const bool f54 = phases == 7;
   const size_t T = f54 ? (size_t)kWino7Tiles * n_img : (size_t)n_img;
-  const size_t units = f54 ? kWino7Units : phases == 4 ? kWinoUnits4 : kWinoPoints, points = f54 ? kWino7Points : kWinoPoints;
+  const size_t units = f54 ? kWino7UUnits : phases == 4 ? kWinoUnits4 : kWinoPoints, points = f54 ? kWino7Points : kWinoPoints;
   const size_t need = units * Ci * ((size_t)Co + T) + points * T * Co;
   if (scratch_floats < need) return fail(nullptr, OFFK_ERR_INVALID, std::string(who) + ": scratch too small");
   hipStream_t st = static_cast<hipStream_t>(stream);
@@ -2012,8 +2030,8 @@
   hipError_t e = f54 ? wino7_weight_launch(w_packed, Co, Ci, U, st) : wino_weight_launch(w_packed, Co, Ci, phases, U, st);
   if (e == hipSuccess) e = f54 ? wino7_input_launch(x, x_cstride, x_coff, n_img, Ci, V, st) : wino_input_launch(x, x_cstride, x_coff, n_img, Ci, phases, V, st);
   if (e != hipSuccess) return fail_hip(nullptr, e, who);
-  WinoGroup grp[4];
-  const int ngrp = f54 ? wino7_groups((long long)T, Ci, Co, grp) : wino_groups(phases, (long long)T, Ci, Co, grp);
+  WinoGroup grp[kMaxWinoGroups];
+  const int ngrp = f54 ? wino7_groups(n_img, Ci, Co, grp) : wino_groups(phases, (long long)T, Ci, Co, grp);
   {
     const char* why = nullptr;
     e = wino_gemms_launch(grp, ngrp, (int)points, (int)T, Ci, Co, V, U, M, wino_gemm_stage_default(), st, &why);
@@ -2086,7 +2104,7 @@
   if (precision != OFFK_PRECISION_FP32 && precision != OFFK_PRECISION_F32SPLIT)
     return fail(nullptr, OFFK_ERR_INVALID, std::string(who) + ": precision must be OFFK_PRECISION_FP32 or OFFK_PRECISION_F32SPLIT");
   hipStream_t st = static_cast<hipStream_t>(stream);
-  WinoGroup grp{batch, 1, 0, 0, 0};
+  WinoGroup grp{batch, 1, M, 0, 0, 0, 0, {}};
   const void* planes = nullptr;
   if (precision == OFFK_PRECISION_F32SPLIT) {
     if (K < 64) return fail(nullptr, OFFK_ERR_INVALID, std::string(who) + ": the split-fp32 form takes K >= 64");
diff --git a/optical-flow-guided-feature-pytorch_amd/csrc/offk_common.h b/optical-flow-guided-feature-pytorch_amd/csrc/offk_common.h
--- a/optical-flow-guided-feature-pytorch_amd/csrc/offk_common.h
+++ b/optical-flow-guided-feature-pytorch_amd/csrc/offk_common.h
@@ -79,4 +79,13 @@
                      ((unsigned)(u >> 32) & 0xFFFFu) >= thresh ? scale : 0.f, (unsigned)(u >> 48) >= thresh ? scale : 0.f);
 }
 
+template <class T>
+__device__ __forceinline__ const T __attribute__((address_space(4)))* kernarg_as() {
+#if defined(__HIP_DEVICE_COMPILE__)
+  return (const T __attribute__((address_space(4)))*)__builtin_amdgcn_kernarg_segment_ptr();
+#else
+  return nullptr;
+#endif
 }
+
+}
diff --git a/optical-flow-guided-feature-pytorch_amd/csrc/offk_internal.h b/optical-flow-guided-feature-pytorch_amd/csrc/offk_internal.h
--- a/optical-flow-guided-feature-pytorch_amd/csrc/offk_internal.h
+++ b/optical-flow-guided-feature-pytorch_amd/csrc/offk_internal.h
@@ -28,8 +28,10 @@
   int batch = 1;
   long long x_bstride = 0, w_bstride = 0, y_bstride = 0;
   int ngroups = 0;
-  int g_batch[4] = {0, 0, 0, 0}, g_Ci[4] = {0, 0, 0, 0};
-  long long g_x[4] = {0, 0, 0, 0}, g_w[4] = {0, 0, 0, 0}, g_y[4] = {0, 0, 0, 0};
+  int g_batch[9] = {}, g_Ci[9] = {}, g_M[9] = {};
+  long long g_x[9] = {}, g_w[9] = {}, g_y[9] = {};
+  int w_sel_on = 0;
+  unsigned w_sel[32] = {};
   float* pool_part = nullptr;
   int pool_hw = 0;
 };
@@ -67,20 +69,26 @@
 hipError_t wino_output_launch(const float* M, int n_img, int Co, int phases, const float* bias, const float* res, int res_cs,
                               int res_coff, int flags, float* y, int y_cs, int y_coff, float* pool_part, hipStream_t st, int pool_cs = 0,
                               int pool_coff = 0);
-struct WinoGroup { int batch, kmul; long long v_off, u_off, m_off; };
-int wino_groups(int phases, long long rows, int Ci, int Co, WinoGroup out[4]);
+constexpr int kMaxWinoGroups = 9, kMaxWinoSel = 128;
+struct WinoGroup { int batch, kmul; long long rows, v_off, u_off, m_off; int nsel; unsigned char u_sel[40]; };
+int wino_groups(int phases, long long rows, int Ci, int Co, WinoGroup out[kMaxWinoGroups]);
 struct WinoGemmArgs {
   const float* x; const float* w; float* y;
   int M, Co;
-  int ngroups, g_batch[4], g_K[4];
-  long long g_x[4], g_w[4], g_y[4];
+  int ngroups, g_batch[kMaxWinoGroups], g_K[kMaxWinoGroups], g_M[kMaxWinoGroups];
+  long long g_x[kMaxWinoGroups], g_w[kMaxWinoGroups], g_y[kMaxWinoGroups];
+  int w_sel_on;
+  unsigned w_sel[kMaxWinoSel / 4];
   int gm, gn, total_items;
+  int g_first[kMaxWinoGroups];
+  int nclass, c_grp[kMaxWinoGroups + 1], c_prob[kMaxWinoGroups + 1], c_item[kMaxWinoGroups + 1], c_gm[kMaxWinoGroups], c_main[kMaxWinoGroups];
   const void* w_planes = nullptr;
   long long x_bytes = 0, w_bytes = 0, y_bytes = 0;
   int epilogue = 0, x_rs = 0, x_coff = 0, y_rs = 0, y_coff = 0, relu = 0, pool_hw = 0;
   const float* bias = nullptr;
   float* pool_part = nullptr;
 };
+bool wino_gemm_plan(WinoGemmArgs& a, int bm, int bn);
 bool wino_gemm_supported(const WinoGemmArgs& a);
 hipError_t wino_gemm_launch(const WinoGemmArgs& a, hipStream_t st);
 bool wino_gemm_split_supported(const WinoGemmArgs& a);
@@ -102,11 +110,12 @@
 };
 bool wino_mid_supported(int Cin, int Cmid, bool gemm, int phases_in);
 hipError_t wino_mid_launch(const WinoMidArgs& a, hipStream_t st);
-constexpr int kWino7Units = 225, kWino7Points = 64, kWino7Tiles = 9;
+constexpr int kWino7UUnits = 225, kWino7Units = 1849, kWino7Pairs = 529, kWino7Points = 64, kWino7Tiles = 9;
 hipError_t wino7_weight_launch(const float* w_packed, int Co, int Ci, float* U, hipStream_t st);
 hipError_t wino7_input_launch(const float* x, int x_cs, int x_coff, int n_img, int Ci, float* V, hipStream_t st);
 hipError_t wino7_output_launch(const float* M, int n_img, int Co, const float* bias, int flags, float* y, int y_cs, int y_coff, hipStream_t st);
-int wino7_groups(long long T, int Ci, int Co, WinoGroup out[4]);
+int wino7_groups(long long n_img, int Ci, int Co, WinoGroup out[kMaxWinoGroups]);
+int wino7_u_groups(int Ci, int Co, WinoGroup out[4]);
 
 struct PwSite {
   const float* xp[4];
diff --git a/optical-flow-guided-feature-pytorch_amd/csrc/wino_gemm.hip b/optical-flow-guided-feature-pytorch_amd/csrc/wino_gemm.hip
--- a/optical-flow-guided-feature-pytorch_amd/csrc/wino_gemm.hip
+++ b/optical-flow-guided-feature-pytorch_amd/csrc/wino_gemm.hip
@@ -37,43 +37,47 @@
     boff[g] = WG_BM * 128 + (wn * 32 + r32) * 128 + ((sw ^ (2 * g)) << 4);
   }
 
-  const int gx = p.gm * p.gn;
-  const int nK0 = p.g_K[0], nK1 = p.g_K[1], nK2 = p.g_K[2], nK3 = p.g_K[3];
-  const int nB0 = p.g_batch[0], nB1 = p.g_batch[1], nB2 = p.g_batch[2];
-  const long long oX0 = p.g_x[0], oX1 = p.g_x[1], oX2 = p.g_x[2], oX3 = p.g_x[3];
-  const long long oW0 = p.g_w[0], oW1 = p.g_w[1], oW2 = p.g_w[2], oW3 = p.g_w[3];
-  const long long oY0 = p.g_y[0], oY1 = p.g_y[1], oY2 = p.g_y[2], oY3 = p.g_y[3];
-  const int ngroups = p.ngroups, argM = p.M, argCo = p.Co, gn = p.gn, total_items = p.total_items;
+  const auto* const kp = kernarg_as<WinoGemmArgs>();
+  const int ngroups = p.ngroups, nclass = p.nclass, argCo = p.Co, gn = p.gn, total_items = p.total_items, w_sel_on = p.w_sel_on;
   const float* const argx = p.x; const float* const argw = p.w; float* const argy = p.y;
   struct Item {
     i32x4 adesc, bdesc;
     int a_off[2], b_off[2];
     int nkt;
     float* y;
-    int m0, n0;
+    int m0, n0, M;
   };
   auto locate = [&](int l, Item& it) {
-    const int prob = __builtin_amdgcn_readfirstlane(l / gx), bx = l - prob * gx;
+    auto sc = [](int v) { return __builtin_amdgcn_readfirstlane(v); };
+    int c = 0;
+#pragma unroll
+    for (int i = 1; i < kMaxWinoGroups; ++i)
+      if (i < nclass && l >= kp->c_item[i]) c = i;
+    c = sc(c);
+    const int gx = kp->c_gm[c] * gn, lc = l - kp->c_item[c];
+    const int pq = sc(lc / gx), bx = lc - pq * gx, prob = kp->c_prob[c] + pq;
     const int xcd = bx & 7, q = gx >> 3, r = gx & 7;
     const int lid = (xcd < r ? xcd * (q + 1) : r * (q + 1) + (xcd - r) * q) + (bx >> 3);
-    const int mt = __builtin_amdgcn_readfirstlane(lid / gn), nt = lid - mt * gn;
-    int b = prob, K = nK0;
-    long long ox = oX0, ow = oW0, oy = oY0;
-    if (ngroups > 1 && prob >= nB0) { b = prob - nB0; K = nK1; ox = oX1; ow = oW1; oy = oY1; }
-    if (ngroups > 2 && prob >= nB0 + nB1) { b = prob - nB0 - nB1; K = nK2; ox = oX2; ow = oW2; oy = oY2; }
-    if (ngroups > 3 && prob >= nB0 + nB1 + nB2) { b = prob - nB0 - nB1 - nB2; K = nK3; ox = oX3; ow = oW3; oy = oY3; }
-    const float* xa = argx + ox + (long long)b * argM * K;
-    const float* wa = argw + ow + (long long)b * argCo * K;
-    it.y = argy + oy + (long long)b * argM * argCo;
+    const int mt = sc(lid / gn), nt = lid - mt * gn;
+    int g = 0;
+#pragma unroll
+    for (int i = 1; i < kMaxWinoGroups; ++i)
+      if (i < ngroups && prob >= kp->g_first[i]) g = i;
+    g = sc(g);
+    const int b = prob - kp->g_first[g], K = kp->g_K[g], M = kp->g_M[g];
+    const int wb = w_sel_on ? (int)((kp->w_sel[prob >> 2] >> ((prob & 3) * 8)) & 255u) : b;
+    const float* xa = argx + kp->g_x[g] + (long long)b * M * K;
+    const float* wa = argw + kp->g_w[g] + (long long)wb * argCo * K;
+    it.y = argy + kp->g_y[g] + (long long)b * M * argCo;
+    it.M = M;
     const unsigned long long xu = reinterpret_cast<unsigned long long>(xa), wu = reinterpret_cast<unsigned long long>(wa);
-    auto sc = [](int v) { return __builtin_amdgcn_readfirstlane(v); };
-    it.adesc = i32x4{sc((int)(unsigned)xu), sc((int)(unsigned)(xu >> 32) & 0xffff), sc(argM * K * 4), 0x00020000};
+    it.adesc = i32x4{sc((int)(unsigned)xu), sc((int)(unsigned)(xu >> 32) & 0xffff), sc(M * K * 4), 0x00020000};
     it.bdesc = i32x4{sc((int)(unsigned)wu), sc((int)(unsigned)(wu >> 32) & 0xffff), sc(argCo * K * 4), 0x00020000};
     it.m0 = mt * WG_BM; it.n0 = nt * WG_BN; it.nkt = sc(K >> 5);
 #pragma unroll
     for (int r = 0; r < 2; ++r) {
       const int m = it.m0 + lrow + 32 * r;
-      it.a_off[r] = m < argM ? (m * K + kpos) * 4 : (int)0x80000000;
+      it.a_off[r] = m < M ? (m * K + kpos) * 4 : (int)0x80000000;
       it.b_off[r] = ((it.n0 + lrow + 32 * r) * K + kpos) * 4;
     }
   };
@@ -122,7 +126,7 @@
   };
   auto store_tile = [&](const Item& it) {
     const unsigned long long yu = reinterpret_cast<unsigned long long>(it.y);
-    const __amdgpu_buffer_rsrc_t yrs = __builtin_amdgcn_make_buffer_rsrc(reinterpret_cast<float*>(yu), 0, argM * argCo * 4, 0x00020000);
+    const __amdgpu_buffer_rsrc_t yrs = __builtin_amdgcn_make_buffer_rsrc(reinterpret_cast<float*>(yu), 0, it.M * argCo * 4, 0x00020000);
     const int co4 = argCo * 4, mb = it.m0 + wm * 32;
     const int voff = (4 * hh * argCo + it.n0 + wn * 32 + r32) * 4;
 #pragma unroll
@@ -161,7 +165,7 @@
     __syncthreads();
     if (item_done) {
       if (!ld_next) return false;
-      cp.y = ld.y; cp.m0 = ld.m0; cp.n0 = ld.n0; cp.nkt = ld.nkt; cp_t = 0; ld_next = false;
+      cp.y = ld.y; cp.m0 = ld.m0; cp.n0 = ld.n0; cp.M = ld.M; cp.nkt = ld.nkt; cp_t = 0; ld_next = false;
       zero();
     }
     return true;
@@ -172,26 +176,50 @@
   }
 }
 
-bool wino_gemm_supported(const WinoGemmArgs& a) {
-  if (a.M <= 0 || a.Co % WG_BN || a.ngroups < 1 || a.ngroups > 4) return false;
-  long long problems = 0;
+bool wino_gemm_plan(WinoGemmArgs& a, int bm, int bn) {
+  if (a.ngroups < 1 || a.ngroups > kMaxWinoGroups || a.Co <= 0 || a.Co % bn) return false;
+  a.gn = a.Co / bn;
+  a.nclass = 0;
+  long long prob = 0, item = 0;
   for (int g = 0; g < a.ngroups; ++g) {
-    if (a.g_K[g] % 32 || a.g_K[g] <= 0 || (long long)a.M * a.g_K[g] * 4 >= 0x7fffff00ll || (long long)a.Co * a.g_K[g] * 4 >= 0x7fffff00ll) return false;
-    problems += a.g_batch[g];
-  }
-  if ((long long)a.M * a.Co * 4 >= 0x7f000000ll) return false;
-  const long long total = problems * ((a.M + WG_BM - 1) / WG_BM) * (a.Co / WG_BN);
-  return total > 0 && total < (1ll << 30);
+    if (a.g_M[g] <= 0) a.g_M[g] = a.M;
+    if (a.g_M[g] <= 0 || a.g_batch[g] <= 0) return false;
+    if (g == 0 || a.g_M[g] != a.g_M[g - 1]) {
+      for (int c = 0; c < a.nclass; ++c)
+        if (a.g_M[a.c_grp[c]] == a.g_M[g]) return false;
+      a.c_grp[a.nclass] = g; a.c_prob[a.nclass] = (int)prob; a.c_item[a.nclass] = (int)item; a.c_gm[a.nclass] = (a.g_M[g] + bm - 1) / bm;
+      ++a.nclass;
+    }
+    a.g_first[g] = (int)prob;
+    prob += a.g_batch[g];
+    item += (long long)a.g_batch[g] * a.c_gm[a.nclass - 1] * a.gn;
+    if (item >= (1ll << 30)) return false;
+  }
+  a.c_grp[a.nclass] = a.ngroups; a.c_prob[a.nclass] = (int)prob; a.c_item[a.nclass] = (int)item;
+  for (int c = 0; c < a.nclass; ++c) a.c_main[c] = (a.c_prob[c + 1] - a.c_prob[c]) / 8 * 8 * a.c_gm[c] * a.gn;
+  for (int c = a.nclass; c < kMaxWinoGroups; ++c) { a.c_gm[c] = 0; a.c_main[c] = 0; if (c > a.nclass) { a.c_grp[c] = a.ngroups; a.c_prob[c] = (int)prob; a.c_item[c] = (int)item; } }
+  for (int g = a.ngroups; g < kMaxWinoGroups; ++g) a.g_first[g] = (int)prob;
+  if (a.w_sel_on && prob > kMaxWinoSel) return false;
+  a.M = 0;
+  for (int g = 0; g < a.ngroups; ++g) a.M = a.g_M[g] > a.M ? a.g_M[g] : a.M;
+  a.gm = a.c_gm[0];
+  a.total_items = (int)item;
+  return item > 0;
+}
+
+bool wino_gemm_supported(const WinoGemmArgs& a_in) {
+  WinoGemmArgs a = a_in;
+  if (!wino_gemm_plan(a, WG_BM, WG_BN)) return false;
+  for (int g = 0; g < a.ngroups; ++g) {
+    if (a.g_K[g] % 32 || a.g_K[g] <= 0 || (long long)a.g_M[g] * a.g_K[g] * 4 >= 0x7fffff00ll || (long long)a.Co * a.g_K[g] * 4 >= 0x7fffff00ll) return false;
+    if ((long long)a.g_M[g] * a.Co * 4 >= 0x7f000000ll) return false;
+  }
+  return true;
 }
 
 hipError_t wino_gemm_launch(const WinoGemmArgs& a_in, hipStream_t st) {
   WinoGemmArgs a = a_in;
-  if (!wino_gemm_supported(a)) return hipErrorInvalidValue;
-  int problems = 0;
-  for (int g = 0; g < a.ngroups; ++g) problems += a.g_batch[g];
-  a.gm = (a.M + WG_BM - 1) / WG_BM;
-  a.gn = a.Co / WG_BN;
-  a.total_items = (int)((long long)problems * a.gm * a.gn);
+  if (!wino_gemm_supported(a) || !wino_gemm_plan(a, WG_BM, WG_BN)) return hipErrorInvalidValue;
   hipError_t e = lds_attr_once(reinterpret_cast<const void*>(wino_gemm_kernel), WG_LDS);
   if (e != hipSuccess) return e;
   const int grid = a.total_items < WG_RESIDENT ? a.total_items : WG_RESIDENT;
diff --git a/optical-flow-guided-feature-pytorch_amd/csrc/wino_gemm_split.hip b/optical-flow-guided-feature-pytorch_amd/csrc/wino_gemm_split.hip
--- a/optical-flow-guided-feature-pytorch_amd/csrc/wino_gemm_split.hip
+++ b/optical-flow-guided-feature-pytorch_amd/csrc/wino_gemm_split.hip
@@ -49,49 +49,51 @@
   const __amdgpu_buffer_rsrc_t wrs = __builtin_amdgcn_make_buffer_rsrc(const_cast<void*>(p.w_planes), 0, (int)p.w_bytes, 0x00020000);
   const __amdgpu_buffer_rsrc_t yrs = __builtin_amdgcn_make_buffer_rsrc(p.y, 0, (int)p.y_bytes, 0x00020000);
 
-  const int gx = p.gm * p.gn;
-  const int nK0 = p.g_K[0], nK1 = p.g_K[1], nK2 = p.g_K[2], nK3 = p.g_K[3];
-  const int nB0 = p.g_batch[0], nB1 = p.g_batch[1], nB2 = p.g_batch[2];
-  const long long oX0 = p.g_x[0], oX1 = p.g_x[1], oX2 = p.g_x[2], oX3 = p.g_x[3];
-  const long long oW0 = p.g_w[0], oW1 = p.g_w[1], oW2 = p.g_w[2], oW3 = p.g_w[3];
-  const long long oY0 = p.g_y[0], oY1 = p.g_y[1], oY2 = p.g_y[2], oY3 = p.g_y[3];
-  const int ngroups = p.ngroups, argM = p.M, argCo = p.Co, total_items = p.total_items;
-  const int gm = p.gm;
-  const int main_items = (total_items / gx / 8) * 8 * gx;
+  const auto* const kp = kernarg_as<WinoGemmArgs>();
+  const int ngroups = p.ngroups, nclass = p.nclass, argM = p.M, argCo = p.Co, total_items = p.total_items, w_sel_on = p.w_sel_on;
+  const int gn = p.gn;
   const int x_rs = p.x_rs, y_rs = EPI ? p.y_rs : p.Co;
   const int ukstep = (argCo >> 4) * 3072;
   const int grid = (int)gridDim.x;
   auto sc = [](int v) { return __builtin_amdgcn_readfirstlane(v); };
 
   int x_l = (int)blockIdx.x, x_t = 0, x_nkt = 0, x_soff = 0, x_off[2] = {GS_OOB, GS_OOB};
-  int pu_soff = 0, pu_nkt = 0, pc_ysoff = 0, pc_m0 = 0, pc_n0 = 0;
-  int pd_ysoff = 0, pd_m0 = 0, pd_n0 = 0, pd_nkt = 0;
+  int pu_soff = 0, pu_nkt = 0, pc_ysoff = 0, pc_m0 = 0, pc_n0 = 0, pc_M = 0;
+  int pd_ysoff = 0, pd_m0 = 0, pd_n0 = 0, pd_nkt = 0, pd_M = 0;
   auto locate = [&](int l) {
+    int c = 0;
+#pragma unroll
+    for (int i = 1; i < kMaxWinoGroups; ++i)
+      if (i < nclass && l >= kp->c_item[i]) c = i;
+    c = sc(c);
+    const int gm = kp->c_gm[c], gx = gm * gn, main_items = kp->c_main[c], ll = l - kp->c_item[c];
     int prob, lid;
-    if (l < main_items) { const int j = l >> 3, jq = sc(j / gx); prob = jq * 8 + (l & 7); lid = j - jq * gx; }
-    else { const int lr = l - main_items; const int pq = sc(lr / gx); prob = (main_items / gx) + pq; lid = lr - pq * gx; }
-    prob = sc(prob);
+    if (ll < main_items) { const int j = ll >> 3, jq = sc(j / gx); prob = jq * 8 + (ll & 7); lid = j - jq * gx; }
+    else { const int lr = ll - main_items; const int pq = sc(lr / gx); prob = (main_items / gx) + pq; lid = lr - pq * gx; }
+    prob = sc(prob) + kp->c_prob[c];
     const int nt = sc(lid / gm), mt = lid - nt * gm;
-    int b = prob, K = nK0;
-    long long ox = oX0, ow = oW0, oy = oY0;
-    if (ngroups > 1 && prob >= nB0) { b = prob - nB0; K = nK1; ox = oX1; ow = oW1; oy = oY1; }
-    if (ngroups > 2 && prob >= nB0 + nB1) { b = prob - nB0 - nB1; K = nK2; ox = oX2; ow = oW2; oy = oY2; }
-    if (ngroups > 3 && prob >= nB0 + nB1 + nB2) { b = prob - nB0 - nB1 - nB2; K = nK3; ox = oX3; ow = oW3; oy = oY3; }
+    int g = 0;
+#pragma unroll
+    for (int i = 1; i < kMaxWinoGroups; ++i)
+      if (i < ngroups && prob >= kp->g_first[i]) g = i;
+    g = sc(g);
+    const int b = prob - kp->g_first[g], K = kp->g_K[g], M = kp->g_M[g];
+    const int wb = w_sel_on ? (int)((kp->w_sel[prob >> 2] >> ((prob & 3) * 8)) & 255u) : b;
     const int m0 = mt * GS_BM, n0 = nt * GS_BN;
-    x_soff = sc((int)((ox + (long long)b * argM * K) * 4));
+    x_soff = sc((int)((kp->g_x[g] + (long long)b * M * K) * 4));
     x_nkt = sc(K >> 5);
 #pragma unroll
     for (int r2 = 0; r2 < 2; ++r2) {
       const int m = m0 + lrow + 32 * r2;
-      x_off[r2] = m < argM ? (m * (EPI ? x_rs : K) + lc * 4) * 4 : GS_OOB;
-    }
-    pu_soff = sc((int)((ow + (long long)b * argCo * K) * 6) + ((n0 >> 4) + CT * wave) * 3072);
+      x_off[r2] = m < M ? (m * (EPI ? x_rs : K) + lc * 4) * 4 : GS_OOB;
+    }
+    pu_soff = sc((int)((kp->g_w[g] + (long long)wb * argCo * K) * 6) + ((n0 >> 4) + CT * wave) * 3072);
     pu_nkt = x_nkt;
-    pc_ysoff = sc((int)((oy + (long long)b * argM * argCo) * 4));
-    pc_m0 = m0; pc_n0 = n0;
+    pc_ysoff = sc((int)((kp->g_y[g] + (long long)b * M * argCo) * 4));
+    pc_m0 = m0; pc_n0 = n0; pc_M = M;
   };
   int u_l = x_l, u_t = 0, u_nkt = 0, u_soff = 0, u_voff = lane * 16;
-  int c_l = x_l, c_t = 0, c_nkt = 0, c_ysoff = 0, c_m0 = 0, c_n0 = 0;
+  int c_l = x_l, c_t = 0, c_nkt = 0, c_ysoff = 0, c_m0 = 0, c_n0 = 0, c_M = 0;
 
   u32x4 xr[2][2];
   u32x4 wr[2][CT][3];
@@ -117,7 +119,7 @@
     ++u_t;
     if (u_t == u_nkt) {
       u_l += grid; u_t = 0;
-      if (u_l < total_items) { u_soff = pu_soff; u_nkt = pu_nkt; pd_ysoff = pc_ysoff; pd_m0 = pc_m0; pd_n0 = pc_n0; pd_nkt = pu_nkt; }
+      if (u_l < total_items) { u_soff = pu_soff; u_nkt = pu_nkt; pd_ysoff = pc_ysoff; pd_m0 = pc_m0; pd_n0 = pc_n0; pd_nkt = pu_nkt; pd_M = pc_M; }
       else { u_voff = GS_OOB; u_nkt = INT_MAX; }
     }
   };
@@ -211,7 +213,7 @@
 #pragma unroll
     for (int i = 0; i < NT; ++i) {
       const int rt = i / CT;
-      const int voff = li < argM - c_m0 - rt * 16 ? st_voff : GS_OOB;
+      const int voff = li < c_M - c_m0 - rt * 16 ? st_voff : GS_OOB;
       __builtin_amdgcn_raw_buffer_store_b128(__builtin_bit_cast(u32x4, acc[i]), yrs, voff, ybase + (rt * 16 * y_rs + (i % CT) * 16) * 4, 0);
       OFFK_SB;
       asm volatile("s_nop 1");
@@ -223,7 +225,7 @@
 
   locate(x_l);
   u_soff = pu_soff; u_nkt = pu_nkt;
-  c_ysoff = pc_ysoff; c_m0 = pc_m0; c_n0 = pc_n0; c_nkt = pu_nkt;
+  c_ysoff = pc_ysoff; c_m0 = pc_m0; c_n0 = pc_n0; c_nkt = pu_nkt; c_M = pc_M;
   load_x(0, 0); load_x(0, 1);
   adv_x();
   load_x(1, 0); load_x(1, 1);
@@ -273,7 +275,7 @@
     if (c_t == c_nkt) {
       store_item();
       c_l += grid; c_t = 0;
-      if (c_l < total_items) { c_ysoff = pd_ysoff; c_m0 = pd_m0; c_n0 = pd_n0; c_nkt = pd_nkt; }
+      if (c_l < total_items) { c_ysoff = pd_ysoff; c_m0 = pd_m0; c_n0 = pd_n0; c_nkt = pd_nkt; c_M = pd_M; }
       else go_on = false;
     }
     adv_u();
@@ -322,37 +324,37 @@
   return hipGetLastError();
 }
 
-bool wino_gemm_split_supported(const WinoGemmArgs& a) {
-  if (!a.w_planes || a.M <= 0 || a.Co % 64 || a.ngroups < 1 || a.ngroups > 4) return false;
-  long long problems = 0, xe = 0, we = 0, ye = 0;
+static bool gs_extents(const WinoGemmArgs& a, long long* xe_o, long long* we_o, long long* ye_o) {
+  long long xe = 0, we = 0, ye = 0;
   for (int g = 0; g < a.ngroups; ++g) {
-    if (a.g_K[g] % 32 || a.g_K[g] < 64 || a.g_batch[g] <= 0) return false;
-    problems += a.g_batch[g];
-    xe = std::max(xe, a.g_x[g] + (long long)a.g_batch[g] * a.M * a.g_K[g]);
-    we = std::max(we, a.g_w[g] + (long long)a.g_batch[g] * a.Co * a.g_K[g]);
-    ye = std::max(ye, a.g_y[g] + (long long)a.g_batch[g] * a.M * a.Co);
-    if ((long long)a.M * a.g_K[g] * 4 >= 0x7fffff00ll) return false;
+    if (a.g_K[g] % 32 || a.g_K[g] < 64) return false;
+    long long wprob = a.g_batch[g];
+    if (a.w_sel_on)
+      for (int i = 0; i < a.g_batch[g]; ++i) wprob = std::max(wprob, (long long)((a.w_sel[(a.g_first[g] + i) >> 2] >> (((a.g_first[g] + i) & 3) * 8)) & 255u) + 1);
+    xe = std::max(xe, a.g_x[g] + (long long)a.g_batch[g] * a.g_M[g] * a.g_K[g]);
+    we = std::max(we, a.g_w[g] + wprob * a.Co * a.g_K[g]);
+    ye = std::max(ye, a.g_y[g] + (long long)a.g_batch[g] * a.g_M[g] * a.Co);
+    if ((long long)a.g_M[g] * a.g_K[g] * 4 >= 0x7fffff00ll) return false;
   }
   if (xe * 4 >= 0x7fffff00ll || we * 6 >= 0x7fffff00ll || ye * 4 >= 0x7fffff00ll) return false;
-  const long long total = problems * ((a.M + GS_BM - 1) / GS_BM) * (a.Co / 64);
-  return total > 0 && total < (1ll << 30);
+  *xe_o = xe; *we_o = we; *ye_o = ye;
+  return true;
+}
+
+bool wino_gemm_split_supported(const WinoGemmArgs& a_in) {
+  WinoGemmArgs a = a_in;
+  if (!a.w_planes || a.Co % 64 || !wino_gemm_plan(a, GS_BM, a.Co % 128 == 0 ? 128 : 64)) return false;
+  long long xe, we, ye;
+  return gs_extents(a, &xe, &we, &ye);
 }
 
 hipError_t wino_gemm_split_launch(const WinoGemmArgs& a_in, hipStream_t st) {
   WinoGemmArgs a = a_in;
-  if (!wino_gemm_split_supported(a)) return hipErrorInvalidValue;
-  long long problems = 0, xe = 0, we = 0, ye = 0;
-  for (int g = 0; g < a.ngroups; ++g) {
-    problems += a.g_batch[g];
-    xe = std::max(xe, a.g_x[g] + (long long)a.g_batch[g] * a.M * a.g_K[g]);
-    we = std::max(we, a.g_w[g] + (long long)a.g_batch[g] * a.Co * a.g_K[g]);
-    ye = std::max(ye, a.g_y[g] + (long long)a.g_batch[g] * a.M * a.Co);
-  }
+  const bool wide = a.Co % 128 == 0;
+  long long xe, we, ye;
+  if (!a.w_planes || a.Co % 64 || !wino_gemm_plan(a, GS_BM, wide ? 128 : 64) || !gs_extents(a, &xe, &we, &ye)) return hipErrorInvalidValue;
+  const long long problems = a.c_prob[a.nclass];
   a.x_bytes = xe * 4; a.w_bytes = we * 6; a.y_bytes = ye * 4;
-  a.gm = (a.M + GS_BM - 1) / GS_BM;
-  const bool wide = a.Co % 128 == 0;
-  a.gn = a.Co / (wide ? 128 : 64);
-  a.total_items = (int)(problems * a.gm * a.gn);
   const bool epi = a.epilogue != 0;
   if (epi) {
     if (problems != 1 || a.x_rs < a.g_K[0] || a.y_rs < a.Co || ((a.x_rs | a.y_rs | a.x_coff | a.y_coff) & 3) || a.x_coff < 0 || a.y_coff < 0 ||
diff --git a/optical-flow-guided-feature-pytorch_amd/csrc/winograd.hip b/optical-flow-guided-feature-pytorch_amd/csrc/winograd.hip
--- a/optical-flow-guided-feature-pytorch_amd/csrc/winograd.hip
+++ b/optical-flow-guided-feature-pytorch_amd/csrc/winograd.hip
@@ -187,11 +187,11 @@
   wino_weight_tile<NPH, 1, 1>(g, Co, co, Ci, ci, pa, pb, kk, U);
 }
 
-int wino_groups(int phases, long long rows, int Ci, int Co, WinoGroup out[4]) {
-  if (phases == 1) { out[0] = WinoGroup{kWinoPoints, 1, 0, 0, 0}; return 1; }
+int wino_groups(int phases, long long rows, int Ci, int Co, WinoGroup out[kMaxWinoGroups]) {
+  if (phases == 1) { out[0] = WinoGroup{kWinoPoints, 1, rows, 0, 0, 0, 0, {}}; return 1; }
   const int batch[4] = {81, 18, 18, 4}, kmul[4] = {4, 2, 2, 1}, base[4] = {0, 324, 360, 396}, first[4] = {0, 81, 99, 117};
   for (int g = 0; g < 4; ++g)
-    out[g] = WinoGroup{batch[g], kmul[g], (long long)base[g] * rows * Ci, (long long)base[g] * Co * Ci, (long long)first[g] * rows * Co};
+    out[g] = WinoGroup{batch[g], kmul[g], rows, (long long)base[g] * rows * Ci, (long long)base[g] * Co * Ci, (long long)first[g] * rows * Co, 0, {}};
   return 4;
 }
 
diff --git a/optical-flow-guided-feature-pytorch_amd/csrc/winograd7.hip b/optical-flow-guided-feature-pytorch_amd/csrc/winograd7.hip
--- a/optical-flow-guided-feature-pytorch_amd/csrc/winograd7.hip
+++ b/optical-flow-guided-feature-pytorch_amd/csrc/winograd7.hip
@@ -32,17 +32,104 @@
   u[7] = g[3];
 }
 
+__device__ __forceinline__ void bt7(const float (&d)[7], float (&t)[7]) {
+  t[0] = fmaf(-2.0f, d[5], fmaf(-4.0f, d[4], fmaf(2.5f, d[3], fmaf(5.0f, d[2], fmaf(-0.5f, d[1], -d[0])))));
+  t[1] = fmaf(-3.0f, d[4], fmaf(-1.75f, d[3], fmaf(0.75f, d[2], 0.5f * d[1]))) - d[5];
+  t[2] = fmaf(-3.0f, d[5], fmaf(-3.0f, d[4], fmaf(6.75f, d[3], fmaf(0.75f, d[2], -1.5f * d[1]))));
+  t[3] = fmaf(-1.5f, d[5], fmaf(-3.75f, d[4], fmaf(3.75f, d[2], 1.5f * d[1])));
+  t[4] = fmaf(-2.5f, d[5], fmaf(-3.75f, d[4], fmaf(5.0f, d[3], fmaf(3.75f, d[2], -2.5f * d[1]))));
+  t[5] = fmaf(-4.0f, d[5], fmaf(5.0f, d[3], -d[1]));
+  t[6] = fmaf(2.0f, d[5], fmaf(-1.25f, d[4], fmaf(-2.5f, d[3], fmaf(0.25f, d[2], 0.5f * d[1])))) + d[6];
+}
+__device__ __forceinline__ void at4x7(const float (&m)[7], float (&s)[4]) {
+  s[0] = m[0] + m[1] + m[2] + m[3] + m[4] + m[5];
+  s[1] = fmaf(-2.0f, m[5], fmaf(-0.5f, m[4], fmaf(0.5f, m[3], m[1] - m[2])));
+  s[2] = fmaf(4.0f, m[5], fmaf(0.25f, m[4], fmaf(0.25f, m[3], m[1] + m[2])));
+  s[3] = fmaf(-8.0f, m[5], fmaf(-0.125f, m[4], fmaf(0.125f, m[3], m[1] - m[2]))) + m[6];
+}
+__device__ __forceinline__ void btn(const float (&d)[8], float (&t)[8]) { bt8(d, t); }
+__device__ __forceinline__ void btn(const float (&d)[7], float (&t)[7]) { bt7(d, t); }
+__device__ __forceinline__ void atn(const float (&m)[8], float (&s)[5]) { at5x8(m, s); }
+__device__ __forceinline__ void atn(const float (&m)[7], float (&s)[4]) { at4x7(m, s); }
+
+constexpr int kDrop = 5;
+__host__ __device__ constexpr int wino7_point(int i, int N) { return N == 8 || i < kDrop ? i : i + 1; }
+__host__ __device__ constexpr int wino7_rank(int p) { return p - 1 - (p > kDrop ? 1 : 0); }
+
 struct Wino7Place { int base_ci, idx, kmul, slot; };
-__device__ __forceinline__ bool wino7_place(int p, int q, int pa, int pb, Wino7Place& o) {
+__device__ __forceinline__ bool wino7_uplace(int p, int q, int pa, int pb, Wino7Place& o) {
   if (p != 0 && q != 0) { o = Wino7Place{0, (p - 1) * 7 + (q - 1), 4, 2 * pa + pb}; return true; }
   if (p == 0 && q != 0) { o = Wino7Place{196, q - 1, 2, pb}; return pa == 1; }
   if (q == 0 && p != 0) { o = Wino7Place{210, p - 1, 2, pa}; return pb == 1; }
   o = Wino7Place{224, 0, 1, 0};
   return pa == 1 && pb == 1;
 }
-__device__ __forceinline__ int wino7_mindex(int p, int q) {
-  return p != 0 && q != 0 ? (p - 1) * 7 + (q - 1) : (p == 0 && q != 0 ? 49 + q - 1 : (q == 0 && p != 0 ? 56 + p - 1 : 63));
-}
+struct Wino7VPlace { int vbase, mbase, idx, kmul, ry, rx; };
+__host__ __device__ constexpr Wino7VPlace wino7_vplace(int p, int q) {
+  const bool dp = p == kDrop, dq = q == kDrop;
+  const int ry = dp ? 2 : 3, rx = dq ? 2 : 3;
+  if (p != 0 && q != 0) {
+    if (!dp && !dq) return Wino7VPlace{0, 0, wino7_rank(p) * 6 + wino7_rank(q), 4, ry, rx};
+    if (dp && dq) return Wino7VPlace{1833, 525, 0, 4, ry, rx};
+    return Wino7VPlace{1521, 441, dp ? wino7_rank(q) : 6 + wino7_rank(p), 4, ry, rx};
+  }
+  if (p == 0 && q != 0) return dq ? Wino7VPlace{1809, 513, 0, 2, ry, rx} : Wino7VPlace{1296, 324, wino7_rank(q), 2, ry, rx};
+  if (q == 0 && p != 0) return dp ? Wino7VPlace{1821, 519, 0, 2, ry, rx} : Wino7VPlace{1404, 378, wino7_rank(p), 2, ry, rx};
+  return Wino7VPlace{1512, 432, 0, 1, ry, rx};
+}
+static_assert(wino7_vplace(kDrop, kDrop).vbase + 16 == kWino7Units && wino7_vplace(kDrop, kDrop).mbase + 4 == kWino7Pairs, "V / M sizes");
+__device__ __forceinline__ bool wino7_slot(int p, int q, int pa, int pb, int& slot) {
+  if (p != 0 && q != 0) { slot = 2 * pa + pb; return true; }
+  if (p == 0 && q != 0) { slot = pb; return pa == 1; }
+  if (q == 0 && p != 0) { slot = pa; return pb == 1; }
+  slot = 0;
+  return pa == 1 && pb == 1;
+}
+}
+
+template <int NY, int NX>
+__device__ __forceinline__ void wino7_input_tile(const float* xi, int x_cs, unsigned c4, int pa, int pb, int ty, int tx, int img, int n_img,
+                                                 int Ci, float* __restrict__ V) {
+  const int oy = ty * 5, ox = tx * 5;
+  float t[NY][NX];
+#pragma unroll
+  for (int j = 0; j < NX; ++j) {
+    const int col = ox - 2 + j, cc = min(max(col, 0), 13);
+#pragma unroll
+    for (int i = 0; i < NY; ++i) {
+      const int row = oy - 2 + i, rr = min(max(row, 0), 13);
+      t[i][j] = *reinterpret_cast<const float*>(reinterpret_cast<const char*>(xi + (size_t)((2 * rr + pa) * 28 + 2 * cc + pb) * x_cs) + c4);
+    }
+  }
+#pragma unroll
+  for (int j = 0; j < NX; ++j) {
+    const int col = ox - 2 + j;
+    float d[NY];
+#pragma unroll
+    for (int i = 0; i < NY; ++i) {
+      const int row = oy - 2 + i;
+      d[i] = (unsigned)row < 14u && (unsigned)col < 14u ? t[i][j] : 0.f;
+    }
+    float tc[NY];
+    btn(d, tc);
+#pragma unroll
+    for (int i = 0; i < NY; ++i) t[i][j] = tc[i];
+  }
+#pragma unroll
+  for (int pi = 0; pi < NY; ++pi) {
+    float v[NX];
+    btn(t[pi], v);
+#pragma unroll
+    for (int qi = 0; qi < NX; ++qi) {
+      const int p = wino7_point(pi, NY), q = wino7_point(qi, NX);
+      const Wino7VPlace pl = wino7_vplace(p, q);
+      int slot;
+      if (wino7_slot(p, q, pa, pb, slot)) {
+        const size_t row = (size_t)pl.idx * n_img * (pl.ry * pl.rx) + (size_t)((img * pl.ry + ty) * pl.rx + tx);
+        __builtin_nontemporal_store(v[qi], reinterpret_cast<float*>(reinterpret_cast<char*>(V + ((size_t)pl.vbase * n_img + row * pl.kmul + slot) * Ci) + c4));
+      }
+    }
+  }
 }
 
 __global__ __launch_bounds__(256) void wino7_input_kernel(const float* __restrict__ x, int x_cs, int x_coff, int n_img, int Ci,
@@ -54,42 +141,14 @@
   const unsigned c = (unsigned)(r - ph * cw) * 64u + (threadIdx.x & 63u);
   if (c >= (unsigned)Ci) return;
   const unsigned c4 = c * 4u;
-  const int img = tile / kWino7Tiles, tt = tile - img * kWino7Tiles, oy = (tt / 3) * 5, ox = (tt % 3) * 5;
+  const int img = tile / kWino7Tiles, tt = tile - img * kWino7Tiles, ty = tt / 3, tx = tt - ty * 3;
   const float* xi = x + (size_t)img * 784 * x_cs + x_coff;
-  float t[8][8];
-#pragma unroll
-  for (int j = 0; j < 8; ++j) {
-    const int col = ox - 2 + j, cc = min(max(col, 0), 13);
-#pragma unroll
-    for (int i = 0; i < 8; ++i) {
-      const int row = oy - 2 + i, rr = min(max(row, 0), 13);
-      t[i][j] = *reinterpret_cast<const float*>(reinterpret_cast<const char*>(xi + (size_t)((2 * rr + pa) * 28 + 2 * cc + pb) * x_cs) + c4);
-    }
-  }
-#pragma unroll
-  for (int j = 0; j < 8; ++j) {
-    const int col = ox - 2 + j;
-    float d[8];
-#pragma unroll
-    for (int i = 0; i < 8; ++i) {
-      const int row = oy - 2 + i;
-      d[i] = (unsigned)row < 14u && (unsigned)col < 14u ? t[i][j] : 0.f;
-    }
-    float tc[8];
-    bt8(d, tc);
-#pragma unroll
-    for (int i = 0; i < 8; ++i) t[i][j] = tc[i];
-  }
-#pragma unroll
-  for (int p = 0; p < 8; ++p) {
-    float v[8];
-    bt8(t[p], v);
-#pragma unroll
-    for (int q = 0; q < 8; ++q) {
-      Wino7Place pl;
-      if (wino7_place(p, q, pa, pb, pl))
-        __builtin_nontemporal_store(v[q], reinterpret_cast<float*>(reinterpret_cast<char*>(V + ((size_t)pl.base_ci * T + ((size_t)pl.idx * T + tile) * pl.kmul + pl.slot) * Ci) + c4));
-    }
+  if (ty < 2) {
+    if (tx < 2) wino7_input_tile<8, 8>(xi, x_cs, c4, pa, pb, ty, tx, img, n_img, Ci, V);
+    else wino7_input_tile<8, 7>(xi, x_cs, c4, pa, pb, ty, tx, img, n_img, Ci, V);
+  } else {
+    if (tx < 2) wino7_input_tile<7, 8>(xi, x_cs, c4, pa, pb, ty, tx, img, n_img, Ci, V);
+    else wino7_input_tile<7, 7>(xi, x_cs, c4, pa, pb, ty, tx, img, n_img, Ci, V);
   }
 }
 
@@ -99,41 +158,51 @@
   float* y; int y_cs, y_coff;
   int n_img, Co, flags;
 };
+template <int NY, int NX>
+__device__ __forceinline__ void wino7_output_tile(const Wino7OutArgs& a, int ty, int tx, int img, int c) {
+  constexpr int OY = NY - 3, OX = NX - 3;
+  float s[OY][NX];
+#pragma unroll
+  for (int qi = 0; qi < NX; ++qi) {
+    float m[NY];
+#pragma unroll
+    for (int pi = 0; pi < NY; ++pi) {
+      const Wino7VPlace pl = wino7_vplace(wino7_point(pi, NY), wino7_point(qi, NX));
+      const size_t row = (size_t)pl.idx * a.n_img * (pl.ry * pl.rx) + (size_t)((img * pl.ry + ty) * pl.rx + tx);
+      m[pi] = a.M[((size_t)pl.mbase * a.n_img + row) * a.Co + c];
+    }
+    float sc[OY];
+    atn(m, sc);
+#pragma unroll
+    for (int i = 0; i < OY; ++i) s[i][qi] = sc[i];
+  }
+  const float bv = a.bias ? a.bias[c] : 0.f;
+  const bool relu = (a.flags & OFFK_CONV_RELU_PRE_) || (a.flags & OFFK_CONV_RELU_POST_);
+#pragma unroll
+  for (int i = 0; i < OY; ++i) {
+    float yv[OX];
+    atn(s[i], yv);
+    const int row = ty * 5 + i;
+#pragma unroll
+    for (int j = 0; j < OX; ++j) {
+      float v = yv[j] + bv;
+      if (relu) v = fmaxf(v, 0.f);
+      a.y[((size_t)img * 196 + row * 14 + tx * 5 + j) * a.y_cs + a.y_coff + c] = v;
+    }
+  }
+}
 __global__ __launch_bounds__(256) void wino7_output_kernel(Wino7OutArgs a) {
   const int T = a.n_img * kWino7Tiles;
   const long long gid = (long long)blockIdx.x * 256 + threadIdx.x;
   if (gid >= (long long)T * a.Co) return;
   const int tile = (int)(gid / a.Co), c = (int)(gid - (long long)tile * a.Co);
-  const int img = tile / kWino7Tiles, tt = tile - img * kWino7Tiles, oy = (tt / 3) * 5, ox = (tt % 3) * 5;
-  const float* mp = a.M + (size_t)tile * a.Co + c;
-  const size_t pstride = (size_t)T * a.Co;
-  float s[5][8];
-#pragma unroll
-  for (int q = 0; q < 8; ++q) {
-    float m[8];
-#pragma unroll
-    for (int p = 0; p < 8; ++p) m[p] = mp[(size_t)wino7_mindex(p, q) * pstride];
-    float sc[5];
-    at5x8(m, sc);
-#pragma unroll
-    for (int i = 0; i < 5; ++i) s[i][q] = sc[i];
-  }
-  const float bv = a.bias ? a.bias[c] : 0.f;
-  const bool relu = (a.flags & OFFK_CONV_RELU_PRE_) || (a.flags & OFFK_CONV_RELU_POST_);
-#pragma unroll
-  for (int i = 0; i < 5; ++i) {
-    float yv[5];
-    at5x8(s[i], yv);
-    const int row = oy + i;
-#pragma unroll
-    for (int j = 0; j < 5; ++j) {
-      const int col = ox + j;
-      if (row < 14 && col < 14) {
-        float v = yv[j] + bv;
-        if (relu) v = fmaxf(v, 0.f);
-        a.y[((size_t)img * 196 + row * 14 + col) * a.y_cs + a.y_coff + c] = v;
-      }
-    }
+  const int img = tile / kWino7Tiles, tt = tile - img * kWino7Tiles, ty = tt / 3, tx = tt - ty * 3;
+  if (ty < 2) {
+    if (tx < 2) wino7_output_tile<8, 8>(a, ty, tx, img, c);
+    else wino7_output_tile<8, 7>(a, ty, tx, img, c);
+  } else {
+    if (tx < 2) wino7_output_tile<7, 8>(a, ty, tx, img, c);
+    else wino7_output_tile<7, 7>(a, ty, tx, img, c);
   }
 }
 
@@ -165,17 +234,36 @@
 #pragma unroll
     for (int q = 0; q < 8; ++q) {
       Wino7Place pl;
-      if (wino7_place(p, q, pa, pb, pl))
+      if (wino7_uplace(p, q, pa, pb, pl))
         U[((size_t)pl.base_ci * Co + ((size_t)pl.idx * Co + co) * pl.kmul + pl.slot) * Ci + ci] = uu[q];
     }
   }
 }
 
-int wino7_groups(long long T, int Ci, int Co, WinoGroup out[4]) {
-  const int batch[4] = {49, 7, 7, 1}, kmul[4] = {4, 2, 2, 1}, base[4] = {0, 196, 210, 224}, first[4] = {0, 49, 56, 63};
-  for (int g = 0; g < 4; ++g)
-    out[g] = WinoGroup{batch[g], kmul[g], (long long)base[g] * T * Ci, (long long)base[g] * Co * Ci, (long long)first[g] * T * Co};
+int wino7_u_groups(int Ci, int Co, WinoGroup out[4]) {
+  const int batch[4] = {49, 7, 7, 1}, kmul[4] = {4, 2, 2, 1}, base[4] = {0, 196, 210, 224};
+  for (int g = 0; g < 4; ++g) out[g] = WinoGroup{batch[g], kmul[g], 0, 0, (long long)base[g] * Co * Ci, 0, 0, {}};
   return 4;
+}
+
+int wino7_groups(long long n_img, int Ci, int Co, WinoGroup out[kMaxWinoGroups]) {
+  WinoGroup ug[4];
+  wino7_u_groups(Ci, Co, ug);
+  const int vbase[8] = {1512, 0, 1296, 1404, 1833, 1521, 1809, 1821}, kg[8] = {3, 0, 1, 2, 0, 0, 1, 2};
+  for (int g = 0; g < 8; ++g) out[g] = WinoGroup{0, ug[kg[g]].kmul, 0, (long long)vbase[g] * n_img * Ci, ug[kg[g]].u_off, 0, 0, {}};
+  for (int p = 0; p < 8; ++p)
+    for (int q = 0; q < 8; ++q) {
+      const Wino7VPlace pl = wino7_vplace(p, q);
+      int g = 0;
+      while (vbase[g] != pl.vbase) ++g;
+      WinoGroup& o = out[g];
+      o.rows = n_img * pl.ry * pl.rx;
+      o.m_off = (long long)pl.mbase * n_img * Co;
+      o.u_sel[pl.idx] = (unsigned char)(p != 0 && q != 0 ? (p - 1) * 7 + (q - 1) : p == 0 && q != 0 ? q - 1 : q == 0 && p != 0 ? p - 1 : 0);
+      ++o.batch;
+    }
+  for (int g = 0; g < 8; ++g) out[g].nsel = out[g].batch;
+  return 8;
 }
 
 hipError_t wino7_weight_launch(const float* w_packed, int Co, int Ci, float* U, hipStream_t st) {
```
